# elybrand/quantized_neural_networks

Hardware: AMD Instinct MI355X
Metric: weights_quantized_per_sec (higher is better)
Workload: dtype f64; 1 GPU; Dense(4096->4096) whole-layer GPFQ, m=1024 calibration samples, M=3 alphabet, alphabet_scalar=3 (BASELINE.json configs[1], the north-star layer); N=4096, C=4096, m=1024, M=3, neurons_per_gpu=4096, arithmetic=f32 products / f64 residual and dot products (reference's mixed flow)

## Files before the change

quantized_neural_networks_amd/csrc/gpfq_blk.hip:

```cpp
#include <atomic>
#include <cmath>
#include <cstring>
#include <type_traits>

#include <cstdlib>
#include <mutex>
#include <optional>
#include <utility>
#include "gpfq_device.hpp"
#include <hip/hip_ext.h>
#include "gpfq_launch.hpp"
#include "gpfq_roles.hpp"

namespace gpfq {

namespace {

struct BlkStats {
    double rden, G, cb, ca, Ea, nrm;
    double sE1, sE2;
};
struct BandEntry {
    double H1, H2, E1, E2;
};
static_assert(sizeof(BlkStats) == 64 && sizeof(BandEntry) == 32, "header layout");

__host__ __device__ constexpr int blk_band(int B, bool CL = false) { return CL ? 3 * B - 1 : 2 * B - 1; }
__host__ __device__ constexpr int blk_hdr_bytes(int B, bool CL = false) { return (64 + blk_band(B, CL) * 32 + 127) & ~127; }
__host__ __device__ constexpr bool blk_row64(int G, int B) { return B > 1 && G > 1; }
__host__ __device__ constexpr int64_t blk_rec_bytes(int64_t mp, int B, int G, bool CL = false) { return blk_hdr_bytes(B, CL) + (blk_row64(G, B) ? 16 : 12) * mp; }

template <int B, bool R64, bool CL = false>
__global__ void __launch_bounds__(256)
gpfq_blk_prep_kernel(const float *__restrict__ X, const float *__restrict__ Xq, int64_t ld, int64_t N, int m, int mp,
                     const float *__restrict__ nrm32, char *__restrict__ recs, char *__restrict__ hdrs,
                     const DevAlphabet *__restrict__ alpha, int sym, int nsl, int64_t slice_bytes)
{
    const float sym_a = sym ? alpha->sym_a : 0.f;
    constexpr int GREC = R64 ? 2 : 1;
    constexpr int ND = blk_band(B, CL), NV = 3 + 4 * ND;
    constexpr int DN = CL ? 2 * B : B;
    __shared__ double sm[4][((NV + 3) & ~3) + 1];
    const int64_t t = blockIdx.x;
    constexpr int hdr = blk_hdr_bytes(B, CL);
    const int mps = nsl > 1 ? mp / nsl : mp;
    char *rb = recs + t * blk_rec_bytes(mps, B, GREC, CL);
    float  *ox = reinterpret_cast<float *>(rb + hdr);
    float  *oq = ox + mps;
    double *od = reinterpret_cast<double *>(rb + hdr + 8 * (int64_t)mps);
    const bool has_prev = t >= B && t - B < N, has_cur = t < N, has_next = t + DN < N;
    const float *px = X + (t - B) * ld, *pq = Xq + (t - B) * ld;
    const float *cx = X + t * ld, *cq = Xq + t * ld;
    const float *nq = Xq + (t + DN) * ld;
    const int lane = threadIdx.x & 63, wave = threadIdx.x >> 6;
    const double up = 1.0 + 0x1p-20;

    constexpr int NP = (NV + 3) & ~3;
    double v[NP];
#pragma unroll
    for (int k = 0; k < NP; ++k) v[k] = 0.0;
    auto one = [&](float xc, float qc_, const float (&bx)[ND], const float (&bq)[ND]) {
        const double q = (double)qc_, pr = q * (double)xc;
        v[0] += pr; v[1] += fabs(pr); v[2] += fabs(q);
#pragma unroll
        for (int d = 1; d <= ND; ++d) {
            const double p1 = q * (double)bx[d - 1], p2 = q * (double)bq[d - 1];
            v[3 + 4 * (d - 1) + 0] += p1;       v[3 + 4 * (d - 1) + 1] += p2;
            v[3 + 4 * (d - 1) + 2] += fabs(p1); v[3 + 4 * (d - 1) + 3] += fabs(p2);
        }
    };
    const bool vec = (ld % 4 == 0) && (((uintptr_t)X | (uintptr_t)Xq) % 16 == 0);
    if (vec) {
        const float4 z4 = make_float4(0.f, 0.f, 0.f, 0.f);
        for (int i = 4 * threadIdx.x; i < mp; i += 1024) {
            auto row = [&](const float *base, int64_t r) -> float4 {
                if (r < 0 || r >= N || i >= m) return z4;
                float4 w = *reinterpret_cast<const float4 *>(base + r * ld + i);
                if (i + 3 >= m) { w.y = i + 1 < m ? w.y : 0.f; w.z = i + 2 < m ? w.z : 0.f; w.w = 0.f; }
                return w;
            };
            const float4 xp = row(X, t - B), qp = row(Xq, t - B), qn = row(Xq, t + DN);
            const float4 xc = row(X, t), qc4 = row(Xq, t);
            float4 bx4[ND], bq4[ND];
#pragma unroll
            for (int d = 1; d <= ND; ++d) { bx4[d - 1] = row(X, t - d); bq4[d - 1] = row(Xq, t - d); }
            const int sl = nsl > 1 ? i / mps : 0, il = i - sl * mps;
            const int64_t so = (int64_t)sl * slice_bytes;
            float *oxs = reinterpret_cast<float *>(reinterpret_cast<char *>(ox) + so), *oqs = reinterpret_cast<float *>(reinterpret_cast<char *>(oq) + so);
            double *ods = reinterpret_cast<double *>(reinterpret_cast<char *>(od) + so);
            *reinterpret_cast<float4 *>(oxs + il) = xp;
            *reinterpret_cast<float4 *>(oqs + il) = sym_a != 0.f ? make_float4(__fmul_rn(sym_a, qp.x), __fmul_rn(sym_a, qp.y), __fmul_rn(sym_a, qp.z), __fmul_rn(sym_a, qp.w)) : qp;
            if constexpr (R64) {
                *reinterpret_cast<double2 *>(ods + il) = make_double2((double)qn.x, (double)qn.y);
                *reinterpret_cast<double2 *>(ods + il + 2) = make_double2((double)qn.z, (double)qn.w);
            } else {
                *reinterpret_cast<float4 *>(reinterpret_cast<float *>(ods) + il) = qn;
            }
            float b1[ND], b2[ND];
#pragma unroll
            for (int d = 0; d < ND; ++d) { b1[d] = bx4[d].x; b2[d] = bq4[d].x; }
            one(xc.x, qc4.x, b1, b2);
#pragma unroll
            for (int d = 0; d < ND; ++d) { b1[d] = bx4[d].y; b2[d] = bq4[d].y; }
            one(xc.y, qc4.y, b1, b2);
#pragma unroll
            for (int d = 0; d < ND; ++d) { b1[d] = bx4[d].z; b2[d] = bq4[d].z; }
            one(xc.z, qc4.z, b1, b2);
#pragma unroll
            for (int d = 0; d < ND; ++d) { b1[d] = bx4[d].w; b2[d] = bq4[d].w; }
            one(xc.w, qc4.w, b1, b2);
        }
    } else {
        for (int i = threadIdx.x; i < mp; i += 256) {
            const bool in = i < m;
            const int sl = nsl > 1 ? i / mps : 0, il = i - sl * mps;
            const int64_t so = (int64_t)sl * slice_bytes;
            float *oxs = reinterpret_cast<float *>(reinterpret_cast<char *>(ox) + so), *oqs = reinterpret_cast<float *>(reinterpret_cast<char *>(oq) + so);
            double *ods = reinterpret_cast<double *>(reinterpret_cast<char *>(od) + so);
            oxs[il] = (has_prev && in) ? px[i] : 0.f;
            oqs[il] = (has_prev && in) ? (sym_a != 0.f ? __fmul_rn(sym_a, pq[i]) : pq[i]) : 0.f;
            if constexpr (R64) ods[il] = (double)((has_next && in) ? nq[i] : 0.f);
            else reinterpret_cast<float *>(ods)[il] = (has_next && in) ? nq[i] : 0.f;
            if (has_cur && in) {
                float b1[ND], b2[ND];
#pragma unroll
                for (int d = 1; d <= ND; ++d) {
                    b1[d - 1] = t - d >= 0 ? X[(t - d) * ld + i] : 0.f;
                    b2[d - 1] = t - d >= 0 ? Xq[(t - d) * ld + i] : 0.f;
                }
                one(cx[i], cq[i], b1, b2);
            }
        }
    }
#pragma unroll
    for (int g = 0; g < NP / 4; ++g) {
        double x = fold16(fold32(v[4 * g], v[4 * g + 2]), fold32(v[4 * g + 1], v[4 * g + 3]));
        x = ror_add<8>(x); x = ror_add<4>(x); x = ror_add<2>(x); x = ror_add<1>(x);
        if ((lane & 15) == 0) sm[wave][4 * g + (lane >> 4)] = x;
    }
    __syncthreads();
    auto total = [&](int k) { return (sm[0][k] + sm[1][k]) + (sm[2][k] + sm[3][k]); };
    if (threadIdx.x == 0) {
        BlkStats st{};
        const double nrm = has_cur ? (double)nrm32[t] : 0.0;
        const double s1 = total(1), s2 = total(2);
        st.nrm = nrm;
        st.rden = nrm < 1e-16 ? 0.0 : 1.0 / (nrm * nrm);
        st.G = total(0);
        st.cb = 0x1p-23 * s1 * st.rden * up;
        st.ca = 0x1p-149 * s2 * st.rden * up;
        st.Ea = 0x1p-149 * s2 * up;
        double e1 = 0.0, e2 = 0.0;
#pragma unroll
        for (int d = 1; d <= ND; ++d) { e1 += total(5 + 4 * (d - 1)); e2 += total(6 + 4 * (d - 1)); }
        st.sE1 = 0x1p-23 * e1 * up * up; st.sE2 = 0x1p-23 * e2 * up * up;
        for (int sl = 0; sl < (nsl > 1 ? nsl : 1); ++sl) *reinterpret_cast<BlkStats *>(rb + (int64_t)sl * slice_bytes) = st;
        *reinterpret_cast<BlkStats *>(hdrs + t * hdr) = st;
    } else if (threadIdx.x <= ND) {
        const int d = threadIdx.x;
        BandEntry e;
        e.H1 = total(3 + 4 * (d - 1)); e.H2 = total(4 + 4 * (d - 1));
        e.E1 = 0x1p-23 * total(5 + 4 * (d - 1)) * up; e.E2 = 0x1p-23 * total(6 + 4 * (d - 1)) * up;
        for (int sl = 0; sl < (nsl > 1 ? nsl : 1); ++sl) *reinterpret_cast<BandEntry *>(rb + (int64_t)sl * slice_bytes + 64 + 32 * (d - 1)) = e;
        *reinterpret_cast<BandEntry *>(hdrs + t * hdr + 64 + 32 * (d - 1)) = e;
    }
}

constexpr int kPrepRunMax = 16;
template <int B, bool R64>
__global__ void __launch_bounds__(256)
gpfq_blk_prep_run_kernel(const float *__restrict__ X, const float *__restrict__ Xq, int64_t ld, int64_t N, int m, int mp, int64_t nrec, int RUN,
                         const float *__restrict__ nrm32, char *__restrict__ recs, char *__restrict__ hdrs,
                         const DevAlphabet *__restrict__ alpha, int sym, unsigned *__restrict__ zero16)
{
    constexpr int GREC = R64 ? 2 : 1;
    constexpr int ND = blk_band(B), NV = 3 + 4 * ND, NP = (NV + 3) & ~3;
    constexpr int hdr = blk_hdr_bytes(B);
    __shared__ double sm[kPrepRunMax][4][NP + 1];
    __shared__ double nsm[kPrepRunMax][4];
    const bool own_norms = nrm32 == nullptr;
    if (zero16 && blockIdx.x == 0 && threadIdx.x < 16) zero16[threadIdx.x] = 0u;
    const float sym_a = sym ? alpha->sym_a : 0.f;
    const int64_t t0 = (int64_t)blockIdx.x * RUN;
    const int lane = threadIdx.x & 63, wave = threadIdx.x >> 6;
    const double up = 1.0 + 0x1p-20;
    for (int k = threadIdx.x; k < RUN * 4 * (NP + 1); k += 256) (&sm[0][0][0])[k] = 0.0;
    __syncthreads();
    const float4 z4 = make_float4(0.f, 0.f, 0.f, 0.f);
    const int64_t rbytes = blk_rec_bytes(mp, B, GREC);
    for (int i = 4 * threadIdx.x; i < mp; i += 1024) {
        auto row = [&](const float *base, int64_t r) -> float4 {
            if (r < 0 || r >= N || i >= m) return z4;
            float4 w = *reinterpret_cast<const float4 *>(base + r * ld + i);
            if (i + 3 >= m) { w.y = i + 1 < m ? w.y : 0.f; w.z = i + 2 < m ? w.z : 0.f; w.w = 0.f; }
            return w;
        };
        float4 wx[ND], wq[ND];
#pragma unroll
        for (int d = 1; d <= ND; ++d) { wx[d - 1] = row(X, t0 - d); wq[d - 1] = row(Xq, t0 - d); }
        float4 xc = row(X, t0), qc4 = row(Xq, t0), qn = row(Xq, t0 + B);
#pragma unroll 1
        for (int r = 0; r < RUN; ++r) {
            const int64_t t = t0 + r;
            const float4 xc1 = r + 1 < RUN ? row(X, t + 1) : z4, qc1 = r + 1 < RUN ? row(Xq, t + 1) : z4, qn1 = r + 1 < RUN ? row(Xq, t + 1 + B) : z4;
            if (t < nrec) {
                char *rb = recs + t * rbytes;
                float *ox = reinterpret_cast<float *>(rb + hdr), *oq = ox + mp;
                const float4 xp = wx[B - 1], qp = wq[B - 1];
                *reinterpret_cast<float4 *>(ox + i) = xp;
                *reinterpret_cast<float4 *>(oq + i) = sym_a != 0.f ? make_float4(__fmul_rn(sym_a, qp.x), __fmul_rn(sym_a, qp.y), __fmul_rn(sym_a, qp.z), __fmul_rn(sym_a, qp.w)) : qp;
                if constexpr (R64) {
                    double *od = reinterpret_cast<double *>(rb + hdr + 8 * (int64_t)mp);
                    *reinterpret_cast<double2 *>(od + i) = make_double2((double)qn.x, (double)qn.y);
                    *reinterpret_cast<double2 *>(od + i + 2) = make_double2((double)qn.z, (double)qn.w);
                } else {
                    *reinterpret_cast<float4 *>(reinterpret_cast<float *>(rb + hdr + 8 * (int64_t)mp) + i) = qn;
                }
            }
            if (own_norms) {
                double s = 0.0;
                s = fma((double)qc4.x, (double)qc4.x, s);
                s = fma((double)qc4.y, (double)qc4.y, s);
                s = fma((double)qc4.z, (double)qc4.z, s);
                s = fma((double)qc4.w, (double)qc4.w, s);
                s = wave_sum(s);
                if (lane == 0) nsm[r][wave] = s;
            }
            double v[NP];
#pragma unroll
            for (int k = 0; k < NP; ++k) v[k] = 0.0;
            auto one = [&](float xcs, float qcs, const float (&bx)[ND], const float (&bq)[ND]) {
                const double q = (double)qcs, pr = q * (double)xcs;
                v[0] += pr; v[1] += fabs(pr); v[2] += fabs(q);
#pragma unroll
                for (int d = 1; d <= ND; ++d) {
                    const double p1 = q * (double)bx[d - 1], p2 = q * (double)bq[d - 1];
                    v[3 + 4 * (d - 1) + 0] += p1;       v[3 + 4 * (d - 1) + 1] += p2;
                    v[3 + 4 * (d - 1) + 2] += fabs(p1); v[3 + 4 * (d - 1) + 3] += fabs(p2);
                }
            };
            float b1[ND], b2[ND];
#pragma unroll
            for (int d = 0; d < ND; ++d) { b1[d] = wx[d].x; b2[d] = wq[d].x; }
            one(xc.x, qc4.x, b1, b2);
#pragma unroll
            for (int d = 0; d < ND; ++d) { b1[d] = wx[d].y; b2[d] = wq[d].y; }
            one(xc.y, qc4.y, b1, b2);
#pragma unroll
            for (int d = 0; d < ND; ++d) { b1[d] = wx[d].z; b2[d] = wq[d].z; }
            one(xc.z, qc4.z, b1, b2);
#pragma unroll
            for (int d = 0; d < ND; ++d) { b1[d] = wx[d].w; b2[d] = wq[d].w; }
            one(xc.w, qc4.w, b1, b2);
#pragma unroll
            for (int g = 0; g < NP / 4; ++g) {
                double x = fold16(fold32(v[4 * g], v[4 * g + 2]), fold32(v[4 * g + 1], v[4 * g + 3]));
                x = ror_add<8>(x); x = ror_add<4>(x); x = ror_add<2>(x); x = ror_add<1>(x);
                if ((lane & 15) == 0) sm[r][wave][4 * g + (lane >> 4)] += x;
            }
#pragma unroll
            for (int d = ND - 1; d >= 1; --d) { wx[d] = wx[d - 1]; wq[d] = wq[d - 1]; }
            wx[0] = xc; wq[0] = qc4;
            xc = xc1; qc4 = qc1; qn = qn1;
        }
    }
    __syncthreads();
    for (int w = threadIdx.x; w < RUN * (ND + 1); w += 256) {
        const int r = w / (ND + 1), e = w - r * (ND + 1);
        const int64_t t = t0 + r;
        if (t >= nrec) continue;
        auto total = [&](int k) { return (sm[r][0][k] + sm[r][1][k]) + (sm[r][2][k] + sm[r][3][k]); };
        char *rb = recs + t * rbytes;
        if (e == 0) {
            BlkStats st{};
            const double nrm = t < N ? (own_norms ? (double)(float)sqrt(nsm[r][0] + nsm[r][1] + nsm[r][2] + nsm[r][3]) : (double)nrm32[t]) : 0.0;
            const double s1 = total(1), s2 = total(2);
            st.nrm = nrm;
            st.rden = nrm < 1e-16 ? 0.0 : 1.0 / (nrm * nrm);
            st.G = total(0);
            st.cb = 0x1p-23 * s1 * st.rden * up;
            st.ca = 0x1p-149 * s2 * st.rden * up;
            st.Ea = 0x1p-149 * s2 * up;
            double e1 = 0.0, e2 = 0.0;
#pragma unroll
            for (int d = 1; d <= ND; ++d) { e1 += total(5 + 4 * (d - 1)); e2 += total(6 + 4 * (d - 1)); }
            st.sE1 = 0x1p-23 * e1 * up * up; st.sE2 = 0x1p-23 * e2 * up * up;
            *reinterpret_cast<BlkStats *>(rb) = st;
            *reinterpret_cast<BlkStats *>(hdrs + t * hdr) = st;
        } else {
            const int d = e;
            BandEntry be;
            be.H1 = total(3 + 4 * (d - 1)); be.H2 = total(4 + 4 * (d - 1));
            be.E1 = 0x1p-23 * total(5 + 4 * (d - 1)) * up; be.E2 = 0x1p-23 * total(6 + 4 * (d - 1)) * up;
            *reinterpret_cast<BandEntry *>(rb + 64 + 32 * (d - 1)) = be;
            *reinterpret_cast<BandEntry *>(hdrs + t * hdr + 64 + 32 * (d - 1)) = be;
        }
    }
}

__global__ void __launch_bounds__(256)
gpfq_blk_scale_kernel(char *__restrict__ recs, int64_t rec_bytes, int hdr, int mps, int64_t slice_bytes, const DevAlphabet *__restrict__ alpha)
{
    const float a = alpha->sym_a;
    float4 *row = reinterpret_cast<float4 *>(recs + (int64_t)blockIdx.y * slice_bytes + (int64_t)blockIdx.x * rec_bytes + hdr + 4 * (int64_t)mps);
    for (int i = threadIdx.x; i < mps / 4; i += 256) {
        const float4 v = row[i];
        row[i] = make_float4(__fmul_rn(a, v.x), __fmul_rn(a, v.y), __fmul_rn(a, v.z), __fmul_rn(a, v.w));
    }
}

template <int G, int NL, bool CL = false> constexpr bool blk_sweep_flush() { return (G == 4 && NL == 1) || CL; }

struct BlkLds {
    int tile_bytes, tile_pitch, off_w, off_d, off_wq, off_x2, off_e, off_out, off_ctl, off_zero, off_hr, hr_pitch, total;
};
constexpr int kOutSteps = 32;

__host__ __device__ constexpr int blk_sublanes(int nb) { return 64 / nb > 8 ? 8 : 64 / nb; }
__host__ __device__ constexpr int blk_slots(int nsw, int nb) { return (nsw + blk_sublanes(nb) - 1) / blk_sublanes(nb) * blk_sublanes(nb); }

__host__ __device__ inline BlkLds blk_lds(int mp, int nb, int B, int nsw, int G, bool CL = false)
{
    BlkLds L;
    const int nw = blk_slots(nsw, nb);
    L.tile_bytes = B * (int)blk_rec_bytes(mp, B, G, CL);
    L.tile_pitch = (L.tile_bytes + 1023) & ~1023;
    int o = 2 * L.tile_pitch;
    L.off_w = o;    o += 2 * nb * B * 4;    o = (o + 15) & ~15;
    L.off_d = o;    o += 2 * nw * B * nb * 8;
    L.off_wq = o;   o += 2 * nb * B * 8;
    L.off_x2 = o;   o += nw * nb * 16;
    L.off_e = o;    o += 68 * 8;
    L.off_out = o;  o += nb * kOutSteps * 8;
    L.off_ctl = o;  o += 16;
    L.off_zero = o; o += 32;
    o = (o + 15) & ~15;
    L.hr_pitch = (B * blk_hdr_bytes(B, CL) + 1023) & ~1023;
    L.off_hr = o;   o += 3 * L.hr_pitch;
    L.total = o;
    return L;
}

struct BlkK {
    const char *recs;
    const char *hdrs;
    const float *Wt;
    int64_t ldw, ldt;
    int64_t N, C;
    int m, M, zero_idx, nblk;
    int8_t *qidx;
    float *Qt;
    int64_t o_sj, o_st;
    const DevAlphabet *alpha;
    int *alpha_err;
    double *resid, *u_out;
    unsigned long long *fallback_count;
    unsigned long long *stamps;
    const float *Xq;
    int64_t ldx;
    unsigned char pw[12];
    int nsl;
    int cl_map;
    int64_t slice_bytes;
    unsigned long long *mbox;
    int64_t u_ld;
    double slack;
    int *cl_err;
    unsigned long long cl_timeout;
    int cl_fault;
};

constexpr int kTop3Ship = 3;
constexpr int kPkAheadShip = 3;
struct BlkPrioSched { int d21[3], d10[3]; };
constexpr BlkPrioSched kPrioSched[2] = {{{4, 4, 4}, {8, 8, 8}}, {{2, 4, 6}, {6, 8, 10}}};
constexpr int kPrioShip = 3 + 4 * 1;
#ifdef GPFQ_BLK_DIAG
#include "gpfq_blk_diag.hpp"
#else
constexpr bool kNoMfmaD = false, kNoFused = false;
constexpr int kTop3 = kTop3Ship;
constexpr int kPkAhead = kPkAheadShip;
constexpr int kPrio = kPrioShip;
#define STAMP(var) do { } while (0)
#define STAMP_DO(...)
#endif

struct ClState { int64_t cl; int slice; unsigned seq; bool dead; int64_t rec_off; int m_sl; };
typedef unsigned cl_u32x4 __attribute__((ext_vector_type(4)));

__device__ __forceinline__ cl_u32x4 cl_load16(const unsigned long long *p)
{
    cl_u32x4 r;
    asm volatile("global_load_dwordx4 %0, %1, off sc1" : "=&v"(r) : "v"(p) : "memory");
    return r;
}

template <int KV>
__device__ __forceinline__ void cl_publish(const BlkK &K, ClState &cs, int lane, const double (&v)[KV])
{
    const unsigned seq = ++cs.seq;
    if (K.cl_fault && cs.cl == 0 && cs.slice == 1) return;
    unsigned long long *buf = K.mbox + ((cs.cl * 2 + (int64_t)(seq & 1u)) * (int64_t)K.nsl) * 256;
    unsigned long long *mine = buf + ((int64_t)cs.slice * 64 + lane) * 4;
#pragma unroll
    for (int k = 0; k < KV; ++k) {
        const cl_u32x4 w = {(unsigned)__double2loint(v[k]), seq, (unsigned)__double2hiint(v[k]), seq};
        asm volatile("global_store_dwordx4 %0, %1, off sc1" :: "v"(mine + 2 * k), "v"(w) : "memory");
// ... 50 lines not shown
template <int KV, int CLB>
__device__ __forceinline__ void cl_exchange(const BlkK &K, ClState &cs, int lane, double (&v)[KV])
{
    cl_publish<KV>(K, cs, lane, v);
    cl_gather<KV, CLB>(K, cs, lane, v);
}

struct BlkPairs { int pw[11]; };
constexpr BlkPairs kP8{{1, 1, 1, 1, 1, 1, 1, 1}}, kP12{{1, 2, 2, 1, 1, 2, 2, 1}}, kP16{{1, 2, 2, 2, 1, 3, 3, 2}},
                   kP24{{1, 3, 3, 3, 2, 4, 4, 4}}, kP32{{2, 4, 4, 4, 3, 5, 5, 5}}, kP40{{5, 5, 5, 5, 5, 5, 5, 5}};
constexpr BlkPairs kP16x7{{3, 3, 2, 1, 3, 2, 2}}, kP24x7{{4, 4, 4, 1, 4, 4, 3}}, kP32x7{{5, 5, 5, 2, 5, 5, 5}};
constexpr BlkPairs kP32quad{{2, 5, 5, 4, 2, 5, 5, 4}};
constexpr BlkPairs kP16x11{{2, 2, 1, 1, 2, 2, 1, 1, 1, 1, 2}}, kP24x11{{2, 2, 2, 2, 2, 2, 2, 1, 3, 3, 3}}, kP32x11{{3, 3, 3, 3, 3, 3, 3, 2, 3, 3, 3}},
                   kP48x11{{4, 5, 4, 4, 5, 4, 4, 5, 4, 4, 5}}, kP64x11{{4, 6, 6, 6, 6, 6, 6, 6, 6, 6, 6}};
constexpr BlkPairs kP64oct{{6, 6, 6, 6, 6, 6, 6, 4, 6, 6, 6}};
struct BlkInst { int G, S, B, NSW, NL, CLM; BlkPairs split; };
constexpr BlkInst kBlkInst[] = {
    {4, 16, 4,  7, 1, 0, kP16x7},   {4, 16, 4,  7, 2, 0, kP16x7},   {4, 24, 4,  7, 1, 0, kP24x7},   {4, 24, 4,  7, 2, 0, kP24x7},   {4, 32, 4,  7, 1, 0, kP32x7},   {4, 32, 4,  7, 2, 0, kP32x7},
    {4, 16, 4,  8, 1, 0, kP16},     {4, 16, 4,  8, 2, 0, kP16},     {4, 24, 4,  8, 1, 0, kP24},     {4, 24, 4,  8, 2, 0, kP24},     {4, 32, 4,  8, 1, 0, kP32quad}, {4, 32, 4,  8, 2, 0, kP32quad},
    {1,  4, 4,  4, 1, 0, {{1, 1, 1, 1}}}, {1,  4, 4,  4, 2, 0, {{1, 1, 1, 1}}},
    {1,  8, 4,  8, 1, 0, kP8},      {1,  8, 4,  8, 2, 0, kP8},      {1, 12, 2,  8, 1, 0, kP12},     {1, 12, 2,  8, 2, 0, kP12},
    {1, 16, 2,  8, 1, 0, kP16},     {1, 16, 2,  8, 2, 0, kP16},     {1, 24, 1,  8, 1, 0, kP24},     {1, 24, 1,  8, 2, 0, kP24},
    {1, 32, 1,  8, 1, 0, kP32},     {1, 32, 1,  8, 2, 0, kP32},     {1, 40, 1,  8, 1, 0, kP40},     {1, 40, 1,  8, 2, 0, kP40},
    {1, 40, 1,  8, 4, 0, kP40},     {2, 48, 1, 11, 4, 0, kP48x11},  {2, 64, 1, 11, 4, 0, kP64x11},  {1, 24, 1,  8, 4, 0, kP24},     {1, 32, 1,  8, 4, 0, kP32},
    {4, 48, 2, 11, 4, 0, kP48x11},  {4, 64, 2, 11, 4, 0, kP64x11},
    {4, 16, 4, 11, 4, 0, kP16x11},  {4, 24, 4, 11, 4, 0, kP24x11},  {4, 32, 4, 11, 4, 0, kP32x11},  {8, 64, 4, 11, 2, 0, kP64oct},
    {4, 16, 4,  8, 4, 0, kP16},     {4, 24, 4,  8, 4, 0, kP24},     {4, 32, 4,  8, 4, 0, kP32},
    {1,  8, 4,  8, 4, 0, kP8},      {1, 12, 2,  8, 4, 0, kP12},     {1, 16, 2,  8, 4, 0, {{1, 2, 2, 3, 2, 2, 2, 2}}},
    {2, 16, 4,  8, 4, 0, kP16},     {2, 24, 2,  8, 4, 0, kP24},     {2, 32, 2,  8, 4, 0, kP32},
    {4, 24, 4,  8, 4, 1, kP24},     {4, 24, 4, 11, 4, 1, kP24x11},  {4, 32, 4, 11, 4, 1, kP32x11},  {8, 64, 4, 11, 2, 1, kP64oct},  {4, 32, 4,  8, 1, 1, kP32quad}, {4, 32, 4,  8, 2, 1, kP32quad},
};
constexpr int kBlkInsts = (int)(sizeof(kBlkInst) / sizeof(kBlkInst[0]));
constexpr bool blk_sym_only(const BlkInst &r) { return r.G == 8; }

constexpr int blk_inst_find(int G, int S, int B, int NSW, int NL, int CLM)
{
    int row = -1;
    for (int i = 0; i < kBlkInsts && (B < 0 || row < 0); ++i) {
        const BlkInst &r = kBlkInst[i];
        if (r.G != G || r.S != S || r.NSW != NSW || r.NL != NL || (B >= 0 && (r.B != B || r.CLM != CLM))) continue;
        if (row < 0) row = i;
        for (int w = 0; w < 11; ++w)
            if (r.split.pw[w] != kBlkInst[row].split.pw[w]) return -1;
    }
    return row;
}
constexpr int blk_pairs(const BlkInst &r) { int n = 0; for (int w = 0; w < r.NSW; ++w) n += r.split.pw[w]; return n; }

template <int G, int S, int NSW, int NL> constexpr const int *blk_split()
{
    constexpr int row = blk_inst_find(G, S, -1, NSW, NL, 0);
    static_assert(row >= 0, "kBlkInst has no row for this instantiation, or two with different splits");
    static_assert(blk_pairs(kBlkInst[row]) == S, "the row's pairs do not sum to S");
    return kBlkInst[row].split.pw;
}

template <int G, int S, int NSW, int NL> constexpr bool blk_split_has(int k)
{
    for (int w = 0; w < NSW; ++w)
        if (blk_split<G, S, NSW, NL>()[w] == k) return true;
    return false;
}

template <int G, int PW, int MP, int B, int NSW, bool SYM, int NL, int CLM>
__device__ __forceinline__ void blk_sweep_role(const BlkK &K, char *lds_generic, const BlkLds &L, int wave, int lane, int pbase, const ClState &cs)
{
    constexpr bool CL = CLM != 0;
    constexpr int NB = NL * G, KQ = 64 / G, NW = blk_slots(NSW, NB);
    constexpr int RSH = NL == 4 ? 0 : (NL == 2 ? 1 : 2);
    constexpr int HDR = blk_hdr_bytes(B, CL);
    constexpr int RB = (int)blk_rec_bytes(MP, B, G, CL);
    lchar *lds = (lchar *)lds_generic;
    const int ng = lane & (G - 1), kq = lane / G, row = lane >> 4;
    const bool writer = (lane & 15 & ~(G - 1)) == 0 && (row & ((1 << RSH) - 1)) == 0;
    const int nloc = NL * ng;
    const int nrow = row >> RSH;
    const int64_t jbase = cs.cl * NB;
    const unsigned ldsT_addr = lds_addr(lds_generic), ldsW_addr = lds_addr(lds_generic + L.off_w);
    const int64_t N = K.N;
    const int nslots = K.nblk + 1;
    constexpr int PU = G == 8 ? 2 : 1;
    static_assert(PW % PU == 0, "whole units per wavefront");
    auto pair_off = [](int p) { return PU * (p / PU) * KQ + p % PU; };
    const int o_x  = HDR + 8 * (pbase + PU * kq);
    int o_q = o_x + 4 * MP;
    asm volatile("" : "+v"(o_q));
    constexpr int DB = blk_row64(G, B) ? 16 : 8;
    const int o_d  = HDR + 8 * MP + DB * (pbase + PU * kq);
    using DRaw = std::conditional_t<blk_row64(G, B), double2, float2>;
    auto ld_d = [&](int off) -> DRaw { return lds_ld<DRaw>(lds, off); };
    auto to_d2 = [](const DRaw &v) -> double2 { return make_double2((double)v.x, (double)v.y); };
    const int o_wq = L.off_wq + nloc * B * 8;
    const int o_dw = L.off_d + (wave * B * NB + nloc + nrow) * 8;
    const int o_x2 = L.off_x2 + (wave * NB + nloc + nrow) * 16;

    double u[NL][2 * PW];
#pragma unroll
    for (int i = 0; i < NL; ++i)
#pragma unroll
        for (int e = 0; e < 2 * PW; ++e) u[i][e] = 0.0;

    constexpr int NPIECES = (B * RB + 1023) >> 10;
    constexpr int PER_MIN = NPIECES / NSW;
    constexpr int PTS = PW >= 2 ? 2 : 1;
    constexpr int PPP = PER_MIN / (PTS * B) > 0 ? PER_MIN / (PTS * B) : 1;
    const unsigned lane16 = (unsigned)lane * 16u;
    auto issue_piece = [&](int b1, int k) {
        const int pc = wave + NSW * k;
        glds16_s(K.recs + (CL ? cs.rec_off : (int64_t)0) + (int64_t)b1 * L.tile_bytes + ((int64_t)pc << 10), lane16,
                 ldsT_addr + (unsigned)(b1 & 1) * (unsigned)L.tile_pitch + ((unsigned)pc << 10));
    };
    auto load_weights = [&](int b1) {
        const unsigned dw = ldsW_addr + (unsigned)((b1 & 1) * NB * B * 4);
        for (int i0 = wave * 64; i0 < NB * B; i0 += NSW * 64) {
            const int i = i0 + lane;
            const int n = i / B, s = i - n * B;
            const int64_t jn = jbase + n, t = (int64_t)b1 * B + s;
            if (i < NB * B && jn < K.C && t < N) glds4(K.Wt + jn * K.ldw + t * K.ldt, dw + 4 * (unsigned)i0);
        }
    };

    constexpr int NHP = (B * HDR + 1023) >> 10;
    auto load_headers = [&](int b2, int buf) {
        if (wave < NHP && b2 <= K.nblk)
            glds16_s(K.hdrs + (int64_t)b2 * B * HDR + ((int64_t)wave << 10), lane16,
                     lds_addr(lds_generic + L.off_hr) + (unsigned)buf * (unsigned)L.hr_pitch + ((unsigned)wave << 10));
    };
    for (int k = 0; wave + NSW * k < NPIECES; ++k) issue_piece(0, k);
    load_weights(0);
    load_headers(0, 0); load_headers(1, 1);
    dma_wait();
    slot_barrier();
    int hbuf = 2;
    unsigned long long st0 = 0, st1 = 0, st2 = 0, st3 = 0, st4 = 0, st5 = 0, acc_dma = 0, acc_u = 0, acc_d = 0, acc_w = 0, acc_b = 0, acc_t = 0;
    (void)st0; (void)st1; (void)st2; (void)st3; (void)st4; (void)st5; (void)acc_dma; (void)acc_u; (void)acc_d; (void)acc_w; (void)acc_b; (void)acc_t;

    constexpr bool kMfmaD = (G == 4 || (G == 8 && NL == 2)) && B == 4 && blk_row64(G, B) && (!kNoMfmaD || G == 8);
    constexpr bool kFused = kMfmaD && (!kNoFused || G == 8);
    static_assert(G != 8 || kFused, "the eight-group lane map exists in the fused form only");
    constexpr bool kBatchTop = kFused && (NL == 4 || G == 8) && NSW == 11;
    constexpr bool kTopSym = kBatchTop && SYM;
    constexpr int kPrioForm = CL ? (kPrio >> 2) & 3 : kPrio & 3;
    constexpr bool kPrioUp = kTopSym && G == 8 && (kPrioForm & 1) != 0;
    constexpr int NUW = PW / PU;
    constexpr bool kLateHdr = kTopSym && NUW >= 2 && (kTop3 & 1) != 0, kLateW = kTopSym && NUW >= 2 && (kTop3 & 2) != 0;
    constexpr int kHdrStep = NUW >= 3 ? 8 : 6, kWStep = NUW >= 3 ? 10 : 7;
    static_assert(!(kLateHdr || kLateW) || (NUW <= 3 && B == 4 && PTS == 2 && PER_MIN <= 6), "the free pair-steps of a two- or three-pair wavefront");
    static_assert(!kLateW || NB * B == 64, "one 256-byte weight piece per block");
    unsigned long long w_lanes = 0ull, w_tail = 0ull;
    int w_whole = 0;
    const float *wsrc = nullptr;
    if constexpr (kLateW) {
        w_lanes = wave == 0 ? __builtin_amdgcn_ballot_w64(jbase + lane / B < K.C) : 0ull;
        w_tail = w_lanes & (0x1111111111111111ull * ((1ull << (int)(N % B)) - 1ull));
        w_whole = (int)(N / B);
        wsrc = K.Wt + (jbase + lane / B) * K.ldw + (int64_t)(B + lane % B) * K.ldt;
    }
    (void)w_lanes; (void)w_tail; (void)w_whole; (void)wsrc;
    constexpr bool kPreloadAll = PW * B <= 8 && PW <= 5 && !kFused;
    constexpr bool kHoist = kPreloadAll && PW * B <= 4;
    constexpr int PB = kPreloadAll ? B : 1, PP = kPreloadAll ? PW : 1;
    constexpr bool kPreD = kHoist && PW * B * (blk_row64(G, B) ? 4 : 2) <= 16 && !kMfmaD;
    constexpr int DBn = kPreD ? B : 1, DPn = kPreD ? PW : 1;
    float2 xs[PB][PP], qs[PB][PP], wqa[PB][NL];
    DRaw ds[DBn][DPn];
    auto preload_wq = [&](int b) {
        const int pbq = ((b - 1) & 1) * NB * B * 8;
#pragma unroll
        for (int s = 0; s < PB; ++s)
#pragma unroll
            for (int n = 0; n < NL; ++n) wqa[s][n] = lds_ld<float2>(lds, o_wq + pbq + (n * B + s) * 8);
    };
    auto preload_rows = [&](int b) {
        const int tbase = (b & 1) * L.tile_pitch;
#pragma unroll
        for (int s = 0; s < PB; ++s)
#pragma unroll
            for (int p = 0; p < PP; ++p) {
                xs[s][p] = lds_ld<float2>(lds, tbase + s * RB + o_x + 8 * p * KQ);
                qs[s][p] = lds_ld<float2>(lds, tbase + s * RB + o_q + 8 * p * KQ);
                if constexpr (kPreD) ds[s][p] = ld_d(tbase + s * RB + o_d + DB * p * KQ);
            }
    };
    if constexpr (kHoist) { preload_wq(0); preload_rows(0); }

    auto slow_path = [&](int b, int ctl) {
        for (;;) {
            const int S = __builtin_amdgcn_readfirstlane(ctl);
            if (S < 0) break;
            const int nb_ = ((b + 1) & 1) * L.tile_pitch;
            const int cbq = (b & 1) * NB * B * 8;
            double eu[NL], ew[NL];
#pragma unroll
            for (int n = 0; n < NL; ++n) { eu[n] = 0.0; ew[n] = 0.0; }
#pragma unroll
            for (int n = 0; n < NL; ++n) {
                const float w = lds_ld<float2>(lds, o_wq + cbq + (n * B + S) * 8).x;
#pragma unroll 1
                for (int p = 0; p < PW; ++p) {
                    double t0 = u[n][0], t1 = u[n][1];
#pragma unroll
                    for (int pp = 1; pp < PW; ++pp) { t0 = (p == pp) ? u[n][2 * pp] : t0; t1 = (p == pp) ? u[n][2 * pp + 1] : t1; }
                    for (int j = 0; j < S; ++j) {
                        const int rb = nb_ + j * RB;
                        const float2 x2 = lds_ld<float2>(lds, rb + o_x + 8 * pair_off(p)), q2 = lds_ld<float2>(lds, rb + o_q + 8 * pair_off(p));
                        const float2 wq = lds_ld<float2>(lds, o_wq + cbq + (n * B + j) * 8);
                        if constexpr (SYM) {
                            t0 += (double)__fmaf_rn(wq.y, q2.x, __fmul_rn(wq.x, x2.x));
                            t1 += (double)__fmaf_rn(wq.y, q2.y, __fmul_rn(wq.x, x2.y));
                        } else {
                            t0 += (double)__fsub_rn(__fmul_rn(wq.x, x2.x), __fmul_rn(wq.y, q2.x));
                            t1 += (double)__fsub_rn(__fmul_rn(wq.x, x2.y), __fmul_rn(wq.y, q2.y));
                        }
                    }
                    const int rb = nb_ + S * RB;
                    const float2 x2 = lds_ld<float2>(lds, rb + o_x + 8 * pair_off(p));
                    float2 q2;
                    if constexpr (SYM) {
                        const int i0 = 2 * (pbase + pair_off(p) + PU * kq);
                        const float *xr = K.Xq + ((int64_t)b * B + S) * K.ldx + (CL ? (int64_t)cs.slice * MP : (int64_t)0);
                        const int mrow = CL ? cs.m_sl : K.m;
                        q2.x = i0 < mrow ? xr[i0] : 0.f;
                        q2.y = i0 + 1 < mrow ? xr[i0 + 1] : 0.f;
                    } else {
                        q2 = lds_ld<float2>(lds, rb + o_q + 8 * pair_off(p));
                    }
                    eu[n] = fma((double)q2.x, t0, eu[n]);
                    eu[n] = fma((double)q2.y, t1, eu[n]);
                    ew[n] = fma((double)q2.x, t0 + (double)__fmul_rn(w, x2.x), ew[n]);
                    ew[n] = fma((double)q2.y, t1 + (double)__fmul_rn(w, x2.y), ew[n]);
                }
            }
            const double vu = fold_klanes_n<G, NL>(eu), vw = fold_klanes_n<G, NL>(ew);
            if (writer) lds_st<double2>(lds, o_x2, make_double2(vu, vw));
            slot_barrier();
            slot_barrier();
            if constexpr (kBatchTop) ctl = lds_read_now(lds + L.off_ctl + 4 * (b & 1));
            else ctl = lds_ld<int>(lds, L.off_ctl + 4 * (b & 1));
        }
    };
    if constexpr (kBatchTop) __builtin_amdgcn_s_waitcnt(0);
    for (int b = 0; b < nslots; ++b) {
        STAMP(st0);
        STAMP_DO(if (b) acc_t += st0 - st5;)
        if (blk_sweep_flush<G, NL, CL>() && b >= 1 && wave == b % NSW && lane < NB * B && (!CL || cs.slice == 0)) {
            const int nn = lane / B, sidx = lane % B;
            const int64_t t = (int64_t)(b - 1) * B + sidx, jn = jbase + nn;
            if (t < N && jn < K.C) {
                const int2 v = lds_ld<int2>(lds, L.off_out + (nn * kOutSteps + (int)(t % kOutSteps)) * 8);
                if (K.qidx) K.qidx[jn * N + t] = (int8_t)v.x;
                if (K.Qt) K.Qt[jn * N + t] = __int_as_float(v.y);
            }
        }
        if constexpr (!kLateW) {
            if (b + 1 < nslots) load_weights(b + 1);
        }
        if constexpr (!kLateHdr) { load_headers(b + 2, hbuf); hbuf = hbuf == 2 ? 0 : hbuf + 1; }
        const int bn = b + 1 < nslots ? b + 1 : b;
        STAMP(st1);
        const int tbase = (b & 1) * L.tile_pitch;
        const int pbq = ((b - 1) & 1) * NB * B * 8;

        auto update_pair = [&](int p, const float2 &x2, const float2 &q2, const float (&wv)[NL], const float (&qv)[NL]) {
            const pk2 xv = {x2.x, x2.y}, qx = {q2.x, q2.y};
            pk2 pr[NL], rr[NL], dd[NL];
            double c0[NL], c1[NL];
#pragma unroll
            for (int n = 0; n < NL; ++n) pr[n] = pk2{wv[n], wv[n]} * xv;
            if constexpr (SYM) {
#pragma unroll
                for (int n = 0; n < NL; ++n) dd[n] = __builtin_elementwise_fma(pk2{qv[n], qv[n]}, qx, pr[n]);
            } else {
#pragma unroll
                for (int n = 0; n < NL; ++n) rr[n] = pk2{qv[n], qv[n]} * qx;
#pragma unroll
                for (int n = 0; n < NL; ++n) dd[n] = pr[n] - rr[n];
            }
#pragma unroll
            for (int n = 0; n < NL; ++n) { c0[n] = (double)dd[n].x; c1[n] = (double)dd[n].y; }
#pragma unroll
            for (int n = 0; n < NL; ++n) { u[n][2 * p] += c0[n]; u[n][2 * p + 1] += c1[n]; }
        };
        auto update_unit2 = [&](int P, const float4 &x4, const float4 &q4, const float (&wv)[NL], const float (&qv)[NL]) {
            const pk2 xv[2] = {{x4.x, x4.y}, {x4.z, x4.w}}, qx[2] = {{q4.x, q4.y}, {q4.z, q4.w}};
            pk2 pr[2][NL], rr[2][NL], dd[2][NL];
            double c0[2][NL], c1[2][NL];
#pragma unroll
            for (int h = 0; h < 2; ++h)
#pragma unroll
                for (int n = 0; n < NL; ++n) pr[h][n] = pk2{wv[n], wv[n]} * xv[h];
            if constexpr (SYM) {
#pragma unroll
                for (int h = 0; h < 2; ++h)
#pragma unroll
                    for (int n = 0; n < NL; ++n) dd[h][n] = __builtin_elementwise_fma(pk2{qv[n], qv[n]}, qx[h], pr[h][n]);
            } else {
#pragma unroll
                for (int h = 0; h < 2; ++h)
#pragma unroll
                    for (int n = 0; n < NL; ++n) rr[h][n] = pk2{qv[n], qv[n]} * qx[h];
#pragma unroll
                for (int h = 0; h < 2; ++h)
#pragma unroll
                    for (int n = 0; n < NL; ++n) dd[h][n] = pr[h][n] - rr[h][n];
            }
#pragma unroll
            for (int h = 0; h < 2; ++h)
#pragma unroll
                for (int n = 0; n < NL; ++n) { c0[h][n] = (double)dd[h][n].x; c1[h][n] = (double)dd[h][n].y; }
#pragma unroll
            for (int h = 0; h < 2; ++h)
#pragma unroll
                for (int n = 0; n < NL; ++n) { u[n][4 * P + 2 * h] += c0[h][n]; u[n][4 * P + 2 * h + 1] += c1[h][n]; }
        };
        (void)update_unit2;
        auto unit2_products = [&](pk2 (&dd)[2][NL], const float4 &x4, const float4 &q4, const float2 (&wq)[NL]) {
            const pk2 xv[2] = {{x4.x, x4.y}, {x4.z, x4.w}}, qx[2] = {{q4.x, q4.y}, {q4.z, q4.w}};
#pragma unroll
            for (int h = 0; h < 2; ++h)
#pragma unroll
                for (int n = 0; n < NL; ++n) dd[h][n] = pk2{wq[n].x, wq[n].x} * xv[h];
#pragma unroll
            for (int h = 0; h < 2; ++h)
#pragma unroll
                for (int n = 0; n < NL; ++n) dd[h][n] = __builtin_elementwise_fma(pk2{wq[n].y, wq[n].y}, qx[h], dd[h][n]);
        };
        auto unit2_accumulate_ahead = [&](int P, pk2 (&dd)[2][NL], bool nxt, const float4 &x4, const float4 &q4, const float2 (&wq)[NL]) {
            const pk2 xv[2] = {{x4.x, x4.y}, {x4.z, x4.w}}, qx[2] = {{q4.x, q4.y}, {q4.z, q4.w}};
            double c0[2][NL], c1[2][NL];
#pragma unroll
            for (int h = 0; h < 2; ++h)
#pragma unroll
                for (int n = 0; n < NL; ++n) {
                    c0[h][n] = (double)dd[h][n].x; c1[h][n] = (double)dd[h][n].y;
                    if (nxt) dd[h][n] = pk2{wq[n].x, wq[n].x} * xv[h];
                    __builtin_amdgcn_sched_barrier(0);
                }
#pragma unroll
            for (int h = 0; h < 2; ++h)
#pragma unroll
                for (int n = 0; n < NL; ++n) {
                    u[n][4 * P + 2 * h] += c0[h][n]; u[n][4 * P + 2 * h + 1] += c1[h][n];
                    if (nxt) dd[h][n] = __builtin_elementwise_fma(pk2{wq[n].y, wq[n].y}, qx[h], dd[h][n]);
                    __builtin_amdgcn_sched_barrier(0);
                }
        };
        (void)unit2_products; (void)unit2_accumulate_ahead;
        if constexpr (kFused) {
            const int rbm = tbase + (G == 8 ? lane & 3 : ng) * RB + o_d;
            constexpr int NU = PW / PU;
            constexpr bool kRows2 = kTopSym && G == 8 && (kPkAhead & 1) != 0;
            constexpr bool kPkA = kRows2 && (kPkAhead & 2) != 0;
            constexpr int PF = (NSW == 7 || kRows2) ? 2 : 1, NPS = NU * B;
            using XRow = std::conditional_t<PU == 2, float4, float2>;
            struct DRow2 { double2 v[2]; };
            using DRow = std::conditional_t<PU == 2, DRow2, double2>;
            auto dhalf = [](const DRow &r, int h) -> const double2 & { if constexpr (PU == 2) return r.v[h]; else return r; };
            float2 fwq[B][NL];
            XRow xbuf[PF], qbuf[PF];
            DRow dcur;
            auto row_off = [&](int i, bool q) { return tbase + (i % B) * RB + (q ? o_q : o_x) + 8 * PU * (i / B) * KQ; };
            auto ld_drow = [&](int off) -> DRow {
                if constexpr (PU == 2) return DRow{{lds_ld<double2>(lds, off), lds_ld<double2>(lds, off + 16)}};
                else return lds_ld<double2>(lds, off);
            };
            auto first_requests = [&]() {
#pragma unroll
                for (int s = 0; s < B; ++s)
#pragma unroll
                    for (int n = 0; n < NL; ++n) fwq[s][n] = lds_ld<float2>(lds, o_wq + pbq + (n * B + s) * 8);
#pragma unroll
                for (int i = 0; i < PF; ++i)
                    if (i < NPS) { xbuf[i] = lds_ld<XRow>(lds, row_off(i, false)); qbuf[i] = lds_ld<XRow>(lds, row_off(i, true)); }
                dcur = ld_drow(rbm);
            };
            if constexpr (kTopSym && G == 8) {
                static_assert(!(kTopSym && G == 8) || (B == 4 && NL == 2 && PU == 2 && PF == (kRows2 ? 2 : 1) && NPS >= 4), "slot_top_sym2: two neurons per lane, pair-steps 0..2 are unit 0's steps 0..2");
                nf4 w01[2], w23[2], x2n, q2n;
                nd2 d01[2];
                __builtin_amdgcn_s_setprio(2);
                slot_top_sym2<RB>(w01, w23, x2n, q2n, d01, u[0][0], u[0][1], u[0][2], u[0][3], u[1][0], u[1][1], u[1][2], u[1][3],
                                  lds + row_off(0, false), lds + row_off(0, true), lds + o_wq + pbq, lds + rbm);
                __builtin_amdgcn_s_waitcnt(0xC07F);
                __builtin_memcpy(&xbuf[0], &x2n, sizeof(XRow)); __builtin_memcpy(&qbuf[0], &q2n, sizeof(XRow));
                if constexpr (kRows2) { xbuf[PF - 1] = lds_ld<XRow>(lds, row_off(3, false)); qbuf[PF - 1] = lds_ld<XRow>(lds, row_off(3, true)); }
#pragma unroll
                for (int h = 0; h < PU; ++h) dcur.v[h] = make_double2(d01[h].x, d01[h].y);
#pragma unroll
                for (int n = 0; n < NL; ++n) {
                    fwq[0][n] = make_float2(w01[n].x, w01[n].y); fwq[1][n] = make_float2(w01[n].z, w01[n].w);
                    fwq[2][n] = make_float2(w23[n].x, w23[n].y); fwq[3][n] = make_float2(w23[n].z, w23[n].w);
                }
            } else if constexpr (kTopSym) {
                static_assert(!kTopSym || (B == 4 && NL == 4 && PF == 1), "slot_top_sym: four neurons per lane, pair-steps 0..2 are pair 0's steps 0..2");
                nf4 w01[4], w23[4];
                nf2 x2n, q2n;
                nd2 d0;
                __builtin_amdgcn_s_setprio(2);
                slot_top_sym<RB>(w01, w23, x2n, q2n, d0, u[0][0], u[0][1], u[1][0], u[1][1], u[2][0], u[2][1], u[3][0], u[3][1],
                                 lds + row_off(0, false), lds + row_off(0, true), lds + o_wq + pbq, lds + rbm);
                __builtin_amdgcn_s_waitcnt(0xC07F);
                xbuf[0] = make_float2(x2n.x, x2n.y); qbuf[0] = make_float2(q2n.x, q2n.y);
                dcur = make_double2(d0.x, d0.y);
#pragma unroll
                for (int n = 0; n < NL; ++n) {
                    fwq[0][n] = make_float2(w01[n].x, w01[n].y); fwq[1][n] = make_float2(w01[n].z, w01[n].w);
                    fwq[2][n] = make_float2(w23[n].x, w23[n].y); fwq[3][n] = make_float2(w23[n].z, w23[n].w);
                }
            } else if constexpr (kBatchTop) {
                static_assert(!kBatchTop || (B == 4 && NL == 4), "lds_read_slot_top reads four neurons' steps 0 and 1: 16 bytes at a stride of 4 steps x 8 bytes");
                nf2 x0, q0;
                nf4 w01[4];
                lds_read_slot_top(x0, q0, w01, lds + row_off(0, false), lds + row_off(0, true), lds + o_wq + pbq);
                xbuf[0] = make_float2(x0.x, x0.y); qbuf[0] = make_float2(q0.x, q0.y);
#pragma unroll
                for (int n = 0; n < NL; ++n) { fwq[0][n] = make_float2(w01[n].x, w01[n].y); fwq[1][n] = make_float2(w01[n].z, w01[n].w); }
#pragma unroll
                for (int s = 2; s < B; ++s)
#pragma unroll
                    for (int n = 0; n < NL; ++n) fwq[s][n] = lds_ld<float2>(lds, o_wq + pbq + (n * B + s) * 8);
                dcur = lds_ld<double2>(lds, rbm);
            } else {
                first_requests();
            }
            pk2 ddn[2][NL];
            if constexpr (kPkA) unit2_products(ddn, xbuf[2 % PF], qbuf[2 % PF], fwq[2]);
            (void)ddn;
            DRow dprev;
            if constexpr (PU == 2) dprev = DRow{{make_double2(0.0, 0.0), make_double2(0.0, 0.0)}};
            else dprev = make_double2(0.0, 0.0);
            double acc[NL];
#pragma unroll
            for (int n = 0; n < NL; ++n) acc[n] = 0.0;
            constexpr int NM = 2 * PU * NL;
            auto mfma_pair = [&](int pp, int i, const DRow &dd) {
                const int n = i % NL, e = i / NL;
                const double2 &dh = dhalf(dd, e / 2);
                acc[n] = __builtin_amdgcn_mfma_f64_4x4x4f64(u[n][2 * PU * pp + e], (e & 1) ? dh.y : dh.x, acc[n], 0, 0, 0);
            };
            constexpr int kSched = (kTopSym && G == 8 && NU == 3) ? (kPrioForm >> 1) & 1 : 0;
            auto prio_at = [&](int ips) {
                constexpr BlkPrioSched sc = kPrioSched[kSched];
                if (sc.d21[0] == sc.d21[1] && sc.d21[1] == sc.d21[2]) {
                    if (ips == sc.d21[0]) __builtin_amdgcn_s_setprio(1);
                } else {
                    if (ips == sc.d21[0]) setprio_if_age<0, 1>(wave);
                    if (ips == sc.d21[1]) setprio_if_age<1, 1>(wave);
                    if (ips == sc.d21[2]) setprio_if_age<2, 1>(wave);
                }
                if (sc.d10[0] == sc.d10[1] && sc.d10[1] == sc.d10[2]) {
                    if (ips == sc.d10[0]) __builtin_amdgcn_s_setprio(0);
                } else {
                    if (ips == sc.d10[0]) setprio_if_age<0, 0>(wave);
                    if (ips == sc.d10[1]) setprio_if_age<1, 0>(wave);
                    if (ips == sc.d10[2]) setprio_if_age<2, 0>(wave);
                }
            };
            (void)prio_at;
#pragma unroll
            for (int p = 0; p < NU; ++p) {
                if constexpr (kSched != 0) {
                    if (p == 0) __builtin_amdgcn_s_setprio(2);
                } else {
                    const int pr = 2 - (3 * p) / NU;
                    if (p == 0 || pr != 2 - (3 * (p - 1)) / NU) {
                        const int v = pr;
                        if (v >= 2) __builtin_amdgcn_s_setprio(2);
                        else if (v == 1) __builtin_amdgcn_s_setprio(1);
                        else __builtin_amdgcn_s_setprio(0);
                    }
                }
                if (p > 0) dcur = ld_drow(rbm + DB * PU * p * KQ);
#pragma unroll
                for (int st = 0; st < B; ++st) {
                    const int ips = p * B + st;
                    if (kTopSym && ips < 2) continue;
                    const XRow x2 = xbuf[ips % PF], q2 = qbuf[ips % PF];
                    const int pn = (ips + 1) / B, sn = (ips + 1) % B;
                    (void)pn; (void)sn;
                    if (ips + PF < NPS) {
                        xbuf[ips % PF] = lds_ld<XRow>(lds, row_off(ips + PF, false));
                        qbuf[ips % PF] = lds_ld<XRow>(lds, row_off(ips + PF, true));
                    }
                    if (kTopSym && ips < 4) {
#pragma unroll
                        for (int i = 0; i < PPP; ++i) {
                            const int k = (PTS * (ips - 2)) * PPP + i;
                            if (PTS * B * PPP <= PER_MIN || k < PER_MIN) issue_piece(bn, k);
                        }
                    }
                    if (p < PTS) {
#pragma unroll
                        for (int i = 0; i < PPP; ++i) {
                            const int k = (PTS * st + p) * PPP + i;
                            if (PTS * B * PPP <= PER_MIN || k < PER_MIN) issue_piece(bn, k);
                        }
                    }
                    if (kLateHdr && ips == kHdrStep) {
                        int b2 = b + 2;
                        asm volatile("" : "+s"(b2));
                        const unsigned on = ((unsigned)(wave - NHP) & (unsigned)(b2 - K.nblk - 1)) >> 31;
                        glds16_s_lanes(K.hdrs + (int64_t)b2 * B * HDR + ((int64_t)wave << 10), lane16,
                                       lds_addr(lds_generic + L.off_hr) + (unsigned)hbuf * (unsigned)L.hr_pitch + ((unsigned)wave << 10), 0ull - (unsigned long long)on);
                        hbuf = hbuf == 2 ? 0 : hbuf + 1;
                    }
                    if (kLateW && ips == kWStep) {
                        int b1 = b + 1;
                        asm volatile("" : "+s"(b1));
                        glds4_lanes(wsrc, ldsW_addr + (unsigned)((b1 & 1) * NB * B * 4), b1 < w_whole ? w_lanes : b1 == w_whole ? w_tail : 0ull);
                        wsrc += (int64_t)B * K.ldt;
                    }
                    __builtin_amdgcn_sched_barrier(0);
                    if constexpr (kSched != 0) prio_at(ips);
                    float wv[NL], qv[NL];
#pragma unroll
                    for (int n = 0; n < NL; ++n) { wv[n] = fwq[st][n].x; qv[n] = fwq[st][n].y; }
                    if constexpr (kPkA) unit2_accumulate_ahead(p, ddn, ips + 1 < NPS, xbuf[(ips + 1) % PF], qbuf[(ips + 1) % PF], fwq[(st + 1) % B]);
                    else if constexpr (PU == 2) update_unit2(p, x2, q2, wv, qv);
                    else update_pair(p, x2, q2, wv, qv);
                    if (p > 0) {
#pragma unroll
                        for (int i = 0; i < NM; ++i)
                            if (i * B / NM == st) mfma_pair(p - 1, i, dprev);
                    }
                    __builtin_amdgcn_sched_barrier(0);
                }
                dprev = dcur;
            }
            for (int k = PTS * B * PPP < PER_MIN ? PTS * B * PPP : PER_MIN; wave + NSW * k < NPIECES; ++k) issue_piece(bn, k);
            STAMP(st2);
#pragma unroll
            for (int i = 0; i < NM; ++i) mfma_pair(NU - 1, i, dprev);
#pragma unroll
            for (int n = 0; n < NL; ++n) {
                acc[n] = ror_add<8>(acc[n]);
                if constexpr (G == 4) acc[n] = ror_add<4>(acc[n]);
            }
            const bool dwriter = G == 8 ? (lane & 8) == 0 : (lane & 12) == 0;
            const int dgroup = G == 8 ? (lane >> 4) + (lane & 4) : lane >> 4;
            if (b + 1 < nslots && dwriter) {
                const int od = L.off_d + ((((((b + 1) & 1) * NW + wave) * B) + (lane & 3)) * NB + NL * dgroup) * 8;
                if constexpr (NL == 4) {
                    lds_st<double2>(lds, od, make_double2(acc[0], acc[1]));
                    lds_st<double2>(lds, od + 16, make_double2(acc[2], acc[3]));
                } else if constexpr (NL == 2) {
                    lds_st<double2>(lds, od, make_double2(acc[0], acc[NL - 1]));
                } else {
                    lds_st<double>(lds, od, acc[0]);
                }
            }
        } else {
        if constexpr (kPreloadAll) {
            if constexpr (!kHoist) { preload_wq(b); preload_rows(b); __builtin_amdgcn_sched_barrier(0); }
#pragma unroll
            for (int s = 0; s < B; ++s) {
                if (s == 0) __builtin_amdgcn_s_setprio(2);
                if (s == B / 2) __builtin_amdgcn_s_setprio(1);
                float wv[NL], qv[NL];
#pragma unroll
                for (int n = 0; n < NL; ++n) { wv[n] = wqa[s][n].x; qv[n] = wqa[s][n].y; }
#pragma unroll
                for (int p = 0; p < PW; ++p) {
                    if (p < PTS) {
#pragma unroll
                        for (int i = 0; i < PPP; ++i) {
                            const int k = (PTS * s + p) * PPP + i;
                            if (PTS * B * PPP <= PER_MIN || k < PER_MIN) issue_piece(bn, k);
                        }
                    }
                    update_pair(p, xs[s][p], qs[s][p], wv, qv);
                    __builtin_amdgcn_sched_barrier(0);
                }
            }
        } else
        {
            float2 x2n = lds_ld<float2>(lds, tbase + o_x), q2n = lds_ld<float2>(lds, tbase + o_q);
            float2 wqn[NL];
#pragma unroll
            for (int n = 0; n < NL; ++n) wqn[n] = lds_ld<float2>(lds, o_wq + pbq + (n * B) * 8);
#pragma clang loop unroll_count(B == 4 ? 2 : 1)
            for (int s = 0; s < B; ++s) {
                if (s == 0) __builtin_amdgcn_s_setprio(2);
                if (s == B / 2) __builtin_amdgcn_s_setprio(1);
                float wv[NL], qv[NL];
#pragma unroll
                for (int n = 0; n < NL; ++n) { wv[n] = wqn[n].x; qv[n] = wqn[n].y; }
                const int rb = tbase + s * RB;
                const int sn = s + 1 < B ? s + 1 : s;
#pragma unroll
                for (int n = 0; n < NL; ++n) wqn[n] = lds_ld<float2>(lds, o_wq + pbq + (n * B + sn) * 8);
#pragma unroll
                for (int p = 0; p < PW; ++p) {
                    const float2 x2 = x2n, q2 = q2n;
                    const int rbn = p + 1 < PW ? rb : tbase + sn * RB, pn = p + 1 < PW ? p + 1 : 0;
                    x2n = lds_ld<float2>(lds, rbn + o_x + 8 * pn * KQ);
                    q2n = lds_ld<float2>(lds, rbn + o_q + 8 * pn * KQ);
                    if (p < PTS) {
#pragma unroll
                        for (int i = 0; i < PPP; ++i) {
                            const int k = (PTS * s + p) * PPP + i;
                            if (PTS * B * PPP <= PER_MIN || k < PER_MIN) issue_piece(bn, k);
                        }
                    }
                    __builtin_amdgcn_sched_barrier(0);
                    update_pair(p, x2, q2, wv, qv);
                    __builtin_amdgcn_sched_barrier(0);
                }
            }
        }
        for (int k = PTS * B * PPP < PER_MIN ? PTS * B * PPP : PER_MIN; wave + NSW * k < NPIECES; ++k) issue_piece(bn, k);
        STAMP(st2);
        if constexpr (kMfmaD) {
            if (b + 1 < nslots) {
                __builtin_amdgcn_s_setprio(0);
                double acc[NL];
#pragma unroll
                for (int n = 0; n < NL; ++n) acc[n] = 0.0;
                const int rbm = tbase + ng * RB + o_d;
                double2 d2n = lds_ld<double2>(lds, rbm);
#pragma unroll
                for (int p = 0; p < PW; ++p) {
                    const double2 d2 = d2n;
                    if (p + 1 < PW) d2n = lds_ld<double2>(lds, rbm + DB * (p + 1) * KQ);
#pragma unroll
                    for (int n = 0; n < NL; ++n) acc[n] = __builtin_amdgcn_mfma_f64_4x4x4f64(u[n][2 * p], d2.x, acc[n], 0, 0, 0);
#pragma unroll
                    for (int n = 0; n < NL; ++n) acc[n] = __builtin_amdgcn_mfma_f64_4x4x4f64(u[n][2 * p + 1], d2.y, acc[n], 0, 0, 0);
                }
#pragma unroll
                for (int n = 0; n < NL; ++n) { acc[n] = ror_add<8>(acc[n]); acc[n] = ror_add<4>(acc[n]); }
                if ((lane & 12) == 0) {
                    const int od = L.off_d + ((((((b + 1) & 1) * NW + wave) * B) + (lane & 3)) * NB + NL * (lane >> 4)) * 8;
#pragma unroll
                    for (int n = 0; n < NL; ++n) lds_st<double>(lds, od + 8 * n, acc[n]);
                }
            }
        } else
        if (b + 1 < nslots && kPreloadAll) {
            DRaw dsl[B][PW];
#pragma unroll
            for (int r = 0; r < B; ++r)
#pragma unroll
                for (int p = 0; p < PW; ++p) {
                    if constexpr (kPreD) dsl[r][p] = ds[r][p];
                    else dsl[r][p] = ld_d(tbase + r * RB + o_d + DB * p * KQ);
                }
            if constexpr (!kPreD) __builtin_amdgcn_sched_barrier(0);
#pragma unroll
            for (int r = 0; r < B; ++r) {
                if (r == B / 2) __builtin_amdgcn_s_setprio(0);
                double acc[NL];
#pragma unroll
                for (int n = 0; n < NL; ++n) acc[n] = 0.0;
#pragma unroll
                for (int p = 0; p < PW; ++p) {
                    const double2 d2 = to_d2(dsl[r][p]);
#pragma unroll
                    for (int n = 0; n < NL; ++n) {
                        acc[n] = fma(d2.x, u[n][2 * p], acc[n]);
                        acc[n] = fma(d2.y, u[n][2 * p + 1], acc[n]);
                    }
                }
                const double v = fold_klanes_n<G, NL>(acc);
                if (writer) lds_st<double>(lds, o_dw + ((((b + 1) & 1) * NW) * B + r) * NB * 8, v);
            }
        } else
        if (b + 1 < nslots) {
            DRaw d2n = ld_d(tbase + o_d);
#pragma clang loop unroll_count(B == 4 ? 2 : 1)
            for (int r = 0; r < B; ++r) {
                if (r == B / 2) __builtin_amdgcn_s_setprio(0);
                double acc[NL];
#pragma unroll
                for (int n = 0; n < NL; ++n) acc[n] = 0.0;
                const int rb = tbase + r * RB;
                const int rn = r + 1 < B ? r + 1 : r;
#pragma unroll
                for (int p = 0; p < PW; ++p) {
                    const double2 d2 = to_d2(d2n);
                    const int rbn = p + 1 < PW ? rb : tbase + rn * RB, pn = p + 1 < PW ? p + 1 : 0;
                    d2n = ld_d(rbn + o_d + DB * pn * KQ);
                    __builtin_amdgcn_sched_barrier(0);
#pragma unroll
                    for (int n = 0; n < NL; ++n) {
                        acc[n] = fma(d2.x, u[n][2 * p], acc[n]);
                        acc[n] = fma(d2.y, u[n][2 * p + 1], acc[n]);
                    }
                    __builtin_amdgcn_sched_barrier(0);
                }
                const double v = fold_klanes_n<G, NL>(acc);
                if (writer) lds_st<double>(lds, o_dw + ((((b + 1) & 1) * NW) * B + r) * NB * 8, v);
            }
        }
        }
        STAMP(st3);
        dma_wait();
        STAMP(st4);
        if constexpr (kPrioUp) __builtin_amdgcn_s_setprio(2);
        slot_barrier();
        STAMP(st5);
        STAMP_DO(acc_dma += st1 - st0; acc_u += st2 - st1; acc_d += st3 - st2; acc_w += st4 - st3; acc_b += st5 - st4;)

        {
        int ctl;
        if constexpr (kBatchTop) ctl = lds_read_now(lds + L.off_ctl + 4 * (b & 1));
        else ctl = lds_ld<int>(lds, L.off_ctl + 4 * (b & 1));
        if constexpr (kHoist) {
            if (b + 1 < nslots) { preload_wq(b + 1); preload_rows(b + 1); }
        }
        if (__builtin_amdgcn_readfirstlane(ctl) >= 0) {
            slow_path(b, ctl);
            if constexpr (kHoist) {
                if (b + 1 < nslots) { preload_wq(b + 1); preload_rows(b + 1); }
            }
        }
        }
    }

    STAMP_DO(
    if (K.stamps && blockIdx.x == 0 && lane == 0 && (wave == 0 || wave == 7)) {
        unsigned long long *o = K.stamps + (wave == 0 ? 0 : 8);
        o[0] = acc_dma; o[1] = acc_u; o[2] = acc_d; o[3] = acc_w; o[4] = acc_b; o[5] = (unsigned long long)nslots; o[6] = acc_t;
    }
    if (K.stamps && blockIdx.x == 0 && lane == 0) {
        K.stamps[32 + wave] = acc_dma + acc_u + acc_d + acc_w;
        if (K.N * (int64_t)sizeof(RowStats) >= 64 * 8) { K.stamps[21 + wave] = acc_t; K.stamps[48 + wave] = acc_b; }
    }
    )
    if constexpr (kPrioUp) __builtin_amdgcn_s_setprio(0);
    if constexpr (G == 8) {
        if (K.resid) {
            double ss[4];
#pragma unroll
            for (int n = 0; n < NL; ++n)
#pragma unroll
                for (int h = 0; h < PU; ++h) {
                    double q = 0.0;
#pragma unroll
                    for (int P = 0; P < PW / PU; ++P)
#pragma unroll
                        for (int e = 0; e < 2; ++e) q = fma(u[n][2 * (PU * P + h) + e], u[n][2 * (PU * P + h) + e], q);
                    ss[PU * n + h] = q;
                }
            double v = fold_klanes<G>(ss);
            v = fold16(v, v);
            if (writer) lds_st<double>(lds, o_dw, v);
        }
    } else
    if (K.resid) {
        double ss[NL];
#pragma unroll
        for (int n = 0; n < NL; ++n) {
            double q = 0.0;
#pragma unroll
            for (int e = 0; e < 2 * PW; ++e) q = fma(u[n][e], u[n][e], q);
            ss[n] = q;
        }
        const double v = fold_klanes_n<G, NL>(ss);
        if (writer) lds_st<double>(lds, o_dw, v);
    }
    slot_barrier();
    if (K.u_out) {
#pragma unroll
        for (int n = 0; n < NL; ++n) {
            const int64_t jn = jbase + nloc + n;
            if (jn < K.C) {
#pragma unroll
                for (int p = 0; p < PW; ++p)
#pragma unroll
                    for (int e = 0; e < 2; ++e) {
                        const int i = 2 * (pbase + pair_off(p) + PU * kq) + e;
                        if constexpr (CL) {
                            if (i < cs.m_sl) K.u_out[jn * K.u_ld + (int64_t)cs.slice * MP + i] = u[n][2 * p + e];
                        } else {
                            if (i < K.m) K.u_out[jn * (int64_t)K.m + i] = u[n][2 * p + e];
                        }
                    }
            }
        }
    }
}

template <int G, int MP, int B, int NSW, bool SYM, int NL, int CLM, bool KOUT = false>
__device__ __forceinline__ void blk_decision_role(const BlkK &K, char *lds_generic, const BlkLds &L, int lane, ClState &cs)
{
    constexpr bool CL = CLM != 0;
    constexpr int NB = NL * G, R = blk_sublanes(NB), NW = blk_slots(NSW, NB);
    constexpr int RB = (int)blk_rec_bytes(MP, B, G, CL);
    lchar *lds = (lchar *)lds_generic;
    const bool shadow = lane / R >= NB;
    const int n = shadow ? NB - 1 : lane / R, r = lane % R;
    const int64_t wg = cs.cl;
    const int64_t jn = wg * NB + n;
    const bool active = jn < K.C;
// ... 30 lines not shown

    constexpr bool kOwnFlush = !blk_sweep_flush<G, NL, CL>();
    auto flush = [&](int64_t t0, int64_t t1) {
        if constexpr (KOUT) {
            constexpr int NJ = NB < 8 ? NB : 8, GJ = NB / NJ;
            for (int e = lane; e < GJ * kOutSteps; e += 64) {
                const int g = e / kOutSteps, c = e % kOutSteps;
                const int64_t ts = t0 + c, j0 = wg * NB + g * NJ;
                if (ts >= t1 || j0 >= K.C || (CL && cs.slice != 0)) continue;
                int idxj[NJ]; float qj[NJ];
#pragma unroll
                for (int k = 0; k < NJ; ++k) {
                    const int2 v = lds_ld<int2>(lds, L.off_out + ((g * NJ + k) * kOutSteps + (int)(ts % kOutSteps)) * 8);
                    idxj[k] = v.x; qj[k] = __int_as_float(v.y);
                }
                const int64_t o = ts * K.o_st + j0;
                const bool whole = j0 + NJ <= K.C && K.o_sj == 1;
                if (K.qidx) {
                    if (whole && NJ >= 4 && ((uintptr_t)(K.qidx + o) & (NJ - 1)) == 0) {
                        unsigned lo = 0, hi = 0;
#pragma unroll
                        for (int k = 0; k < NJ; ++k) { if (k < 4) lo |= (unsigned)(idxj[k] & 0xff) << (8 * k); else hi |= (unsigned)(idxj[k] & 0xff) << (8 * (k - 4)); }
                        if constexpr (NJ == 8) *reinterpret_cast<uint2 *>(K.qidx + o) = make_uint2(lo, hi);
                        else *reinterpret_cast<unsigned *>(K.qidx + o) = lo;
                    } else {
#pragma unroll
                        for (int k = 0; k < NJ; ++k) if (j0 + k < K.C) K.qidx[ts * K.o_st + (j0 + k) * K.o_sj] = (int8_t)idxj[k];
                    }
                }
                if (K.Qt) {
                    if (whole && NJ >= 4 && ((uintptr_t)(K.Qt + o) & 15) == 0) {
#pragma unroll
                        for (int k = 0; k + 3 < NJ; k += 4) *reinterpret_cast<float4 *>(K.Qt + o + k) = make_float4(qj[k], qj[k + 1], qj[k + 2], qj[k + 3]);
                    } else {
#pragma unroll
                        for (int k = 0; k < NJ; ++k) if (j0 + k < K.C) K.Qt[ts * K.o_st + (j0 + k) * K.o_sj] = qj[k];
                    }
                }
            }
            return;
        }
        for (int e = lane; e < NB * (kOutSteps / 8); e += 64) {
            const int nn = e / (kOutSteps / 8), c = e % (kOutSteps / 8);
            const int64_t j = wg * NB + nn, ts = t0 + 8 * c;
            if (j >= K.C || ts >= t1 || (CL && cs.slice != 0)) continue;
            int idx8[8]; float q8[8];
#pragma unroll
            for (int k = 0; k < 8; ++k) {
                const int2 v = lds_ld<int2>(lds, L.off_out + (nn * kOutSteps + (int)((ts + k) % kOutSteps)) * 8);
                idx8[k] = v.x; q8[k] = __int_as_float(v.y);
            }
            if (ts + 8 <= t1 && ((j * N + ts) & 7) == 0) {
                if (K.qidx) {
                    unsigned lo = 0, hi = 0;
#pragma unroll
                    for (int k = 0; k < 4; ++k) { lo |= (unsigned)(idx8[k] & 0xff) << (8 * k); hi |= (unsigned)(idx8[4 + k] & 0xff) << (8 * k); }
                    *reinterpret_cast<uint2 *>(K.qidx + j * N + ts) = make_uint2(lo, hi);
                }
                if (K.Qt) {
                    float4 *dst = reinterpret_cast<float4 *>(K.Qt + j * N + ts);
                    if (((uintptr_t)dst & 15) == 0) {
                        dst[0] = make_float4(q8[0], q8[1], q8[2], q8[3]);
                        dst[1] = make_float4(q8[4], q8[5], q8[6], q8[7]);
                    } else {
#pragma unroll
                        for (int k = 0; k < 8; ++k) K.Qt[j * N + ts + k] = q8[k];
                    }
                }
            } else {
#pragma unroll
                for (int k = 0; k < 8; ++k)
                    if (ts + k < t1) {
                        if (K.qidx) K.qidx[j * N + ts + k] = (int8_t)idx8[k];
                        if (K.Qt)   K.Qt[j * N + ts + k]   = q8[k];
                    }
            }
        }
    };
    int64_t flushed = 0, flush_hi = 0;

    const int smh = lane & (B - 1);
    constexpr bool kHdrChain = NSW == 7;
    constexpr int BI = B > 1 ? B - 1 : 1, HDRB = blk_hdr_bytes(B, CL);
    double2 g01 = make_double2(0.0, 0.0);
    double2 ghp[B];
    double2 ghi[BI];
    auto prefetch_headers = [&](int buf) {
        const int rm = L.off_hr + buf * L.hr_pitch + smh * HDRB;
        g01 = lds_ld<double2>(lds, rm);
#pragma unroll
        for (int j = 0; j < B; ++j) ghp[j] = lds_ld<double2>(lds, rm + 64 + 32 * (B + smh - j - 1));
#pragma unroll
        for (int j = 0; j + 1 < B; ++j) ghi[j] = lds_ld<double2>(lds, j < smh ? rm + 64 + 32 * (smh - j - 1) : L.off_zero);
    };
    slot_barrier();
    if constexpr (!CL) prefetch_headers(0);
    int hnext = 1;
    __builtin_amdgcn_s_setprio(3);

    unsigned long long dt0 = 0, dt1 = 0, dt2 = 0, dta = 0, dtb = 0, dacc_work = 0, dacc_bar = 0, dacc_pro = 0, dacc_chain = 0, dacc_tail = 0;
    (void)dt0; (void)dt1; (void)dt2; (void)dta; (void)dtb; (void)dacc_work; (void)dacc_bar; (void)dacc_pro; (void)dacc_chain; (void)dacc_tail;
    for (int b = 0; b < nslots; ++b) {
        STAMP(dt0);
        STAMP_DO(if (b) dacc_tail += dt0 - dt2;)
        const int tbase = (b & 1) * L.tile_pitch;
        const int cbq = (b & 1) * NB * B * 8;
        float  wc[B], qc[B];
        double D[B];
        double DmT = 0.0;
        (void)DmT;
        int stop = B;
        double cPm = 0.0, ePm = 0.0;
        int ctl_now = -1;
        unsigned anyP = 0u;
#pragma unroll
        for (int j = 0; j < B; ++j) anyP |= __float_as_uint(wprev[j]) | __float_as_uint(qprev[j]);
        if constexpr (CL) {
#pragma unroll
            for (int j = 0; j < B; ++j) anyP |= __float_as_uint(wprev2[j]) | __float_as_uint(qprev2[j]);
        }
        const int nvalid = (int)min((int64_t)B, N - (int64_t)b * B);
        const int oslot0 = (int)(((int64_t)b * B) % kOutSteps);
        const int o_dummy = L.off_ctl + 8;
        auto quad_bcast = [&](double x, int s) -> double {
            int lo = __double2loint(x), hi = __double2hiint(x);
            if (s == 0) { lo = __builtin_amdgcn_mov_dpp(lo, 0x00, 0xF, 0xF, true); hi = __builtin_amdgcn_mov_dpp(hi, 0x00, 0xF, 0xF, true); }
            if (s == 1) { lo = __builtin_amdgcn_mov_dpp(lo, 0x55, 0xF, 0xF, true); hi = __builtin_amdgcn_mov_dpp(hi, 0x55, 0xF, 0xF, true); }
            if (s == 2) { lo = __builtin_amdgcn_mov_dpp(lo, 0xAA, 0xF, 0xF, true); hi = __builtin_amdgcn_mov_dpp(hi, 0xAA, 0xF, 0xF, true); }
            if (s == 3) { lo = __builtin_amdgcn_mov_dpp(lo, 0xFF, 0xF, 0xF, true); hi = __builtin_amdgcn_mov_dpp(hi, 0xFF, 0xF, 0xF, true); }
            return __hiloint2double(hi, lo);
        };
        if (b < K.nblk) {
            const int sm = smh;
            double dp[NW];
#pragma unroll
            for (int w = 0; w < NW; ++w) dp[w] = lds_ld<double>(lds, L.off_d + ((((b & 1) * NW + w) * B + sm) * NB + n) * 8);
#pragma unroll
            for (int s = 0; s < B; ++s) wc[s] = lds_ld<float>(lds, o_w + (b & 1) * NB * B * 4 + 4 * s);
            const float w_own_raw = lds_ld<float>(lds, o_w + (b & 1) * NB * B * 4 + 4 * sm);
            double2 hp2[CL ? B : 1];
            if constexpr (CL) {
                prefetch_headers(b % 3);
#pragma unroll
                for (int j = 0; j < B; ++j) hp2[j] = lds_ld<double2>(lds, tbase + sm * RB + 64 + 32 * (2 * B + sm - j - 1));
            }
            if constexpr (kOwnFlush) {
                if (flush_hi > flushed) {
                    flush(flushed, flush_hi);
                    flushed = flush_hi;
                }
            }
            double2 hp[B], hi_[BI];
            const double2 o01 = g01;
#pragma unroll
            for (int j = 0; j + 1 < B; ++j) hi_[j] = ghi[j];
#pragma unroll
            for (int s = 0; s < B; ++s) hp[s] = ghp[s];
            __builtin_amdgcn_sched_barrier(0);
            double wd[B];
#pragma unroll
            for (int s = 0; s < B; ++s) {
                wc[s] = s < nvalid ? wc[s] : 0.f;
                qc[s] = 0.f;
                wd[s] = (double)wc[s];
            }
            double Dm;
            {
                double t[NW];
#pragma unroll
                for (int w = 0; w < NW; ++w) t[w] = dp[w];
#pragma unroll
                for (int span = 1; span < NW; span *= 2)
#pragma unroll
                    for (int w = 0; w + span < NW; w += 2 * span) t[w] += t[w + span];
                Dm = t[0];
            }
#pragma unroll
            for (int j = 0; j < B; ++j) {
                const double wj = (double)wprev[j], qj = (double)qprev[j];
                cPm = fma(wj, hp[j].x, cPm); cPm = fma(-qj, hp[j].y, cPm);
            }
            if constexpr (CL) {
#pragma unroll
                for (int j = 0; j < B; ++j) {
                    const double wj = (double)wprev2[j], qj = (double)qprev2[j];
                    cPm = fma(wj, hp2[j].x, cPm); cPm = fma(-qj, hp2[j].y, cPm);
                }
            }
            double Aw = cPm;
#pragma unroll
            for (int j = 0; j + 1 < B; ++j) Aw = fma(wd[j], hi_[j].x, Aw);
            if constexpr (CL) {
                static_assert(!CL || (B == 4 && R % 4 == 0), "cluster form: a quad of lanes = the four steps of a neuron's block");
                __builtin_amdgcn_sched_barrier(0);
                if (b + 1 < K.nblk) {
                    const double xv[1] = {Dm};
                    cl_publish<1>(K, cs, lane, xv);
                }
                Dm = DmCur;
                DmT = Dm;
                __builtin_amdgcn_sched_barrier(0);
            }
            const double Am = Dm + Aw;
            double A[B];
#pragma unroll
            for (int s = 0; s < B; ++s) A[s] = quad_bcast(Am, s);
            const int rbm = tbase + sm * RB;
            const double2 o23 = lds_ld<double2>(lds, rbm + 16);
            const double rEa = lds_ld<double>(lds, rbm + 32);
            const double2 o67 = lds_ld<double2>(lds, rbm + 48);
            STAMP(dta);
            const double u_a0 = al_a0, u_step = al_step, u_inv = al_inv, u_c0 = al_c0, u_kmax = (double)(M - 1);
            const double u_amax = fmax(fabs(u_a0), fabs(fma(u_kmax, u_step, u_a0))) * (1.0 + 0x1p-20);
            const unsigned long long u_plus = al_plus, u_minus = al_minus;
            const int u_zero = K.zero_idx;
            const float sym_a32 = (float)sym_top;
            auto pick = [&](double tt, double &kd) -> float {
                if constexpr (SYM && NB <= 8) {
                    const bool up = tt > sym_hb, mid = tt > -sym_hb;
                    kd = up ? u_kmax : (mid ? 1.0 : 0.0);
                    return up ? sym_a32 : (mid ? 0.f : -sym_a32);
                }
                kd = fmin(fmax(rint(fma(tt, u_inv, u_c0)), 0.0), u_kmax);
                const int ki = (int)kd;
                const int adj = (int)((unsigned)(u_plus >> ki) & 1u) - (int)((unsigned)(u_minus >> ki) & 1u);
                const float v = __int_as_float(__float_as_int((float)fma(kd, u_step, u_a0)) + adj);
                return ki == u_zero ? 0.f : v;
            };
            float q32s[B];
            double qd[B];
#pragma unroll
            for (int s = 0; s < B; ++s) {
                const double rden_s = quad_bcast(o01.x, s), wG_s = wd[s] * quad_bcast(o01.y, s);
                double du = A[s];
#pragma unroll
                for (int j = 0; j + 1 < B; ++j)
                    if (j < s) du = fma(-qd[j], quad_bcast(hi_[j].y, s), du);
                const double tq = (du + wG_s) * rden_s;
                const double tt = fabs(du) < 1e-10 ? wd[s] : tq;
                double kd;
                float q32 = pick(tt, kd);
                q32 = rden_s == 0.0 ? 0.f : q32;
                q32s[s] = q32;
                qd[s] = (double)q32;
            }
            double du_m = Am;
#pragma unroll
            for (int j = 0; j + 1 < B; ++j) du_m = fma(-qd[j], hi_[j].y, du_m);
            if constexpr (kHdrChain) {
                if (b + 1 < K.nblk) prefetch_headers(hnext);
                __builtin_amdgcn_sched_barrier(0);
            }
            const bool valid_m = sm < nvalid;
            const float w_m = valid_m ? w_own_raw : 0.f;
            const double wdm = (double)w_m, rden = o01.x, wGm = wdm * o01.y;
            const double rcb = o23.x, rca = o23.y;
            const bool rule1 = rden == 0.0;
            const bool small = fabs(du_m) < 1e-10;
            const double tq_m = (du_m + wGm) * rden;
            const double tt_m = small ? wdm : tq_m;
            double kd_m;
            const float qk32 = pick(tt_m, kd_m);
            const int ki = (int)kd_m;
            double a_lo, a_k, a_hi;
            if constexpr (SYM) {
                const double kInfD = __longlong_as_double(0x7ff0000000000000LL);
                const double gap = M == 3 ? sym_top : 2.0 * sym_top;
                a_k = fma(kd_m, gap, -sym_top);
                a_lo = ki == 0 ? -kInfD : a_k - gap;
                a_hi = ki == M - 1 ? kInfD : a_k + gap;
            } else
            {
                const int oe = L.off_e + 8 * (1 + ki);
                a_lo = lds_ld<double>(lds, oe); a_k = lds_ld<double>(lds, oe + 8); a_hi = lds_ld<double>(lds, oe + 16);
            }
            const double d_k = fabs(a_k - tt_m), d_lo = fabs(a_lo - tt_m), d_hi = fabs(a_hi - tt_m);
            const double slack43 = (CL ? K.slack : 0x1p-43) * (fabs(Dm) + fabs(du_m - Dm) + fabs(wGm)) * rden;
            const double base2 = 2.0 * fma(fabs(wdm), rcb, rca) + slack43;
            bool ok;
            float wmx = fmaxf(fabsf(wprev[0]), fabsf(wc[0]));
#pragma unroll
            for (int j = 1; j < B; ++j) wmx = fmaxf(wmx, fmaxf(fabsf(wprev[j]), fabsf(wc[j])));
            if constexpr (CL) {
#pragma unroll
                for (int j = 0; j < B; ++j) wmx = fmaxf(wmx, fabsf(wprev2[j]));
            }
            constexpr int NPEND = blk_band(B, CL);
            const double eps_q = fma((double)wmx, o67.x, u_amax * o67.y) + (double)NPEND * rEa;
            const bool sure_q = fabs(du_m) - eps_q >= 1e-10;
            const double delta2_q = base2 + 2.0 * eps_q * rden;
// ... 14 lines not shown
#pragma unroll
                    for (int j = 0; j < B; ++j) {
                        const double2 e2 = lds_ld<double2>(lds, rbm + 64 + 32 * (2 * B + sm - j - 1) + 16);
                        ePm = fma(fabs((double)wprev2[j]), e2.x, ePm); ePm = fma(fabs((double)qprev2[j]), e2.y, ePm);
                    }
                }
                double eps = ePm;
#pragma unroll
                for (int j = 0; j + 1 < B; ++j) { eps = fma(fabs(wd[j]), ei_[j].x, eps); eps = fma(fabs(qd[j]), ei_[j].y, eps); }
                unsigned any_m = anyP;
#pragma unroll
                for (int j = 0; j + 1 < B; ++j) any_m |= j < sm ? (__float_as_uint(wc[j]) | __float_as_uint(q32s[j])) : 0u;
                eps += ((any_m << 1) != 0u) ? (double)NPEND * rEa : 0.0;
                const bool du_exact = eps == 0.0;
                const bool msq = du_exact & small;
                const bool sure = du_exact | (fabs(du_m) - eps >= 1e-10);
                const double delta2 = base2 + 2.0 * eps * rden;
                const bool far = (d_lo - d_k > delta2) & (d_hi - d_k > delta2);
                const bool first = (d_k < d_lo) & (d_k <= d_hi);
                const bool cert = (msq ? first : far) & sure;
                ok = rule1 | cert | !valid_m;
            }
            const unsigned long long bad = __ballot(!ok);
            const float q_m = rule1 ? 0.f : qk32;
            const bool st = r < B;
            if (bad == 0ull) {
                STAMP(dtb);
#pragma unroll
                for (int s = 0; s < B; ++s) qc[s] = q32s[s];
                const float qpub = SYM ? (q_m > 0.f ? -1.f : (q_m < 0.f ? 1.f : 0.f)) : q_m;
                lds_st<float2>(lds, st ? o_wq + cbq + 8 * sm : o_dummy, make_float2(w_m, qpub));
                lds_st<int2>(lds, (st & valid_m) ? o_out + ((oslot0 + sm) % kOutSteps) * 8 : o_dummy,
                             make_int2(rule1 ? K.zero_idx : ki, __float_as_int(q_m)));
                ctl_now = -1;
                if (lane == 0) lds_st<int>(lds, L.off_ctl + 4 * (b & 1), -1);
            } else
            {
            const unsigned field = (unsigned)(bad >> (lane & ~(R - 1))) & ((1u << B) - 1u);
            stop = field ? __builtin_ctz(field) : B;
            STAMP(dtb);
#pragma unroll
            for (int s = 0; s < B; ++s) qc[s] = s < stop ? q32s[s] : 0.f;
            const bool keep = sm < stop;
            const float q_st = keep ? q_m : 0.f;
            const float qpub = SYM ? (q_st > 0.f ? -1.f : (q_st < 0.f ? 1.f : 0.f)) : q_st;
            lds_st<float2>(lds, st ? o_wq + cbq + 8 * sm : o_dummy, make_float2(w_m, qpub));
            lds_st<int2>(lds, (st & keep & valid_m) ? o_out + ((oslot0 + sm) % kOutSteps) * 8 : o_dummy,
                         make_int2(rule1 ? K.zero_idx : ki, __float_as_int(q_m)));
            const unsigned long long badA = __ballot(!ok & active);
            int smin = B;
#pragma unroll
            for (int k = B - 1; k >= 0; --k) {
                unsigned long long pat = 0ull;
#pragma unroll
                for (int g = 0; g < 64 / B; ++g) pat |= 1ull << (g * B + k);
                if (badA & pat) smin = k;
            }
            ctl_now = smin < B ? smin : -1;
            if (lane == 0) lds_st<int>(lds, L.off_ctl + 4 * (b & 1), ctl_now);
            }
            if constexpr (!kHdrChain) {
                asm volatile("s_waitcnt lgkmcnt(0)" ::: "memory");
                if constexpr (!CL) { if (b + 1 < K.nblk) prefetch_headers(hnext); }
            }
            if constexpr (CL) {
                if (b + 1 < K.nblk) {
                    double xv[1] = {0.0};
                    if (NL == 4 && K.nsl > 8) cl_gather<1, NL == 4 ? 16 : 8>(K, cs, lane, xv);
                    else cl_gather<1, 8>(K, cs, lane, xv);
                    DmCur = xv[0];
                }
            }
        } else {
            STAMP(dta);
            STAMP(dtb);
            if (lane == 0) lds_st<int>(lds, L.off_ctl + 4 * (b & 1), -1);
        }

        auto decide = [&](int s, bool commit, auto inregs_tag) -> bool {
            constexpr bool IN_REGS = decltype(inregs_tag)::value;
            double am[4];
#pragma unroll
            for (int q = 0; q < 4; ++q) am[q] = (IN_REGS && r + q * R < M) ? lds_ld<double>(lds, L.off_e + 8 * (2 + r + q * R)) : kNaN;
            const int rb = tbase + s * RB;
            const double2 r01 = lds_ld<double2>(lds, rb), r23 = lds_ld<double2>(lds, rb + 16), r45 = lds_ld<double2>(lds, rb + 32);
            const double rden = r01.x, rG = r01.y, rcb = r23.x, rca = r23.y, rEa = r45.x, nrm = r45.y;
            const bool rule1 = nrm < 1e-16;
            double corr = quad_bcast(cPm, s), eps = quad_bcast(ePm, s);
            unsigned anyinc = anyP;
#pragma unroll
            for (int j = 0; j < B; ++j) {
                if (j < s) {
                    const int d = s - j;
                    const double2 h = lds_ld<double2>(lds, rb + 64 + 32 * (d - 1)), e = lds_ld<double2>(lds, rb + 64 + 32 * (d - 1) + 16);
                    const double wj = (double)wc[j], qj = (double)qc[j];
                    corr = fma(wj, h.x, corr); corr = fma(-qj, h.y, corr);
                    eps = fma(fabs(wj), e.x, eps); eps = fma(fabs(qj), e.y, eps);
                    anyinc |= __float_as_uint(wc[j]) | __float_as_uint(qc[j]);
                }
            }
            eps += ((anyinc << 1) != 0u) ? (double)blk_band(B, CL) * rEa : 0.0;
            const double wd = (double)wc[s];
            const double du = D[s] + corr;
            const bool   du_exact = eps == 0.0;
            const bool   msq = du_exact & (fabs(du) < 1e-10);
            const bool   sure = du_exact | (fabs(du) - eps >= 1e-10);
            const double wG = wd * rG;
            const double tq = (du + wG) * rden;
            const double tt = msq ? wd : tq;
            const double delta2 = 2.0 * (fma(fabs(wd), rcb, rca) + eps * rden)
                                  + (CL ? K.slack : 0x1p-43) * (fabs(D[s]) + fabs(corr) + fabs(wG)) * rden;
            int idx_l;
            double q_l;
            bool cert;
            if constexpr (SYM) {
                const bool up = tt > sym_hb, mid = tt > -sym_hb;
                idx_l = up ? M - 1 : (mid ? 1 : 0);
                q_l = up ? sym_top : (mid ? 0.0 : -sym_top);
                const double m2 = 2.0 * fmin(fabs(tt - sym_hb), fabs(tt + sym_hb));
                cert = (msq | (m2 > delta2)) & sure;
            } else {
            int c = 0;
            if constexpr (IN_REGS) {
#pragma unroll
                for (int q = 0; q < 4; ++q) c += (am[q] < tt) ? 1 : 0;
            } else {
                for (int kk = r; kk < M; kk += R) c += (lds_ld<double>(lds, L.off_e + 8 * (2 + kk)) < tt) ? 1 : 0;
            }
            const int p = sub_sumi<R>(c);
            const int oe = L.off_e + 8 * p;
            const double lolo = lds_ld<double>(lds, oe), lo = lds_ld<double>(lds, oe + 8), hi = lds_ld<double>(lds, oe + 16),
                         hihi = lds_ld<double>(lds, oe + 24);
            const double d_lo = fabs(lo - tt), d_hi = fabs(hi - tt), d_ll = fabs(lolo - tt), d_hh = fabs(hihi - tt);
            const bool at0 = p == 0, atM = p == M;
            const bool use_hi = at0 | (!atM & !(d_lo <= d_hi));
            idx_l = use_hi ? p : p - 1;
            q_l   = use_hi ? hi : lo;
            const double m2_in = fabs(d_hi - d_lo), m2_lo = d_hh - d_hi, m2_hi = d_ll - d_lo;
            const double m2 = at0 ? m2_lo : (atM ? m2_hi : m2_in);
            const bool plateau = !use_hi & (p >= 2) & !(d_ll > d_lo);
            cert = !plateau & (msq | (m2 > delta2)) & sure;
            }
            const bool valid = s < nvalid;
            const float q32 = (rule1 | !valid) ? 0.f : (float)q_l;
            const int   idx = rule1 ? K.zero_idx : idx_l;
            const bool ok = rule1 | cert | !valid;
            const bool sel = commit & ok;
            qc[s] = sel ? q32 : qc[s];
            wc[s] = (sel & !valid) ? 0.f : wc[s];
            const bool st = sel & (r == 0);
            const float qpub = SYM ? (q32 > 0.f ? -1.f : (q32 < 0.f ? 1.f : 0.f)) : q32;
            lds_st<float2>(lds, st ? o_wq + cbq + 8 * s : o_dummy, make_float2(wc[s], qpub));
            lds_st<int2>(lds, (st & valid) ? o_out + ((oslot0 + s) % kOutSteps) * 8 : o_dummy, make_int2(idx, __float_as_int(q32)));
            return ok;
        };
        using T_ = std::true_type;
        using F_ = std::false_type;
        hnext = hnext == 2 ? 0 : hnext + 1;
        STAMP(dt1);
        if (kHdrChain || b >= K.nblk) asm volatile("s_waitcnt lgkmcnt(0)" ::: "memory");
        asm volatile("s_barrier" ::: "memory");
        STAMP(dt2);
        STAMP_DO(dacc_work += dt1 - dt0; dacc_bar += dt2 - dt1; dacc_pro += dta - dt0; dacc_chain += dtb - dta;)

        for (;;) {
            const int S = ctl_now;
            if (S < 0) break;
            slot_barrier();
            if constexpr (CL) {
#pragma unroll
                for (int s = 0; s < B; ++s) D[s] = quad_bcast(DmT, s);
            } else {
#pragma unroll
            for (int s = 0; s < B; ++s) {
                double d = 0.0;
#pragma unroll
                for (int q = 0; q < NW / R; ++q) d += lds_ld<double>(lds, o_d + ((((b & 1) * NW + q * R) * B) + s) * NB * 8);
                D[s] = sub_sum<R>(d);
            }
            }
            double du = 0.0, dw = 0.0;
#pragma unroll
            for (int q = 0; q < NW / R; ++q) {
                const double2 v = lds_ld<double2>(lds, o_x2 + q * R * NB * 16);
                du += v.x; dw += v.y;
            }
            du = sub_sum<R>(du); dw = sub_sum<R>(dw);
            if constexpr (CL) {
                double xv[2] = {du, dw};
                cl_exchange<2, 4>(K, cs, lane, xv);
                du = xv[0]; dw = xv[1];
            }
            const bool mine = active && stop == S;
            if (mine) {
                const int64_t t = (int64_t)b * B + S;
                const double nrm = lds_ld<double2>(lds, tbase + S * RB + 32).y;
                float wS = 0.f;
#pragma unroll
                for (int s = 0; s < B; ++s) wS = (s == S) ? wc[s] : wS;
                const double te = dw / (nrm * nrm);
                const double t2 = fabs(du) < 1e-10 ? (double)wS : te;
                int bi = 0;
                double bq = lds_ld<double>(lds, L.off_e + 16), bdist = fabs(bq - t2);
                for (int kk = 1; kk < M; ++kk) {
                    const double ak = lds_ld<double>(lds, L.off_e + 8 * (2 + kk)), dk = fabs(ak - t2);
                    if (dk < bdist) { bdist = dk; bi = kk; bq = ak; }
                }
                const float q32 = (float)bq;
#pragma unroll
                for (int s = 0; s < B; ++s) qc[s] = (s == S) ? q32 : qc[s];
                if (r == 0) {
                    lds_st<float2>(lds, o_wq + cbq + 8 * S, make_float2(wS, SYM ? (q32 > 0.f ? -1.f : (q32 < 0.f ? 1.f : 0.f)) : q32));
                    lds_st<int2>(lds, o_out + (int)(t % kOutSteps) * 8, make_int2(bi, __float_as_int(q32)));
                    if (!shadow) ++n_fallback;
                }
            }
            int stop2 = mine ? B : stop;
#pragma unroll
            for (int s = 0; s < B; ++s) {
                if (s > S) {
                    const bool ok = in_regs ? decide(s, mine && stop2 == B, T_{}) : decide(s, mine && stop2 == B, F_{});
                    if (mine && stop2 == B && !ok) stop2 = s;
                }
            }
            stop = stop2;
            const int smin = wave_min_stop(active ? stop : B);
            ctl_now = smin < B ? smin : -1;
            if (lane == 0) lds_st<int>(lds, L.off_ctl + 4 * (b & 1), ctl_now);
            slot_barrier();
        }

#pragma unroll
        for (int j = 0; j < B; ++j) {
            if constexpr (CL) { wprev2[j] = wprev[j]; qprev2[j] = qprev[j]; }
            wprev[j] = (b < K.nblk) ? wc[j] : 0.f; qprev[j] = (b < K.nblk) ? qc[j] : 0.f;
        }
        if constexpr (kOwnFlush) {
            const int64_t done = min((int64_t)(b + 1) * B, N);
            if (b < K.nblk && (done - flushed >= kOutSteps - B + 1 || done == N)) { flush_hi = done; }
        }
    }
    if constexpr (kOwnFlush) {
        if (flush_hi > flushed) { asm volatile("s_waitcnt lgkmcnt(0)" ::: "memory"); flush(flushed, flush_hi); }
    }

    if (K.fallback_count && n_fallback && (!CL || cs.slice == 0)) atomicAdd(K.fallback_count, n_fallback);
    STAMP_DO(if (K.stamps && blockIdx.x == 0 && lane == 0) { K.stamps[16] = dacc_work; K.stamps[17] = dacc_bar; K.stamps[18] = dacc_pro; K.stamps[19] = dacc_chain; K.stamps[20] = dacc_tail; })
    slot_barrier();
    if (K.resid) {
        double tot = 0.0;
#pragma unroll
        for (int q = 0; q < NW / R; ++q) tot += lds_ld<double>(lds, o_d + q * R * B * NB * 8);
        tot = sub_sum<R>(tot);
        if constexpr (CL) {
            double xv[1] = {tot};
            cl_exchange<1, 8>(K, cs, lane, xv);
            tot = xv[0];
        }
        if (active && r == 0 && (!CL || cs.slice == 0)) K.resid[jn] = sqrt(tot);
    }
}

}

template <int G, int S, int B, int NSW, bool SYM, int NL, int CLM = 0, bool KOUT = false>
__global__ void __launch_bounds__(64 * (NSW + 1))
gpfq_blk_kernel(BlkK K)
{
    constexpr bool CL = CLM != 0;
    constexpr int NB = NL * G, KQ = 64 / G, MP = 2 * KQ * S;
    if (K.alpha->ok == 0) {
        if (K.alpha_err && blockIdx.x == 0 && threadIdx.x == 0) *K.alpha_err = 1;
        return;
    }
    ClState cs{0, 0, 0u, false, 0, 0};
    if constexpr (CL) {
        const int id = (int)blockIdx.x, j = id >> 3;
        if (K.cl_map == 0) {
            cs.slice = j % K.nsl;
// ... 47 lines not shown
constexpr int64_t kClusterMaxM = 28672;
static bool blk_chip_ok(const Options &opt)
{
    static std::atomic<int> cache[64];
    int dev = 0;
    if (hipGetDevice(&dev) != hipSuccess) { (void)hipGetLastError(); return true; }
    if (dev < 0 || dev >= 64) return false;
    int v = cache[dev].load(std::memory_order_relaxed);
    if (v == 0) {
        int cus = 0;
        bool ok = hipDeviceGetAttribute(&cus, hipDeviceAttributeMultiprocessorCount, dev) == hipSuccess && cus == 256;
        for (const char *name : {"HSA_CU_MASK", "ROC_GLOBAL_CU_MASK", "HSA_CU_MASK_SKIP_INIT"})
            if (const char *e = getenv(name)) ok = ok && e[0] == 0;
        v = ok ? 1 : 2;
        cache[dev].store(v, std::memory_order_relaxed);
    }
    const int forced = opt.blk_chip_ok;
    return forced >= 0 ? forced != 0 : v == 1;
}
static int blk_cluster_map(int nsl, const Options &opt)
{
    if (opt.blk_cluster_map >= 0) return opt.blk_cluster_map;
    if (nsl > 0 && (8 % nsl == 0 || nsl % 8 == 0)) return 1;
    return 1;
}

static BlkShape blk_shape(int64_t m, int64_t C, const Options &opt)
{
    if (m <= 0 || C <= 0) return {0, 0, 0, 0, 0, 0, 0};
    {
        const int clm = opt.blk_cluster;
        const int ns = (int)((m + 1023) / 1024);
        const bool one_round = ns <= 32 && ((C + 15) / 16 + 7) / 8 <= 32 / ns;
        const bool take = blk_chip_ok(opt) && (clm == 1 ? (m > 3072 || (m > 1536 && one_round && (m > 2048 || C > 128))) : (clm > 1 && m > clm));
        if (clm == 1 && blk_chip_ok(opt) && m > 2048 && m <= 3072 && C > 2048 && opt.blk_cluster768 != 0)
            return {4, 24, 4, 768, 11, 4, 4};
        if (take && m <= kClusterMaxM) {
            const int cn = opt.blk_cluster_nl;
            int nl = 4;
            if (cn == 1 || cn == 2) nl = cn;
            else if (cn == 0 && ((C + 7) / 8 + 7) / 8 <= 32 / ns) nl = 2;
            return {4, 32, 4, 1024, nl == 4 ? 11 : 8, nl, ns};
        }
    }
    const int nw_opt = opt.blk_sweep_waves;
    const int nw4 = nw_opt ? nw_opt : 8, nw4_long = nw_opt ? nw_opt : 11;
    const int quad = opt.blk_quad_groups;
    if (quad && C <= 2048 && (quad >= 2 || C > 128) && m > 256 && m <= 1024) {
        const int nl = C > 1024 ? 2 : 1;
        const int qw = opt.blk_quad_waves;
        const int qnw = qw ? qw : (nl == 1 ? 7 : 8);
        if (m <= 512) return {4, 16, 4, 512, qnw, nl};
        if (m <= 768) return {4, 24, 4, 768, qnw, nl};
        return {4, 32, 4, 1024, qw == 7 ? 7 : 8, nl};
    }
    if (C <= 512 && opt.blk_pair_groups) {
        const int nl = C <= 128 && opt.blk_single_groups ? 1 : 2;
        if (m > 256 && m <= 512) return {1, 4, 4, 512, 4, nl};
        if (m > 512 && m <= 1024) return {1, 8, 4, 1024, 8, nl};
        if (m > 1024 && m <= 1536) return {1, 12, 2, 1536, 8, nl};
        if (m > 1536 && m <= 2048) return {1, 16, 2, 2048, 8, nl};
        if (m > 2048 && m <= 3072) return {1, 24, 1, 3072, 8, nl};
        if (m > 3072 && m <= 4096) return {1, 32, 1, 4096, 8, nl};
        if (m > 4096 && m <= 5120) return {1, 40, 1, 5120, 8, nl};
    }
    if (m > 256 && m <= 512) return {4, 16, 4, 512, nw4, 4};
    if (m > 512 && m <= 768) return {4, 24, 4, 768, nw4, 4};
    const bool four = C <= 1024 && opt.blk_four_groups;
    if (four && m > 768 && m <= 1024) return {1, 8, 4, 1024, 8, 4};
    if (four && m > 1024 && m <= 1536) return {1, 12, 2, 1536, 8, 4};
    if (four && m > 1536 && m <= 2048) return {1, 16, 2, 2048, 8, 4};
    if (m > 768 && m <= 1024) return C <= 2048 ? BlkShape{2, 16, 4, 1024, 8, 4} : BlkShape{4, 32, 4, 1024, nw4_long, 4};
    const int64_t rounds16 = (C + 4095) / 4096, rounds8 = (C + 2047) / 2048;
    const bool wide = C > 2048 && 8 * rounds16 <= 5 * rounds8 && opt.blk_wide_groups;
    if (m > 1024 && m <= 1536) return wide ? BlkShape{4, 48, 2, 1536, 11, 4} : BlkShape{2, 24, 2, 1536, 8, 4};
    if (m > 1536 && m <= 2048) return wide ? BlkShape{4, 64, 2, 2048, 11, 4} : BlkShape{2, 32, 2, 2048, 8, 4};
    if (m > 2048 && m <= 3072) return four ? BlkShape{1, 24, 1, 3072, 8, 4} : BlkShape{2, 48, 1, 3072, 11, 4};
    if (m > 3072 && m <= 4096) return four ? BlkShape{1, 32, 1, 4096, 8, 4} : BlkShape{2, 64, 1, 4096, 11, 4};
    if (m > 4096 && m <= 5120) return {1, 40, 1, 5120, 8, 4};
    return {0, 0, 0, 0, 0, 0, 0};
}

constexpr int kGroupsByShape = 8;
static int blk_groups(const BlkShape &sh, bool sym, const Options &opt)
{
    const bool applies = sym && sh.G == 4 && sh.S == 32 && sh.B == 4 && sh.NW == 11 && sh.NL == 4;
    if (!applies) return 4;
    return opt.blk_groups ? opt.blk_groups : kGroupsByShape;
}


__global__ void gpfq_alphabet_store_kernel(DevAlphabet *out, DevAlphabet D, unsigned *counters)
{
    if (threadIdx.x == 0 && blockIdx.x == 0) *out = D;
    if (counters && threadIdx.x < 16) counters[threadIdx.x] = 0u;
}

__global__ void gpfq_alphabet_device_kernel(DevAlphabet *out, const float *__restrict__ median32, double alphabet_scalar, AlphabetArg unit, int want_sym)
{
    if (threadIdx.x != 0 || blockIdx.x != 0) return;
    form_device_alphabet(out, median32[0], alphabet_scalar, unit, want_sym);
}

static size_t blk_recs_bytes(int64_t nblk, const BlkShape &sh)
{
    return ((size_t)((nblk + 1) * sh.B + 1) * (size_t)blk_rec_bytes(sh.mp, sh.B, sh.G, sh.NS != 0) + 255) & ~(size_t)255;
}
static int64_t blk_clusters(int64_t C, const BlkShape &sh) { return (((C + sh.NL * sh.G - 1) / (sh.NL * sh.G)) + 7) / 8 * 8; }
static size_t blk_mbox_bytes(int64_t C, const BlkShape &sh) { return sh.NS > 1 ? (size_t)blk_clusters(C, sh) * 2 * sh.NS * 64 * 4 * 8 : 0; }
static size_t blk_hdrs_bytes(int64_t nblk, int B, bool CL = false) { return (size_t)((nblk + 1) * B + 1) * (size_t)blk_hdr_bytes(B, CL) + 2048; }
static size_t blk_hdrs_off(int64_t nblk, const BlkShape &sh) { return blk_recs_bytes(nblk, sh) * (size_t)(sh.NS ? sh.NS : 1); }
static size_t blk_mbox_off(int64_t nblk, const BlkShape &sh) { return blk_hdrs_off(nblk, sh) + ((blk_hdrs_bytes(nblk, sh.B, sh.NS != 0) + 255) & ~(size_t)255); }

static float blk_sym_a(const PipeArgs &a) { return (a.opt.variant >> 4) & 2 ? 0.f : blk_sym_of(a.A.a, a.A.M); }

constexpr bool blk_kout_shape(int G, int B, int NL, int CLM) { return ((G == 4 && NL == 4) || (G == 8 && NL == 2)) && B == 4 && CLM == 0; }

static const BlkInst *blk_instance(const PipeArgs &a, BlkShape *sh)
{
    *sh = blk_shape(a.m, a.C, a.opt);
    if (!sh->G) return nullptr;
    const bool sym = blk_sym_a(a) != 0.f;
    int G = sh->G, S = sh->S, NSW = sh->NW, NL = sh->NL;
    if (sh->NS && S == 24) {
        NSW = a.opt.blk_cluster768 > 0 ? a.opt.blk_cluster768 : (sym ? 11 : 8);
    } else if (blk_groups(*sh, sym, a.opt) == 8) {
        G = 8; S = 64; NL = 2;
    }
    const int row = blk_inst_find(G, S, sh->B, NSW, NL, sh->NS ? 1 : 0);
    return row < 0 || (blk_sym_only(kBlkInst[row]) && !sym) ? nullptr : &kBlkInst[row];
}

static const char *blk_family(const BlkInst &r)
{
    if (r.CLM)
        return r.G == 8 ? "gpfq_blk_kernel, cluster form (rows cut into 1024-sample slices: one workgroup of 11 sweep wavefronts + 1 decision wavefront per slice, partial dot products exchanged once per slot; eight neuron groups)"
                        : "gpfq_blk_kernel, cluster form (rows cut into 1024-sample slices: one workgroup of 8 or 11 sweep wavefronts + 1 decision wavefront per slice, partial dot products exchanged once per slot)";
    return r.G == 8 ? "gpfq_blk_kernel (4 to 11 sweep wavefronts + 1 decision wavefront per workgroup, blocks of steps per slot; eight neuron groups)"
                    : "gpfq_blk_kernel (4 to 11 sweep wavefronts + 1 decision wavefront per workgroup, blocks of steps per slot)";
}

bool blk_instance_query(const PipeArgs &a, int32_t out[8])
{
    BlkShape sh;
    const BlkInst *r = blk_instance(a, &sh);
    if (!r) return false;
    const int32_t v[8] = {r->G, r->S, r->B, r->NSW, blk_sym_a(a) != 0.f, r->NL, r->CLM, blk_kout_shape(r->G, r->B, r->NL, r->CLM)};
    std::memcpy(out, v, sizeof v);
    return true;
}
bool blk_keras_out_supported(const PipeArgs &a) { int32_t v[8]; return blk_instance_query(a, v) && v[7]; }

bool blk_supported(const PipeArgs &a)
{
    BlkShape sh;
    if (a.N < 1 || a.m < 1 || !blk_instance(a, &sh)) return false;
    if (a.A.M > 64 || !a.A.ascending) return false;
    DevAlphabet D{};
    D.M = a.A.M;
    for (int k = 0; k < a.A.M; ++k) D.a[k] = a.A.a[k];
    if (!blk_uniform(D)) return false;
    return a.N + 64 < (1LL << 31) / 64;
}

constexpr size_t kAlphaBlock = 1024;
static_assert(sizeof(DevAlphabet) <= kAlphaBlock, "alphabet block");

size_t blk_workspace_bytes(int64_t N, int64_t m, int64_t Cn, const Options &opt)
{
    if (m <= 0 || N < 0) return 0;
    size_t need = 0;
    for (int64_t C : {(int64_t)1 << 30, (int64_t)2048, (int64_t)1024, (int64_t)512, Cn > 0 ? Cn : (int64_t)1}) {
        const BlkShape sh = blk_shape(m, C, opt);
        if (!sh.G) continue;
        const int64_t nblk = (N + sh.B - 1) / sh.B;
        const size_t b = blk_mbox_off(nblk, sh) + blk_mbox_bytes(Cn, sh);
        if (b > need) need = b;
    }
    return need ? need + kAlphaBlock : 0;
}

template <int G, int S, int B, int NSW, bool SYM, int NL, int CLM = 0, bool KOUT = false>
static hipError_t launch_blk_sym(const PipeArgs &a, const BlkShape &sh, const DevAlphabet *alpha, hipStream_t stream)
{
    constexpr bool CL = CLM != 0;
    if constexpr (!KOUT && blk_kout_shape(G, B, NL, CLM)) {
        if (a.o_st != 1) return launch_blk_sym<G, S, B, NSW, SYM, NL, CLM, true>(a, sh, alpha, stream);
    }
    if (!KOUT && a.o_st != 1) return hipErrorInvalidValue;
    constexpr int NB = NL * G;
    const BlkLds L = blk_lds(sh.mp, NB, B, NSW, G, CL);
    const unsigned grid = CL ? (unsigned)(blk_clusters(a.C, sh) * sh.NS) : (unsigned)((a.C + NB - 1) / NB);
    auto *kern = gpfq_blk_kernel<G, S, B, NSW, SYM, NL, CLM, KOUT>;
    hipError_t e = ensure_dynamic_lds((const void *)kern, (size_t)L.total);
    if (e != hipSuccess) return e;
    BlkK K;
    const int64_t nblk_ = (a.N + B - 1) / B;
    char *const wbase = static_cast<char *>(a.workspace) + kAlphaBlock;
    K.recs = wbase; K.Wt = a.Wt; K.ldw = a.ldw; K.ldt = a.ldt;
    K.hdrs = K.recs + blk_hdrs_off(nblk_, sh);
    K.alpha = alpha;
    K.alpha_err = a.fallback_count ? reinterpret_cast<int *>(a.fallback_count + 1) + 1 : nullptr;
    K.nsl = CL ? sh.NS : 0; K.cl_map = blk_cluster_map(sh.NS, a.opt); K.slice_bytes = (int64_t)blk_recs_bytes(nblk_, sh); K.mbox = nullptr; K.cl_err = nullptr;
    K.u_ld = a.m; K.slack = 0x1p-43 * (double)(sh.NS > 1 ? sh.NS : 1);
    K.cl_timeout = 100000ull * (unsigned long long)a.opt.blk_cluster_timeout_ms; K.cl_fault = a.opt.blk_cluster_fault;
    if constexpr (CLM == 1) {
        char *mb = wbase + blk_mbox_off(nblk_, sh);
        const size_t mbytes = blk_mbox_bytes(a.C, sh);
        e = hipMemsetAsync(mb, 0, mbytes, stream);
        if (e != hipSuccess) return e;
        K.mbox = reinterpret_cast<unsigned long long *>(mb);
        K.cl_err = a.fallback_count ? reinterpret_cast<int *>(a.fallback_count + 1) : nullptr;
    }
    K.N = a.N; K.C = a.C; K.m = (int)a.m; K.M = a.A.M; K.zero_idx = a.A.zero_idx; K.nblk = (int)((a.N + B - 1) / B);
    K.qidx = a.qidx; K.Qt = a.Qt; K.resid = a.resid; K.u_out = a.u_out; K.fallback_count = a.fallback_count;
    K.o_sj = a.o_st == 1 ? a.N : a.o_sj; K.o_st = a.o_st;
    K.stamps = a.fallback_count ? a.fallback_count + 8 : nullptr;
    K.Xq = a.Xq; K.ldx = a.ld;
    {
        const int *pw = blk_split<G, S, NSW, NL>();
        for (int w = 0; w < 12; ++w) K.pw[w] = (unsigned char)(w < NSW ? pw[w] : 0);
    }
    hipEvent_t ev0, ev1;
    if (main_kernel_events(&ev0, &ev1))
        hipExtLaunchKernelGGL(kern, dim3(grid), dim3(64 * (NSW + 1)), (unsigned)L.total, stream, ev0, ev1, 0, K);
    else
        hipLaunchKernelGGL(kern, dim3(grid), dim3(64 * (NSW + 1)), (size_t)L.total, stream, K);
    return hipGetLastError();
}

template <int I>
static hipError_t launch_blk_row(const PipeArgs &a, const BlkShape &sh, const DevAlphabet *alpha, hipStream_t stream)
{
    constexpr BlkInst R = kBlkInst[I / 2];
    if constexpr (I % 2 || !blk_sym_only(R)) return launch_blk_sym<R.G, R.S, R.B, R.NSW, I % 2 != 0, R.NL, R.CLM>(a, sh, alpha, stream);
    else return hipErrorInvalidValue;
}
template <int... I>
static hipError_t launch_blk_rows(std::integer_sequence<int, I...>, int i, const PipeArgs &a, const BlkShape &sh, const DevAlphabet *alpha, hipStream_t stream)
{
    hipError_t e = hipErrorInvalidValue;
    (void)((i == I && ((e = launch_blk_row<I>(a, sh, alpha, stream)), true)) || ...);
    return e;
}

struct ClusterLaunchGuard {
    static std::mutex &mu() { static std::mutex m; return m; }
    struct Last { hipEvent_t ev = nullptr; hipStream_t stream = nullptr; bool any = false; };
    static Last &last(int dev) { static Last L[64]; return L[dev & 63]; }
    std::unique_lock<std::mutex> lock;
    hipStream_t stream;
    int dev = 0;
    hipError_t err = hipSuccess;
    explicit ClusterLaunchGuard(hipStream_t s) : lock(mu()), stream(s)
    {
        err = hipGetDevice(&dev);
        if (err != hipSuccess) return;
        Last &l = last(dev);
        if (!l.ev) err = hipEventCreateWithFlags(&l.ev, hipEventDisableTiming);
        if (err == hipSuccess && l.any && l.stream != stream) err = hipStreamWaitEvent(stream, l.ev, 0);
    }
    ~ClusterLaunchGuard()
    {
        if (err != hipSuccess) return;
        Last &l = last(dev);
        if (hipEventRecord(l.ev, stream) == hipSuccess) { l.any = true; l.stream = stream; }
    }
};

static hipError_t blk_alphabet(const PipeArgs &a, const DevAlphabet **alpha, hipStream_t stream)
{
    if (a.dev_alpha) {
        *alpha = a.dev_alpha;
        return a.zero_counters && a.fallback_count ? hipMemsetAsync(a.fallback_count, 0, 64, stream) : hipSuccess;
    }
    DevAlphabet D{};
    D.M = a.A.M; D.zero_idx = a.A.zero_idx;
    D.rad = std::nan("");
    for (int k = 0; k < a.A.M && k < 64; ++k) D.a[k] = a.A.a[k];
    if (!blk_uniform(D)) return hipErrorInvalidValue;
    D.sym_a = blk_sym_a(a);
    D.ok = 1;
    DevAlphabet *dst = static_cast<DevAlphabet *>(a.workspace);
    hipLaunchKernelGGL(gpfq_alphabet_store_kernel, dim3(1), dim3(64), 0, stream, dst, D,
                       a.zero_counters ? reinterpret_cast<unsigned *>(a.fallback_count) : (unsigned *)nullptr);
    *alpha = dst;
    return hipGetLastError();
}

bool blk_unit_wants_sym(const AlphabetArg &unit)
{
    PipeArgs a{};
    a.A = unit;
    return blk_sym_a(a) != 0.f;
}

hipError_t launch_alphabet_device(const float *median32, double alphabet_scalar, const AlphabetArg &unit, void *dev_alphabet, hipStream_t stream)
{
    PipeArgs a{};
    a.A = unit;
    hipLaunchKernelGGL(gpfq_alphabet_device_kernel, dim3(1), dim3(64), 0, stream, static_cast<DevAlphabet *>(dev_alphabet), median32,
                       alphabet_scalar, unit, blk_sym_a(a) != 0.f ? 1 : 0);
    return hipGetLastError();
}

hipError_t launch_blk(const PipeArgs &a, hipStream_t stream)
{
    BlkShape sh;
    const BlkInst *const inst = blk_instance(a, &sh);
    if (!inst) return hipErrorInvalidValue;
    const int64_t nblk = (a.N + sh.B - 1) / sh.B;
    const int64_t nrec = (nblk + 1) * sh.B + 1;
    const bool r64 = blk_row64(sh.G, sh.B);
    const bool do_prep = a.phase != 2, do_run = a.phase != 1;
    if (do_run || inst->CLM) note_dense_kernel(blk_family(*inst));
    const DevAlphabet *alpha = nullptr;
    hipError_t e = do_run ? blk_alphabet(a, &alpha, stream) : hipSuccess;
    if (e != hipSuccess) return e;
    char *const wbase = static_cast<char *>(a.workspace) + kAlphaBlock;
    const int sym_shape = blk_sym_a(a) != 0.f ? 1 : 0;
    const int sym_prep = a.phase == 0 ? sym_shape : 0;
    if (a.phase == 2 && sym_shape) {
        const int mps = sh.mp;
        hipLaunchKernelGGL(gpfq_blk_scale_kernel, dim3((unsigned)nrec, (unsigned)(sh.NS ? sh.NS : 1)), dim3(256), 0, stream, wbase,
                           (int64_t)blk_rec_bytes(mps, sh.B, sh.G, sh.NS != 0), blk_hdr_bytes(sh.B, sh.NS != 0), mps, sh.NS ? (int64_t)blk_recs_bytes(nblk, sh) : (int64_t)0, alpha);
        e = hipGetLastError();
        if (e != hipSuccess) return e;
    }
    const bool vec_rows = (a.ld % 4 == 0) && (((uintptr_t)a.X | (uintptr_t)a.Xq) % 16 == 0);
    const int prep_run = a.opt.blk_prep_run;
    const bool run_form = !sh.NS && vec_rows && (prep_run > 1 || (prep_run == 1 && nrec >= 2048));
    const float *nrm32 = a.nrm32;
    unsigned *zero16 = nullptr;
    if (do_prep && !nrm32 && a.nrm32_out) {
        zero16 = reinterpret_cast<unsigned *>(a.fallback_count);
        const bool fuse = run_form && sh.mp == 1024 && a.m % 4 == 0 && a.opt.blk_prep_norms;
        if (!fuse) {
            e = launch_row_norms(a.Xq, a.N, a.m, a.ld, a.nrm32_out, stream, zero16);
            if (e != hipSuccess) return e;
            nrm32 = a.nrm32_out; zero16 = nullptr;
        }
    }
    auto *prep = sh.B == 4 ? (r64 ? gpfq_blk_prep_kernel<4, true> : gpfq_blk_prep_kernel<4, false>)
                           : (sh.B == 2 ? (r64 ? gpfq_blk_prep_kernel<2, true> : gpfq_blk_prep_kernel<2, false>) : gpfq_blk_prep_kernel<1, false>);
    const int sym = sym_prep;
    if (!do_prep) {
    } else if (sh.NS) {
        hipLaunchKernelGGL((gpfq_blk_prep_kernel<4, true, true>), dim3((unsigned)nrec), dim3(256), 0, stream, a.X, a.Xq, a.ld, a.N, (int)a.m, sh.mp * sh.NS,
                           nrm32, wbase, wbase + blk_hdrs_off(nblk, sh), alpha, sym,
                           sh.NS, (int64_t)blk_recs_bytes(nblk, sh));
    } else if (run_form) {
        int run = 8;
        if (prep_run >= 4 && prep_run <= kPrepRunMax) run = prep_run;
        else {
            int64_t best = -1;
            for (int rl = 4; rl <= kPrepRunMax; ++rl) {
                const int64_t wgs = (nrec + rl - 1) / rl, cost = ((wgs + 1023) / 1024) * (1 + rl);
                if (best < 0 || cost < best) { best = cost; run = rl; }
            }
        }
        auto *prun = sh.B == 4 ? (r64 ? gpfq_blk_prep_run_kernel<4, true> : gpfq_blk_prep_run_kernel<4, false>)
                               : (sh.B == 2 ? (r64 ? gpfq_blk_prep_run_kernel<2, true> : gpfq_blk_prep_run_kernel<2, false>) : gpfq_blk_prep_run_kernel<1, false>);
        hipLaunchKernelGGL(prun, dim3((unsigned)((nrec + run - 1) / run)), dim3(256), 0, stream, a.X, a.Xq, a.ld, a.N, (int)a.m, sh.mp, nrec, run,
                           nrm32, wbase, wbase + blk_recs_bytes(nblk, sh), alpha, sym, zero16);
    } else {
        hipLaunchKernelGGL(prep, dim3((unsigned)nrec), dim3(256), 0, stream, a.X, a.Xq, a.ld, a.N, (int)a.m, sh.mp,
                           nrm32, wbase, wbase + blk_recs_bytes(nblk, sh), alpha, sym, 1, (int64_t)0);
    }
    e = hipGetLastError();
    if (e != hipSuccess || !do_run) return e;
    std::optional<ClusterLaunchGuard> one_at_a_time;
    if (inst->CLM && one_at_a_time.emplace(stream).err != hipSuccess) return one_at_a_time->err;
    return launch_blk_rows(std::make_integer_sequence<int, 2 * kBlkInsts>{}, 2 * (int)(inst - kBlkInst) + sym_shape, a, sh, alpha, stream);
}

}
```

quantized_neural_networks_amd/csrc/gpfq_capi.hip:

```cpp
#include <hip/hip_runtime.h>

#include <cmath>
#include <cstdarg>
#include <cstdio>
#include <atomic>
#include <cstring>
#include <map>
#include <mutex>
#include <utility>
#include <vector>

#include "../../include/gpfq.h"
#include "gpfq_launch.hpp"
#include "gpfq_packed.hpp"

namespace {

thread_local char g_err[512] = "";
thread_local const char *g_dense_kernel = "";
thread_local hipEvent_t g_main_ev[2] = {nullptr, nullptr};

int fail(int code, const char *fmt, ...)
{
    va_list ap;
// ... 410 lines not shown
int gpfq_dense_layer_supported(int64_t N, int64_t m, int64_t C, const double *unit_alphabet, int M)
{
    gpfq::PipeArgs pa;
    return dense_layer_supported(N, m, C, unit_alphabet, M, gpfq::options_snapshot(), &pa) ? 1 : 0;
}

int gpfq_dense_layer_keras_out_supported(int64_t N, int64_t m, int64_t C, const double *unit_alphabet, int M)
{
    gpfq::PipeArgs pa;
    return dense_layer_supported(N, m, C, unit_alphabet, M, gpfq::options_snapshot(), &pa) && gpfq::blk_keras_out_supported(pa) ? 1 : 0;
}

int gpfq_blk_instance(int64_t N, int64_t m, int64_t C, const double *alphabet, int M, int32_t out[8])
{
    gpfq::PipeArgs pa;
    if (!out || !dense_layer_supported(N, m, C, alphabet, M, gpfq::options_snapshot(), &pa)) return 0;
    return gpfq::blk_instance_query(pa, out) ? 1 : 0;
}

size_t gpfq_dense_layer_workspace_bytes(int64_t N, int64_t m, int64_t C)
{
    return dense_layer_workspace_bytes(N, m, C, gpfq::options_snapshot());
}

static int dense_layer_impl(int phase, const float *X, const float *Xq, int64_t ld, const float *nrm32,
                            const float *W, int64_t ldc, int64_t c_lo, int64_t C,
                            const void *dev_alphabet, const double *unit_alphabet, int M,
                            int64_t N, int64_t m,
                            int8_t *qidx, float *Q, int out_layout, int64_t ldo, double *resid,
                            void *workspace, size_t workspace_bytes, void *stream, const char *what)
{
    if (N < 1 || m < 1 || C < 0 || c_lo < 0)
        return fail(GPFQ_ERR_INVALID_ARG, "bad size N=%lld m=%lld C=%lld c_lo=%lld", (long long)N, (long long)m, (long long)C, (long long)c_lo);
    HostAlphabet H;
    int rc = unit_alphabet_arg(unit_alphabet, M, &H);
    if (rc != GPFQ_OK) return rc;
    if (C == 0) return GPFQ_OK;
    if (!X || !Xq) return fail(GPFQ_ERR_INVALID_ARG, "NULL pointer");
    if (phase != 1 && (!W || !dev_alphabet)) return fail(GPFQ_ERR_INVALID_ARG, "NULL pointer");
    if (ld < m) return fail(GPFQ_ERR_INVALID_ARG, "row pitch ld=%lld < m=%lld", (long long)ld, (long long)m);
    const gpfq::Options o = gpfq::options_snapshot();
    gpfq::PipeArgs pa{};
    pa.A = H.A; pa.N = N; pa.m = m; pa.C = C;
    pa.opt = o;
    if (phase != 1) {
        if (ldc < c_lo + C) return fail(GPFQ_ERR_INVALID_ARG, "kernel pitch ldc=%lld < c_lo + C=%lld", (long long)ldc, (long long)(c_lo + C));
        if (out_layout != GPFQ_LAYOUT_NEURON_MAJOR && out_layout != GPFQ_LAYOUT_KERAS) return fail(GPFQ_ERR_INVALID_ARG, "unknown output layout %d", out_layout);
        if (out_layout == GPFQ_LAYOUT_KERAS && ldo < c_lo + C) return fail(GPFQ_ERR_INVALID_ARG, "output pitch ldo=%lld < c_lo + C=%lld", (long long)ldo, (long long)(c_lo + C));
        if (out_layout == GPFQ_LAYOUT_KERAS && ldo != 1 && !gpfq::blk_keras_out_supported(pa))
            return fail(GPFQ_ERR_UNSUPPORTED, "the kernel of this shape (m=%lld, C=%lld) writes neuron-major outputs only (gpfq_dense_layer_keras_out_supported): "
                                              "ask for GPFQ_LAYOUT_NEURON_MAJOR and lay them out with gpfq_assemble_kernel_device", (long long)m, (long long)C);
    }
    gpfq::PipeArgs query;
    if (!dense_layer_supported(N, m, C, unit_alphabet, M, o, &query))
        return fail(GPFQ_ERR_UNSUPPORTED, "no block-pipelined kernel for N=%lld m=%lld C=%lld M=%d (gpfq_dense_layer_supported): use gpfq_quantize_neurons with a host alphabet",
                    (long long)N, (long long)m, (long long)C, M);
    if (!workspace || (uintptr_t)workspace % 16 != 0 || workspace_bytes < dense_layer_workspace_bytes(N, m, C, o))
        return fail(GPFQ_ERR_WORKSPACE, "%s needs %zu aligned workspace bytes", what, dense_layer_workspace_bytes(N, m, C, o));
    hipStream_t s = static_cast<hipStream_t>(stream);
    hipError_t e = hipSuccess;
    float *n32_out = nullptr;
    if (phase != 2) {
        if (!nrm32) {
            n32_out = reinterpret_cast<float *>(static_cast<char *>(workspace) + onchip_workspace_bytes(N, m, C, o));
        } else {
            e = hipMemsetAsync(workspace, 0, 64, s);
            if (e != hipSuccess) return hip_fail(e, what);
        }
    }
    pa.X = X; pa.Xq = Xq; pa.ld = ld; pa.nrm32 = nrm32; pa.nrm32_out = n32_out;
    pa.Wt = W ? W + c_lo : nullptr; pa.ldw = 1; pa.ldt = ldc;
    pa.resid = resid; pa.u_out = nullptr;
    if (out_layout == GPFQ_LAYOUT_KERAS) {
        pa.qidx = qidx ? qidx + c_lo : nullptr; pa.Qt = Q ? Q + c_lo : nullptr;
        pa.o_sj = 1; pa.o_st = ldo;
        if (ldo == 1) { pa.o_sj = N; pa.o_st = 1; }
    } else {
        pa.qidx = qidx; pa.Qt = Q;
    }
    pa.dev_alpha = static_cast<const gpfq::DevAlphabet *>(dev_alphabet);
    pa.phase = phase;
    pa.workspace = static_cast<char *>(workspace) + onchip_stats_bytes(N);
    pa.fallback_count = static_cast<unsigned long long *>(workspace);
    e = gpfq::launch_blk(pa, s);
    if (e != hipSuccess) return hip_fail(e, what);
    return (o.sync_errors && phase != 1) ? gpfq_call_status(workspace, stream) : GPFQ_OK;
}

int gpfq_quantize_dense_layer(const float *X, const float *Xq, int64_t ld, const float *nrm32,
                              const float *W, int64_t ldc, int64_t c_lo, int64_t C,
                              const void *dev_alphabet, const double *unit_alphabet, int M,
                              int64_t N, int64_t m,
                              int8_t *qidx, float *Q, int out_layout, int64_t ldo, double *resid,
                              void *workspace, size_t workspace_bytes, void *stream)
{
    return dense_layer_impl(0, X, Xq, ld, nrm32, W, ldc, c_lo, C, dev_alphabet, unit_alphabet, M, N, m, qidx, Q, out_layout, ldo, resid,
                            workspace, workspace_bytes, stream, "gpfq_quantize_dense_layer");
}

int gpfq_dense_layer_prepare(const float *X, const float *Xq, int64_t ld, const float *nrm32, const double *unit_alphabet, int M,
                             int64_t N, int64_t m, int64_t C, void *workspace, size_t workspace_bytes, void *stream)
{
    return dense_layer_impl(1, X, Xq, ld, nrm32, nullptr, 0, 0, C, nullptr, unit_alphabet, M, N, m, nullptr, nullptr, GPFQ_LAYOUT_KERAS, 0, nullptr,
                            workspace, workspace_bytes, stream, "gpfq_dense_layer_prepare");
}

int gpfq_dense_layer_run(const float *X, const float *Xq, int64_t ld,
                         const float *W, int64_t ldc, int64_t c_lo, int64_t C,
                         const void *dev_alphabet, const double *unit_alphabet, int M,
                         int64_t N, int64_t m,
                         int8_t *qidx, float *Q, int out_layout, int64_t ldo, double *resid,
                         void *workspace, size_t workspace_bytes, void *stream)
{
    return dense_layer_impl(2, X, Xq, ld, nullptr, W, ldc, c_lo, C, dev_alphabet, unit_alphabet, M, N, m, qidx, Q, out_layout, ldo, resid,
                            workspace, workspace_bytes, stream, "gpfq_dense_layer_run");
}

int gpfq_assemble_kernel_device(const void *qidx, int bits, const void *dev_alphabet, int M, int64_t N, int64_t C,
                                float *Q, void *qidx_t, void *stream)
{
    if (N < 0 || C < 0) return fail(GPFQ_ERR_INVALID_ARG, "negative size");
    if (bits != 2 && bits != 4 && bits != 8) return fail(GPFQ_ERR_INVALID_ARG, "bits must be 2, 4 or 8 (device-resident alphabets hold up to 64 members)");
    if (M < 1 || M > 64) return fail(GPFQ_ERR_UNSUPPORTED, "device-resident alphabets hold 1..64 members (got %d)", M);
    if (bits < 8 && M + 1 > (1 << bits)) return fail(GPFQ_ERR_INVALID_ARG, "%d-bit codes cannot hold an alphabet of %d", bits, M);
    if (N == 0 || C == 0) return GPFQ_OK;
    if (!qidx || !dev_alphabet) return fail(GPFQ_ERR_INVALID_ARG, "NULL pointer");
    if (N > 2147483647LL * 32) return fail(GPFQ_ERR_UNSUPPORTED, "kernel too large to assemble in one call");
    gpfq::AlphabetArg A{};
    A.M = M;
    hipError_t e = gpfq::launch_assemble(static_cast<const int8_t *>(qidx), A, N, C, bits, Q, static_cast<int8_t *>(qidx_t),
                                         static_cast<hipStream_t>(stream), nullptr, static_cast<const gpfq::DevAlphabet *>(dev_alphabet));
    return e == hipSuccess ? GPFQ_OK : hip_fail(e, "gpfq_assemble_kernel_device");
}

size_t gpfq_gram_workspace_bytes(int64_t N, int64_t m, int64_t C)
{
    if (N < 0 || m < 0 || C < 0) return 0;
    return gpfq::gram_workspace_bytes(N, m, C);
}

int gpfq_quantize_neurons_gram(const float *X, const float *Xq, int64_t ld, float *nrm32, int compute_norms,
                               const float *Wt, int64_t ldw,
                               const double *alphabet, int M, int zero_idx,
                               int64_t N, int64_t m, int64_t C,
                               void *qidx, float *Qt, double *resid, int32_t *uncertified,
                               void *workspace, size_t workspace_bytes, void *stream)
{
    if (N < 0 || m < 0 || C < 0)
        return fail(GPFQ_ERR_INVALID_ARG, "negative size N=%lld m=%lld C=%lld", (long long)N, (long long)m, (long long)C);
    HostAlphabet H;
    int rc = make_alphabet(alphabet, M, zero_idx, &H);
    if (rc != GPFQ_OK) return rc;
    if (C == 0) return GPFQ_OK;
    if (N > GPFQ_GRAM_MAX_N) return fail(GPFQ_ERR_UNSUPPORTED, "Gram path needs N <= %d (got %lld)", GPFQ_GRAM_MAX_N, (long long)N);
    if (m >= (1LL << 30)) return fail(GPFQ_ERR_UNSUPPORTED, "Gram path needs m < 2^30 (error-bound derivation)");
    if (!uncertified) return fail(GPFQ_ERR_INVALID_ARG, "uncertified is NULL");
    if (N > 0 && (!Wt || !nrm32)) return fail(GPFQ_ERR_INVALID_ARG, "Wt/nrm32 is NULL");
    if (N > 0 && m > 0 && (!X || !Xq)) return fail(GPFQ_ERR_INVALID_ARG, "X/Xq is NULL");
    if (ld < m) return fail(GPFQ_ERR_INVALID_ARG, "row pitch ld=%lld < m=%lld", (long long)ld, (long long)m);
    if (ldw < N) return fail(GPFQ_ERR_INVALID_ARG, "weight pitch ldw=%lld < N=%lld", (long long)ldw, (long long)N);
    const size_t need = gpfq::gram_workspace_bytes(N, m, C);
    if (!workspace || workspace_bytes < need || (uintptr_t)workspace % 16 != 0)
        return fail(GPFQ_ERR_WORKSPACE, "Gram path needs %zu aligned workspace bytes", need);
    gpfq::GramArgs a;
    a.X = X; a.Xq = Xq; a.ld = ld; a.nrm32 = nrm32; a.Wt = Wt; a.ldw = ldw; a.A = H.A; a.big = H.big();
    a.N = N; a.m = m; a.C = C; a.qidx = static_cast<int8_t *>(qidx); a.Qt = Qt; a.resid = resid; a.uncertified = uncertified;
    a.workspace = workspace;
    a.nrm32_out = compute_norms ? nrm32 : nullptr;
// ... 974 lines not shown
```

quantized_neural_networks_amd/csrc/gpfq_launch.hpp:

```cpp
#pragma once

#include <hip/hip_runtime.h>
#include <stddef.h>
#include <stdint.h>

#include "gpfq_device.hpp"
#include "gpfq_options.hpp"

namespace gpfq {

struct RowStats {
    double G, rden, cbound, cabs;
};

struct OnchipArgs {
    const float *X, *Xq;
    int64_t ld;
    const float *nrm32;
    const RowStats *stats = nullptr;
    unsigned long long *fallback_count = nullptr;
    int mode = 0;
    const float *Wt;
    int64_t ldw;
    AlphabetArg A;
    const AlphabetBig *big = nullptr;
    int64_t N, m, C;
    int8_t *qidx;
    float *Qt;
    double *resid;
    double *u_out;
    Options opt;
};

struct StreamArgs {
    const float *X, *Xq;
    int64_t ld;
    const float *nrm32;
    const float *Wt;
    int64_t ldw;
    AlphabetArg A;
    const AlphabetBig *big = nullptr;
    int64_t N, m, C;
    int8_t *qidx;
    float *Qt;
    double *resid;
    double *u_out;
    void *workspace;
    size_t workspace_bytes;
};

struct PipeArgs {
    const float *X, *Xq;
    int64_t ld;
    const float *nrm32;
    const float *Wt;
    int64_t ldw;
    AlphabetArg A;
    int64_t N, m, C;
    int8_t *qidx;
    float *Qt;
    double *resid;
    double *u_out;
    void *workspace;
    unsigned long long *fallback_count = nullptr;
    Options opt;
    int64_t ldt = 1;
    int64_t o_sj = 0, o_st = 1;
    const DevAlphabet *dev_alpha = nullptr;
    int zero_counters = 0;
    int phase = 0;
    float *nrm32_out = nullptr;
};
hipError_t launch_alphabet_device(const float *median32, double alphabet_scalar, const AlphabetArg &unit, void *dev_alphabet, hipStream_t stream);
bool blk_supported(const PipeArgs &a);
bool blk_keras_out_supported(const PipeArgs &a);
bool blk_instance_query(const PipeArgs &a, int32_t out[8]);
size_t blk_workspace_bytes(int64_t N, int64_t m, int64_t C, const Options &opt);
hipError_t launch_blk(const PipeArgs &a, hipStream_t stream);
bool pipe_supported(const PipeArgs &a);
size_t pipe_workspace_bytes(int64_t N, int64_t m);
hipError_t launch_pipe(const PipeArgs &a, hipStream_t stream);

hipError_t ensure_dynamic_lds(const void *kernel, size_t bytes);

void note_dense_kernel(const char *name);

bool main_kernel_events(hipEvent_t *start, hipEvent_t *stop);

hipError_t launch_onchip(const OnchipArgs &a, hipStream_t stream);
bool rows_supported(const OnchipArgs &a, int lpn);
hipError_t launch_rows(const OnchipArgs &a, int lpn, hipStream_t stream);
hipError_t launch_wide(const OnchipArgs &a, int W, hipStream_t stream);

size_t stream_workspace_bytes(int64_t N, int64_t m, int64_t C, bool need_u);
hipError_t launch_stream(const StreamArgs &a, hipStream_t stream);

struct GramArgs {
    const float *X, *Xq;
    int64_t ld;
    const float *nrm32;
    float *nrm32_out = nullptr;
    const float *Wt;
    int64_t ldw;
    AlphabetArg A;
    const AlphabetBig *big = nullptr;
    int64_t N, m, C;
    int8_t *qidx;
    float *Qt;
    double *resid;
    int32_t *uncertified;
    void *workspace;
    double slack = 1.0;
    Options opt;
};

size_t gram_workspace_bytes(int64_t N, int64_t m, int64_t C);
hipError_t launch_gram(const GramArgs &a, hipStream_t stream);

bool gram_mfma_supported(const float *X, const float *Xq, int64_t ld, int64_t N);
int64_t gram_mfma_walkers(int64_t N, int64_t m);
hipError_t launch_gram_mfma(const float *X, const float *Xq, int64_t ld, int64_t N, int64_t m, double *part, int *negflag,
                            hipStream_t stream);

struct DecideBatch {
    int64_t nch = 1, gram_cs = 0, nrm_cs = 0, w_cs = 0, out_cs = 0, unc_cs = 0, hist_cs = 0;
};
hipError_t launch_gram_reduce(const double *part, int64_t nparts, int N, double *gram, float *nrm32, int64_t nch,
                              hipStream_t stream);
struct FixSrc {
    const float *X, *Xq;
    int64_t ld, m;
    int planes;
    int64_t plane;
    int64_t pix;
    int n, H, W, oh, ow;
    int kw, sh, sw, rh, rw, pt, pl;
};
size_t gram_fix_bytes();
constexpr int kCanonNormMaxChannels = 15;
bool canonical_norms_apply(const FixSrc &src, int64_t nch);
hipError_t launch_canonical_norms(const FixSrc &src, int N, int64_t nch, float *nrm32, int64_t nrm_cs, void *fix_ws, hipStream_t stream);
hipError_t launch_gram_decide(const double *gram, const float *nrm32, const float *Wt, int64_t ldw, const AlphabetArg &A,
                              int N, int64_t C, double slack, int8_t *qidx, float *Qt, int32_t *uncertified,
                              float *q32_hist, const DecideBatch &bs, const FixSrc *src, void *fix_ws, const int *negflag,
                              hipStream_t stream, const AlphabetBig *big = nullptr);

struct ImageGramArgs {
    const float *act_w, *act_q;
    int64_t n, H, W, nch;
    int pad;
    const float *Wt;
    AlphabetArg A;
    const AlphabetBig *big = nullptr;
    int64_t F;
    int8_t *qidx;
    float *Qt;
    int32_t *uncertified;
    void *workspace;
// ... 233 lines not shown
```

quantized_neural_networks_amd/csrc/gpfq_roles.hpp:

```cpp
#pragma once

#include "gpfq_device.hpp"

namespace gpfq {
namespace {

constexpr int kSweepWaves = 8;

template <int ROR>
__device__ __forceinline__ double ror_add(double x)
{
    const int lo = __builtin_amdgcn_mov_dpp(__double2loint(x), 0x120 + ROR, 0xF, 0xF, true);
    const int hi = __builtin_amdgcn_mov_dpp(__double2hiint(x), 0x120 + ROR, 0xF, 0xF, true);
    return x + __hiloint2double(hi, lo);
}

__device__ __forceinline__ double fold32(double x, double y)
{
    const auto lo = __builtin_amdgcn_permlane32_swap((unsigned)__double2loint(x), (unsigned)__double2loint(y), false, false);
    const auto hi = __builtin_amdgcn_permlane32_swap((unsigned)__double2hiint(x), (unsigned)__double2hiint(y), false, false);
    return __hiloint2double((int)hi[0], (int)lo[0]) + __hiloint2double((int)hi[1], (int)lo[1]);
}

__device__ __forceinline__ double fold16(double x, double y)
// ... 211 lines not shown
    "v_pk_fma_f32 v[156:157], " W2 ", " Q ", v[156:157] op_sel:[1,0,0]\n\t"                                        \
    "v_pk_fma_f32 " X ", " W3 ", " Q ", " X " op_sel:[1,0,0]\n\t"                                                  \
    "v_cvt_f64_f32 " Q ", v152\n\tv_cvt_f64_f32 v[152:153], v153\n\t"                                              \
    "v_cvt_f64_f32 v[158:159], v154\n\tv_cvt_f64_f32 v[154:155], v155\n\t"                                         \
    "v_cvt_f64_f32 v[160:161], v156\n\tv_cvt_f64_f32 v[156:157], v157\n\t"                                         \
    "v_cvt_f64_f32 v[162:163], " XL "\n\tv_cvt_f64_f32 " X ", " XH "\n\t"                                          \
    "v_add_f64 %[u01], %[u01], v[152:153]\n\tv_add_f64 %[u10], %[u10], v[158:159]\n\t"                             \
    "v_add_f64 %[u11], %[u11], v[154:155]\n\tv_add_f64 %[u20], %[u20], v[160:161]\n\t"                             \
    "v_add_f64 %[u21], %[u21], v[156:157]\n\tv_add_f64 %[u30], %[u30], v[162:163]\n\t"                             \
    "v_add_f64 %[u00], %[u00], " Q "\n\tv_add_f64 %[u31], %[u31], " X "\n\t"
    asm volatile("ds_read_b64 v[148:149], %[ax]\n\tds_read_b64 v[150:151], %[aq]\n\t"
                 "ds_read_b128 v[34:37], %[aw]\n\tds_read_b128 v[30:33], %[aw] offset:32\n\t"
                 "ds_read_b128 v[26:29], %[aw] offset:64\n\tds_read_b128 v[22:25], %[aw] offset:96\n\t"
                 "ds_read_b64 v[164:165], %[ax] offset:%[r1]\n\tds_read_b64 v[166:167], %[aq] offset:%[r1]\n\t"
                 "ds_read_b128 %[w2], %[aw] offset:16\n\tds_read_b128 %[w3], %[aw] offset:48\n\t"
                 "ds_read_b128 %[w4], %[aw] offset:80\n\tds_read_b128 %[w5], %[aw] offset:112\n\t"
                 "ds_read_b128 %[d], %[ad]\n\t"
                 "ds_read_b64 %[x2], %[ax] offset:%[r2]\n\tds_read_b64 %[q2], %[aq] offset:%[r2]\n\t"
                 "s_waitcnt lgkmcnt(12)\n\tv_pk_mul_f32 v[152:153], v[148:149], v[34:35] op_sel_hi:[1,0]\n\t"
                 "s_waitcnt lgkmcnt(11)\n\tv_pk_mul_f32 v[154:155], v[148:149], v[30:31] op_sel_hi:[1,0]\n\t"
                 "s_waitcnt lgkmcnt(10)\n\tv_pk_mul_f32 v[156:157], v[148:149], v[26:27] op_sel_hi:[1,0]\n\t"
                 "s_waitcnt lgkmcnt(9)\n\tv_pk_mul_f32 v[148:149], v[148:149], v[22:23] op_sel_hi:[1,0]\n\t"
                 GPFQ_TOP_PAIR_STEP("v[34:35]", "v[30:31]", "v[26:27]", "v[22:23]", "v[148:149]", "v148", "v149", "v[150:151]")
                 "s_waitcnt lgkmcnt(7)\n\tv_pk_mul_f32 v[152:153], v[164:165], v[36:37] op_sel_hi:[1,0]\n\t"
                 "v_pk_mul_f32 v[154:155], v[164:165], v[32:33] op_sel_hi:[1,0]\n\t"
                 "v_pk_mul_f32 v[156:157], v[164:165], v[28:29] op_sel_hi:[1,0]\n\t"
                 "v_pk_mul_f32 v[164:165], v[164:165], v[24:25] op_sel_hi:[1,0]\n\t"
                 GPFQ_TOP_PAIR_STEP("v[36:37]", "v[32:33]", "v[28:29]", "v[24:25]", "v[164:165]", "v164", "v165", "v[166:167]")
                 "s_waitcnt lgkmcnt(0)"
                 : "=&{v[34:37]}"(w01[0]), "=&{v[30:33]}"(w01[1]), "=&{v[26:29]}"(w01[2]), "=&{v[22:25]}"(w01[3]),
                   [w2] "=&v"(w23[0]), [w3] "=&v"(w23[1]), [w4] "=&v"(w23[2]), [w5] "=&v"(w23[3]), [d] "=&v"(d), [x2] "=&v"(x2), [q2] "=&v"(q2),
                   [u00] "+v"(u00), [u01] "+v"(u01), [u10] "+v"(u10), [u11] "+v"(u11), [u20] "+v"(u20), [u21] "+v"(u21), [u30] "+v"(u30), [u31] "+v"(u31)
                 : [ax] "v"((unsigned)(uintptr_t)px), [aq] "v"((unsigned)(uintptr_t)pq), [aw] "v"((unsigned)(uintptr_t)pwq), [ad] "v"((unsigned)(uintptr_t)pd),
                   [r1] "i"(RB), [r2] "i"(2 * RB)
                 : "memory", "v148", "v149", "v150", "v151", "v152", "v153", "v154", "v155", "v156", "v157", "v158", "v159", "v160", "v161", "v162",
                   "v163", "v164", "v165", "v166", "v167");
#undef GPFQ_TOP_PAIR_STEP
}
template <int RB>
__device__ __forceinline__ void slot_top_sym2(nf4 (&w01)[2], nf4 (&w23)[2], nf4 &x2, nf4 &q2, nd2 (&d)[2],
                                              double &u00, double &u01, double &u02, double &u03, double &u10, double &u11, double &u12, double &u13,
                                              lchar *px, lchar *pq, lchar *pwq, lchar *pd)
{
    static_assert(2 * RB + 16 <= 65536, "the rows of pair-steps 1 and 2 are reached through the 16-bit offset field");
#define GPFQ_TOP2_PAIR_STEP(W0, W1, XA, XAL, XAH, XB, XBL, XBH, QA, QB)                                            \
    "v_pk_fma_f32 v[160:161], " W0 ", " QA ", v[160:161] op_sel:[1,0,0]\n\t"                                       \
    "v_pk_fma_f32 v[162:163], " W0 ", " QB ", v[162:163] op_sel:[1,0,0]\n\t"                                       \
    "v_pk_fma_f32 " XA ", " W1 ", " QA ", " XA " op_sel:[1,0,0]\n\t"                                               \
    "v_pk_fma_f32 " XB ", " W1 ", " QB ", " XB " op_sel:[1,0,0]\n\t"                                               \
    "v_cvt_f64_f32 " QA ", v160\n\tv_cvt_f64_f32 v[160:161], v161\n\t"                                             \
    "v_cvt_f64_f32 v[164:165], " XAL "\n\tv_cvt_f64_f32 " XA ", " XAH "\n\t"                                       \
    "v_cvt_f64_f32 " QB ", v162\n\tv_cvt_f64_f32 v[162:163], v163\n\t"                                             \
    "v_cvt_f64_f32 v[166:167], " XBL "\n\tv_cvt_f64_f32 " XB ", " XBH "\n\t"                                       \
    "v_add_f64 %[u01], %[u01], v[160:161]\n\tv_add_f64 %[u10], %[u10], v[164:165]\n\t"                             \
    "v_add_f64 %[u11], %[u11], " XA "\n\tv_add_f64 %[u02], %[u02], " QB "\n\t"                                     \
    "v_add_f64 %[u03], %[u03], v[162:163]\n\tv_add_f64 %[u12], %[u12], v[166:167]\n\t"                             \
    "v_add_f64 %[u00], %[u00], " QA "\n\tv_add_f64 %[u13], %[u13], " XB "\n\t"
    asm volatile("ds_read_b128 v[144:147], %[ax]\n\tds_read_b128 v[148:151], %[aq]\n\t"
                 "ds_read_b128 v[26:29], %[aw]\n\tds_read_b128 v[22:25], %[aw] offset:32\n\t"
                 "ds_read_b128 v[152:155], %[ax] offset:%[r1]\n\tds_read_b128 v[156:159], %[aq] offset:%[r1]\n\t"
                 "ds_read_b128 %[w2], %[aw] offset:16\n\tds_read_b128 %[w3], %[aw] offset:48\n\t"
                 "ds_read_b128 %[d0], %[ad]\n\tds_read_b128 %[d1], %[ad] offset:16\n\t"
                 "ds_read_b128 %[x2], %[ax] offset:%[r2]\n\tds_read_b128 %[q2], %[aq] offset:%[r2]\n\t"
                 "s_waitcnt lgkmcnt(9)\n\tv_pk_mul_f32 v[160:161], v[144:145], v[26:27] op_sel_hi:[1,0]\n\t"
                 "v_pk_mul_f32 v[162:163], v[146:147], v[26:27] op_sel_hi:[1,0]\n\t"
                 "s_waitcnt lgkmcnt(8)\n\tv_pk_mul_f32 v[144:145], v[144:145], v[22:23] op_sel_hi:[1,0]\n\t"
                 "v_pk_mul_f32 v[146:147], v[146:147], v[22:23] op_sel_hi:[1,0]\n\t"
                 GPFQ_TOP2_PAIR_STEP("v[26:27]", "v[22:23]", "v[144:145]", "v144", "v145", "v[146:147]", "v146", "v147", "v[148:149]", "v[150:151]")
                 "s_waitcnt lgkmcnt(6)\n\tv_pk_mul_f32 v[160:161], v[152:153], v[28:29] op_sel_hi:[1,0]\n\t"
                 "v_pk_mul_f32 v[162:163], v[154:155], v[28:29] op_sel_hi:[1,0]\n\t"
                 "v_pk_mul_f32 v[152:153], v[152:153], v[24:25] op_sel_hi:[1,0]\n\t"
                 "v_pk_mul_f32 v[154:155], v[154:155], v[24:25] op_sel_hi:[1,0]\n\t"
                 GPFQ_TOP2_PAIR_STEP("v[28:29]", "v[24:25]", "v[152:153]", "v152", "v153", "v[154:155]", "v154", "v155", "v[156:157]", "v[158:159]")
                 "s_waitcnt lgkmcnt(0)"
                 : "=&{v[26:29]}"(w01[0]), "=&{v[22:25]}"(w01[1]), [w2] "=&v"(w23[0]), [w3] "=&v"(w23[1]), [d0] "=&v"(d[0]), [d1] "=&v"(d[1]),
                   [x2] "=&v"(x2), [q2] "=&v"(q2),
                   [u00] "+v"(u00), [u01] "+v"(u01), [u02] "+v"(u02), [u03] "+v"(u03), [u10] "+v"(u10), [u11] "+v"(u11), [u12] "+v"(u12), [u13] "+v"(u13)
                 : [ax] "v"((unsigned)(uintptr_t)px), [aq] "v"((unsigned)(uintptr_t)pq), [aw] "v"((unsigned)(uintptr_t)pwq), [ad] "v"((unsigned)(uintptr_t)pd),
                   [r1] "i"(RB), [r2] "i"(2 * RB)
                 : "memory", "v144", "v145", "v146", "v147", "v148", "v149", "v150", "v151", "v152", "v153", "v154", "v155", "v156", "v157", "v158",
                   "v159", "v160", "v161", "v162", "v163", "v164", "v165", "v166", "v167");
#undef GPFQ_TOP2_PAIR_STEP
}
__device__ __forceinline__ int lds_read_now(lchar *p)
{
    int v;
    asm volatile("ds_read_b32 %0, %1\n\ts_waitcnt lgkmcnt(0)" : "=&v"(v) : "v"((unsigned)(uintptr_t)p) : "memory");
    return v;
}

}
}
```

Measured before the change: 6.524 billion weights/s.

## Interleave block record rows into per-wavefront owned units for G=8 tiles

Adds an alternative record layout in which the x, q and next-row d streams of each 32-sample unit are interleaved per block row, so each sweep wavefront fetches only the contiguous 1 KiB pieces it consumes, with swizzled d offsets. The prep and scale kernels write through a new address map, headers go only to the separate header array, and the sweep kernel computes offsets and piece issue from the owned layout. A second option issues next-step row LDS reads early in a split inline-asm pair. A prepare/run consistency check is added to the C API.

```diff
diff --git a/quantized_neural_networks_amd/csrc/gpfq_blk.hip b/quantized_neural_networks_amd/csrc/gpfq_blk.hip
--- a/quantized_neural_networks_amd/csrc/gpfq_blk.hip
+++ b/quantized_neural_networks_amd/csrc/gpfq_blk.hip
@@ -1,3 +1,4 @@
+#include <algorithm>
 #include <atomic>
 #include <cmath>
 #include <cstring>
@@ -30,24 +31,62 @@
 __host__ __device__ constexpr bool blk_row64(int G, int B) { return B > 1 && G > 1; }
 __host__ __device__ constexpr int64_t blk_rec_bytes(int64_t mp, int B, int G, bool CL = false) { return blk_hdr_bytes(B, CL) + (blk_row64(G, B) ? 16 : 12) * mp; }
 
+constexpr int kOwnRowsShip = 3 + 4 * 0;
+#ifdef GPFQ_BLK_OWN_ROWS
+constexpr int kOwnRows = GPFQ_BLK_OWN_ROWS;
+#else
+constexpr int kOwnRows = kOwnRowsShip;
+#endif
+__host__ __device__ constexpr bool blk_own_rows(int G, bool CL = false) { return G == 8 && ((kOwnRows >> (CL ? 2 : 0)) & 1) != 0; }
+__host__ __device__ constexpr bool blk_own_early(int G, bool CL = false) { return blk_own_rows(G, CL) && ((kOwnRows >> (CL ? 3 : 1)) & 1) != 0; }
+struct BlkOwn {
+    static constexpr int kUnit = 32, kX = 0, kQ = 128, kD = 256, kStep = 512;
+    __host__ __device__ static constexpr int d_off(int w, int s) { return kD + 32 * ((w / 4) ^ (4 * (s & 1))) + 8 * (w % 4); }
+};
+struct BlkRecMap {
+    int own;
+    int hdr, mps;
+    int64_t rec_bytes;
+    int64_t tile_bytes;
+    int64_t nrows;
+    int64_t stream_bytes;
+    __host__ __device__ int64_t grp(int64_t t, int i, int B) const { return (t / B) * tile_bytes + ((int64_t)(i / BlkOwn::kUnit) * B + t % B) * BlkOwn::kStep; }
+    __host__ __device__ int64_t x(int64_t t, int i, int B) const { return own ? grp(t, i, B) + BlkOwn::kX + 4 * (i % BlkOwn::kUnit) : t * rec_bytes + hdr + 4 * (int64_t)i; }
+    __host__ __device__ int64_t q(int64_t t, int i, int B) const { return own ? grp(t, i, B) + BlkOwn::kQ + 4 * (i % BlkOwn::kUnit) : t * rec_bytes + hdr + 4 * ((int64_t)mps + i); }
+    __host__ __device__ int64_t d(int64_t t, int i, int B) const { return own ? grp(t, i, B) + BlkOwn::d_off(i % BlkOwn::kUnit, (int)(t % B)) : t * rec_bytes + hdr + 8 * ((int64_t)mps + i); }
+    __host__ __device__ int64_t d32(int64_t t, int i) const { return t * rec_bytes + hdr + 8 * (int64_t)mps + 4 * (int64_t)i; }
+};
+__host__ __device__ constexpr int64_t blk_tile_bytes(int64_t mp, int B, int G, bool CL = false)
+{
+    return blk_own_rows(G, CL) ? (mp / BlkOwn::kUnit) * B * BlkOwn::kStep : B * blk_rec_bytes(mp, B, G, CL);
+}
+__host__ __device__ inline BlkRecMap blk_rec_map(int64_t nblk, int mps, int B, int G, bool CL)
+{
+    BlkRecMap M;
+    M.own = blk_own_rows(G, CL) ? 1 : 0;
+    M.hdr = blk_hdr_bytes(B, CL); M.mps = mps;
+    M.rec_bytes = blk_rec_bytes(mps, B, G, CL);
+    M.tile_bytes = blk_tile_bytes(mps, B, G, CL);
+    M.nrows = (nblk + 1) * B + (M.own ? 0 : 1);
+    M.stream_bytes = M.own ? (nblk + 1) * M.tile_bytes : M.nrows * M.rec_bytes;
+    return M;
+}
+
 template <int B, bool R64, bool CL = false>
 __global__ void __launch_bounds__(256)
 gpfq_blk_prep_kernel(const float *__restrict__ X, const float *__restrict__ Xq, int64_t ld, int64_t N, int m, int mp,
                      const float *__restrict__ nrm32, char *__restrict__ recs, char *__restrict__ hdrs,
-                     const DevAlphabet *__restrict__ alpha, int sym, int nsl, int64_t slice_bytes)
+                     const DevAlphabet *__restrict__ alpha, int sym, int nsl, int64_t slice_bytes, BlkRecMap RM)
 {
     const float sym_a = sym ? alpha->sym_a : 0.f;
-    constexpr int GREC = R64 ? 2 : 1;
     constexpr int ND = blk_band(B, CL), NV = 3 + 4 * ND;
     constexpr int DN = CL ? 2 * B : B;
     __shared__ double sm[4][((NV + 3) & ~3) + 1];
     const int64_t t = blockIdx.x;
     constexpr int hdr = blk_hdr_bytes(B, CL);
     const int mps = nsl > 1 ? mp / nsl : mp;
-    char *rb = recs + t * blk_rec_bytes(mps, B, GREC, CL);
-    float  *ox = reinterpret_cast<float *>(rb + hdr);
-    float  *oq = ox + mps;
-    double *od = reinterpret_cast<double *>(rb + hdr + 8 * (int64_t)mps);
+    char *rb = recs + t * RM.rec_bytes;
+    const bool rows = t < RM.nrows;
     const bool has_prev = t >= B && t - B < N, has_cur = t < N, has_next = t + DN < N;
     const float *px = X + (t - B) * ld, *pq = Xq + (t - B) * ld;
     const float *cx = X + t * ld, *cq = Xq + t * ld;
@@ -85,16 +124,17 @@
 #pragma unroll
             for (int d = 1; d <= ND; ++d) { bx4[d - 1] = row(X, t - d); bq4[d - 1] = row(Xq, t - d); }
             const int sl = nsl > 1 ? i / mps : 0, il = i - sl * mps;
-            const int64_t so = (int64_t)sl * slice_bytes;
-            float *oxs = reinterpret_cast<float *>(reinterpret_cast<char *>(ox) + so), *oqs = reinterpret_cast<float *>(reinterpret_cast<char *>(oq) + so);
-            double *ods = reinterpret_cast<double *>(reinterpret_cast<char *>(od) + so);
-            *reinterpret_cast<float4 *>(oxs + il) = xp;
-            *reinterpret_cast<float4 *>(oqs + il) = sym_a != 0.f ? make_float4(__fmul_rn(sym_a, qp.x), __fmul_rn(sym_a, qp.y), __fmul_rn(sym_a, qp.z), __fmul_rn(sym_a, qp.w)) : qp;
-            if constexpr (R64) {
-                *reinterpret_cast<double2 *>(ods + il) = make_double2((double)qn.x, (double)qn.y);
-                *reinterpret_cast<double2 *>(ods + il + 2) = make_double2((double)qn.z, (double)qn.w);
-            } else {
-                *reinterpret_cast<float4 *>(reinterpret_cast<float *>(ods) + il) = qn;
+            char *rs = recs + (int64_t)sl * slice_bytes;
+            if (rows) {
+                *reinterpret_cast<float4 *>(rs + RM.x(t, il, B)) = xp;
+                *reinterpret_cast<float4 *>(rs + RM.q(t, il, B)) = sym_a != 0.f ? make_float4(__fmul_rn(sym_a, qp.x), __fmul_rn(sym_a, qp.y), __fmul_rn(sym_a, qp.z), __fmul_rn(sym_a, qp.w)) : qp;
+                if constexpr (R64) {
+                    double2 *od2 = reinterpret_cast<double2 *>(rs + RM.d(t, il, B));
+                    od2[0] = make_double2((double)qn.x, (double)qn.y);
+                    od2[1] = make_double2((double)qn.z, (double)qn.w);
+                } else {
+                    *reinterpret_cast<float4 *>(rs + RM.d32(t, il)) = qn;
+                }
             }
             float b1[ND], b2[ND];
 #pragma unroll
@@ -114,13 +154,13 @@
         for (int i = threadIdx.x; i < mp; i += 256) {
             const bool in = i < m;
             const int sl = nsl > 1 ? i / mps : 0, il = i - sl * mps;
-            const int64_t so = (int64_t)sl * slice_bytes;
-            float *oxs = reinterpret_cast<float *>(reinterpret_cast<char *>(ox) + so), *oqs = reinterpret_cast<float *>(reinterpret_cast<char *>(oq) + so);
-            double *ods = reinterpret_cast<double *>(reinterpret_cast<char *>(od) + so);
-            oxs[il] = (has_prev && in) ? px[i] : 0.f;
-            oqs[il] = (has_prev && in) ? (sym_a != 0.f ? __fmul_rn(sym_a, pq[i]) : pq[i]) : 0.f;
-            if constexpr (R64) ods[il] = (double)((has_next && in) ? nq[i] : 0.f);
-            else reinterpret_cast<float *>(ods)[il] = (has_next && in) ? nq[i] : 0.f;
+            char *rs = recs + (int64_t)sl * slice_bytes;
+            if (rows) {
+                *reinterpret_cast<float *>(rs + RM.x(t, il, B)) = (has_prev && in) ? px[i] : 0.f;
+                *reinterpret_cast<float *>(rs + RM.q(t, il, B)) = (has_prev && in) ? (sym_a != 0.f ? __fmul_rn(sym_a, pq[i]) : pq[i]) : 0.f;
+                if constexpr (R64) *reinterpret_cast<double *>(rs + RM.d(t, il, B)) = (double)((has_next && in) ? nq[i] : 0.f);
+                else *reinterpret_cast<float *>(rs + RM.d32(t, il)) = (has_next && in) ? nq[i] : 0.f;
+            }
             if (has_cur && in) {
                 float b1[ND], b2[ND];
 #pragma unroll
@@ -154,14 +194,14 @@
 #pragma unroll
         for (int d = 1; d <= ND; ++d) { e1 += total(5 + 4 * (d - 1)); e2 += total(6 + 4 * (d - 1)); }
         st.sE1 = 0x1p-23 * e1 * up * up; st.sE2 = 0x1p-23 * e2 * up * up;
-        for (int sl = 0; sl < (nsl > 1 ? nsl : 1); ++sl) *reinterpret_cast<BlkStats *>(rb + (int64_t)sl * slice_bytes) = st;
+        for (int sl = 0; sl < (nsl > 1 ? nsl : 1) && !RM.own; ++sl) *reinterpret_cast<BlkStats *>(rb + (int64_t)sl * slice_bytes) = st;
         *reinterpret_cast<BlkStats *>(hdrs + t * hdr) = st;
     } else if (threadIdx.x <= ND) {
         const int d = threadIdx.x;
         BandEntry e;
         e.H1 = total(3 + 4 * (d - 1)); e.H2 = total(4 + 4 * (d - 1));
         e.E1 = 0x1p-23 * total(5 + 4 * (d - 1)) * up; e.E2 = 0x1p-23 * total(6 + 4 * (d - 1)) * up;
-        for (int sl = 0; sl < (nsl > 1 ? nsl : 1); ++sl) *reinterpret_cast<BandEntry *>(rb + (int64_t)sl * slice_bytes + 64 + 32 * (d - 1)) = e;
+        for (int sl = 0; sl < (nsl > 1 ? nsl : 1) && !RM.own; ++sl) *reinterpret_cast<BandEntry *>(rb + (int64_t)sl * slice_bytes + 64 + 32 * (d - 1)) = e;
         *reinterpret_cast<BandEntry *>(hdrs + t * hdr + 64 + 32 * (d - 1)) = e;
     }
 }
@@ -171,9 +211,8 @@
 __global__ void __launch_bounds__(256)
 gpfq_blk_prep_run_kernel(const float *__restrict__ X, const float *__restrict__ Xq, int64_t ld, int64_t N, int m, int mp, int64_t nrec, int RUN,
                          const float *__restrict__ nrm32, char *__restrict__ recs, char *__restrict__ hdrs,
-                         const DevAlphabet *__restrict__ alpha, int sym, unsigned *__restrict__ zero16)
-{
-    constexpr int GREC = R64 ? 2 : 1;
+                         const DevAlphabet *__restrict__ alpha, int sym, unsigned *__restrict__ zero16, BlkRecMap RM)
+{
     constexpr int ND = blk_band(B), NV = 3 + 4 * ND, NP = (NV + 3) & ~3;
     constexpr int hdr = blk_hdr_bytes(B);
     __shared__ double sm[kPrepRunMax][4][NP + 1];
@@ -187,7 +226,7 @@
     for (int k = threadIdx.x; k < RUN * 4 * (NP + 1); k += 256) (&sm[0][0][0])[k] = 0.0;
     __syncthreads();
     const float4 z4 = make_float4(0.f, 0.f, 0.f, 0.f);
-    const int64_t rbytes = blk_rec_bytes(mp, B, GREC);
+    const int64_t rbytes = RM.rec_bytes;
     for (int i = 4 * threadIdx.x; i < mp; i += 1024) {
         auto row = [&](const float *base, int64_t r) -> float4 {
             if (r < 0 || r >= N || i >= m) return z4;
@@ -203,18 +242,16 @@
         for (int r = 0; r < RUN; ++r) {
             const int64_t t = t0 + r;
             const float4 xc1 = r + 1 < RUN ? row(X, t + 1) : z4, qc1 = r + 1 < RUN ? row(Xq, t + 1) : z4, qn1 = r + 1 < RUN ? row(Xq, t + 1 + B) : z4;
-            if (t < nrec) {
-                char *rb = recs + t * rbytes;
-                float *ox = reinterpret_cast<float *>(rb + hdr), *oq = ox + mp;
+            if (t < nrec && t < RM.nrows) {
                 const float4 xp = wx[B - 1], qp = wq[B - 1];
-                *reinterpret_cast<float4 *>(ox + i) = xp;
-                *reinterpret_cast<float4 *>(oq + i) = sym_a != 0.f ? make_float4(__fmul_rn(sym_a, qp.x), __fmul_rn(sym_a, qp.y), __fmul_rn(sym_a, qp.z), __fmul_rn(sym_a, qp.w)) : qp;
+                *reinterpret_cast<float4 *>(recs + RM.x(t, i, B)) = xp;
+                *reinterpret_cast<float4 *>(recs + RM.q(t, i, B)) = sym_a != 0.f ? make_float4(__fmul_rn(sym_a, qp.x), __fmul_rn(sym_a, qp.y), __fmul_rn(sym_a, qp.z), __fmul_rn(sym_a, qp.w)) : qp;
                 if constexpr (R64) {
-                    double *od = reinterpret_cast<double *>(rb + hdr + 8 * (int64_t)mp);
-                    *reinterpret_cast<double2 *>(od + i) = make_double2((double)qn.x, (double)qn.y);
-                    *reinterpret_cast<double2 *>(od + i + 2) = make_double2((double)qn.z, (double)qn.w);
+                    double2 *od2 = reinterpret_cast<double2 *>(recs + RM.d(t, i, B));
+                    od2[0] = make_double2((double)qn.x, (double)qn.y);
+                    od2[1] = make_double2((double)qn.z, (double)qn.w);
                 } else {
-                    *reinterpret_cast<float4 *>(reinterpret_cast<float *>(rb + hdr + 8 * (int64_t)mp) + i) = qn;
+                    *reinterpret_cast<float4 *>(recs + RM.d32(t, i)) = qn;
                 }
             }
             if (own_norms) {
@@ -285,27 +322,30 @@
 #pragma unroll
             for (int d = 1; d <= ND; ++d) { e1 += total(5 + 4 * (d - 1)); e2 += total(6 + 4 * (d - 1)); }
             st.sE1 = 0x1p-23 * e1 * up * up; st.sE2 = 0x1p-23 * e2 * up * up;
-            *reinterpret_cast<BlkStats *>(rb) = st;
+            if (!RM.own) *reinterpret_cast<BlkStats *>(rb) = st;
             *reinterpret_cast<BlkStats *>(hdrs + t * hdr) = st;
         } else {
             const int d = e;
             BandEntry be;
             be.H1 = total(3 + 4 * (d - 1)); be.H2 = total(4 + 4 * (d - 1));
             be.E1 = 0x1p-23 * total(5 + 4 * (d - 1)) * up; be.E2 = 0x1p-23 * total(6 + 4 * (d - 1)) * up;
-            *reinterpret_cast<BandEntry *>(rb + 64 + 32 * (d - 1)) = be;
+            if (!RM.own) *reinterpret_cast<BandEntry *>(rb + 64 + 32 * (d - 1)) = be;
             *reinterpret_cast<BandEntry *>(hdrs + t * hdr + 64 + 32 * (d - 1)) = be;
         }
     }
 }
 
 __global__ void __launch_bounds__(256)
-gpfq_blk_scale_kernel(char *__restrict__ recs, int64_t rec_bytes, int hdr, int mps, int64_t slice_bytes, const DevAlphabet *__restrict__ alpha)
-{
+gpfq_blk_scale_kernel(char *__restrict__ recs, BlkRecMap RM, int B, int64_t slice_bytes, const DevAlphabet *__restrict__ alpha)
+{
+    const int64_t t = blockIdx.x;
+    if (t >= RM.nrows) return;
     const float a = alpha->sym_a;
-    float4 *row = reinterpret_cast<float4 *>(recs + (int64_t)blockIdx.y * slice_bytes + (int64_t)blockIdx.x * rec_bytes + hdr + 4 * (int64_t)mps);
-    for (int i = threadIdx.x; i < mps / 4; i += 256) {
-        const float4 v = row[i];
-        row[i] = make_float4(__fmul_rn(a, v.x), __fmul_rn(a, v.y), __fmul_rn(a, v.z), __fmul_rn(a, v.w));
+    char *base = recs + (int64_t)blockIdx.y * slice_bytes;
+    for (int i = threadIdx.x; i < RM.mps / 4; i += 256) {
+        float4 *p = reinterpret_cast<float4 *>(base + RM.q(t, 4 * i, B));
+        const float4 v = *p;
+        *p = make_float4(__fmul_rn(a, v.x), __fmul_rn(a, v.y), __fmul_rn(a, v.z), __fmul_rn(a, v.w));
     }
 }
 
@@ -323,7 +363,7 @@
 {
     BlkLds L;
     const int nw = blk_slots(nsw, nb);
-    L.tile_bytes = B * (int)blk_rec_bytes(mp, B, G, CL);
+    L.tile_bytes = (int)blk_tile_bytes(mp, B, G, CL);
     L.tile_pitch = (L.tile_bytes + 1023) & ~1023;
     int o = 2 * L.tile_pitch;
     L.off_w = o;    o += 2 * nb * B * 4;    o = (o + 15) & ~15;
@@ -540,11 +580,16 @@
     constexpr int PU = G == 8 ? 2 : 1;
     static_assert(PW % PU == 0, "whole units per wavefront");
     auto pair_off = [](int p) { return PU * (p / PU) * KQ + p % PU; };
-    const int o_x  = HDR + 8 * (pbase + PU * kq);
-    int o_q = o_x + 4 * MP;
+    constexpr bool kOwn = blk_own_rows(G, CL);
+    static_assert(!kOwn || (PU == 2 && KQ * 2 * PU == BlkOwn::kUnit && blk_row64(G, B)), "a unit is what the k-lanes read with one 16-byte request each");
+    constexpr int SB = kOwn ? BlkOwn::kStep : RB;
+    constexpr int UB32 = kOwn ? B * BlkOwn::kStep : 8 * PU * KQ, UB64 = kOwn ? B * BlkOwn::kStep : (blk_row64(G, B) ? 16 : 8) * PU * KQ;
+    const int wown = (2 * pbase / BlkOwn::kUnit) * B * BlkOwn::kStep;
+    const int o_x  = kOwn ? wown + BlkOwn::kX + 16 * kq : HDR + 8 * (pbase + PU * kq);
+    int o_q = kOwn ? wown + BlkOwn::kQ + 16 * kq : o_x + 4 * MP;
     asm volatile("" : "+v"(o_q));
     constexpr int DB = blk_row64(G, B) ? 16 : 8;
-    const int o_d  = HDR + 8 * MP + DB * (pbase + PU * kq);
+    const int o_d  = kOwn ? wown + BlkOwn::d_off(4 * kq, lane & 3) : HDR + 8 * MP + DB * (pbase + PU * kq);
     using DRaw = std::conditional_t<blk_row64(G, B), double2, float2>;
     auto ld_d = [&](int off) -> DRaw { return lds_ld<DRaw>(lds, off); };
     auto to_d2 = [](const DRaw &v) -> double2 { return make_double2((double)v.x, (double)v.y); };
@@ -558,13 +603,15 @@
 #pragma unroll
         for (int e = 0; e < 2 * PW; ++e) u[i][e] = 0.0;
 
+    constexpr int OWNP = (PW / PU) * B * BlkOwn::kStep >> 10;
+    static_assert(!kOwn || (PW / PU) * B * BlkOwn::kStep % 1024 == 0, "a wavefront's run of the tile is whole 1 KiB pieces");
     constexpr int NPIECES = (B * RB + 1023) >> 10;
-    constexpr int PER_MIN = NPIECES / NSW;
+    constexpr int PER_MIN = kOwn ? OWNP : NPIECES / NSW;
     constexpr int PTS = PW >= 2 ? 2 : 1;
     constexpr int PPP = PER_MIN / (PTS * B) > 0 ? PER_MIN / (PTS * B) : 1;
     const unsigned lane16 = (unsigned)lane * 16u;
     auto issue_piece = [&](int b1, int k) {
-        const int pc = wave + NSW * k;
+        const int pc = kOwn ? (wown >> 10) + k : wave + NSW * k;
         glds16_s(K.recs + (CL ? cs.rec_off : (int64_t)0) + (int64_t)b1 * L.tile_bytes + ((int64_t)pc << 10), lane16,
                  ldsT_addr + (unsigned)(b1 & 1) * (unsigned)L.tile_pitch + ((unsigned)pc << 10));
     };
@@ -584,7 +631,7 @@
             glds16_s(K.hdrs + (int64_t)b2 * B * HDR + ((int64_t)wave << 10), lane16,
                      lds_addr(lds_generic + L.off_hr) + (unsigned)buf * (unsigned)L.hr_pitch + ((unsigned)wave << 10));
     };
-    for (int k = 0; wave + NSW * k < NPIECES; ++k) issue_piece(0, k);
+    for (int k = 0; kOwn ? k < OWNP : wave + NSW * k < NPIECES; ++k) issue_piece(0, k);
     load_weights(0);
     load_headers(0, 0); load_headers(1, 1);
     dma_wait();
@@ -600,6 +647,13 @@
     constexpr bool kTopSym = kBatchTop && SYM;
     constexpr int kPrioForm = CL ? (kPrio >> 2) & 3 : kPrio & 3;
     constexpr bool kPrioUp = kTopSym && G == 8 && (kPrioForm & 1) != 0;
+    constexpr bool kEarly = kTopSym && blk_own_early(G, CL);
+    [[maybe_unused]] auto rows_early = [&](int b1) {
+        if constexpr (kEarly) {
+            const int tb1 = (b1 & 1) * L.tile_pitch;
+            slot_rows_early<SB, BlkOwn::kQ - BlkOwn::kX>(lds + tb1 + o_x, lds + tb1 + (lane & 3) * SB + o_d);
+        }
+    };
     constexpr int NUW = PW / PU;
     constexpr bool kLateHdr = kTopSym && NUW >= 2 && (kTop3 & 1) != 0, kLateW = kTopSym && NUW >= 2 && (kTop3 & 2) != 0;
     constexpr int kHdrStep = NUW >= 3 ? 8 : 6, kWStep = NUW >= 3 ? 10 : 7;
@@ -659,9 +713,10 @@
                     double t0 = u[n][0], t1 = u[n][1];
 #pragma unroll
                     for (int pp = 1; pp < PW; ++pp) { t0 = (p == pp) ? u[n][2 * pp] : t0; t1 = (p == pp) ? u[n][2 * pp + 1] : t1; }
+                    const int po = kOwn ? (p / PU) * UB32 + 8 * (p % PU) : 8 * pair_off(p);
                     for (int j = 0; j < S; ++j) {
-                        const int rb = nb_ + j * RB;
-                        const float2 x2 = lds_ld<float2>(lds, rb + o_x + 8 * pair_off(p)), q2 = lds_ld<float2>(lds, rb + o_q + 8 * pair_off(p));
+                        const int rb = nb_ + j * SB;
+                        const float2 x2 = lds_ld<float2>(lds, rb + o_x + po), q2 = lds_ld<float2>(lds, rb + o_q + po);
                         const float2 wq = lds_ld<float2>(lds, o_wq + cbq + (n * B + j) * 8);
                         if constexpr (SYM) {
                             t0 += (double)__fmaf_rn(wq.y, q2.x, __fmul_rn(wq.x, x2.x));
@@ -671,8 +726,8 @@
                             t1 += (double)__fsub_rn(__fmul_rn(wq.x, x2.y), __fmul_rn(wq.y, q2.y));
                         }
                     }
-                    const int rb = nb_ + S * RB;
-                    const float2 x2 = lds_ld<float2>(lds, rb + o_x + 8 * pair_off(p));
+                    const int rb = nb_ + S * SB;
+                    const float2 x2 = lds_ld<float2>(lds, rb + o_x + po);
                     float2 q2;
                     if constexpr (SYM) {
                         const int i0 = 2 * (pbase + pair_off(p) + PU * kq);
@@ -681,7 +736,7 @@
                         q2.x = i0 < mrow ? xr[i0] : 0.f;
                         q2.y = i0 + 1 < mrow ? xr[i0 + 1] : 0.f;
                     } else {
-                        q2 = lds_ld<float2>(lds, rb + o_q + 8 * pair_off(p));
+                        q2 = lds_ld<float2>(lds, rb + o_q + po);
                     }
                     eu[n] = fma((double)q2.x, t0, eu[n]);
                     eu[n] = fma((double)q2.y, t1, eu[n]);
@@ -698,6 +753,7 @@
         }
     };
     if constexpr (kBatchTop) __builtin_amdgcn_s_waitcnt(0);
+    if constexpr (kEarly) rows_early(0);
     for (int b = 0; b < nslots; ++b) {
         STAMP(st0);
         STAMP_DO(if (b) acc_t += st0 - st5;)
@@ -805,7 +861,7 @@
         };
         (void)unit2_products; (void)unit2_accumulate_ahead;
         if constexpr (kFused) {
-            const int rbm = tbase + (G == 8 ? lane & 3 : ng) * RB + o_d;
+            const int rbm = tbase + (G == 8 ? lane & 3 : ng) * SB + o_d;
             constexpr int NU = PW / PU;
             constexpr bool kRows2 = kTopSym && G == 8 && (kPkAhead & 1) != 0;
             constexpr bool kPkA = kRows2 && (kPkAhead & 2) != 0;
@@ -817,7 +873,7 @@
             float2 fwq[B][NL];
             XRow xbuf[PF], qbuf[PF];
             DRow dcur;
-            auto row_off = [&](int i, bool q) { return tbase + (i % B) * RB + (q ? o_q : o_x) + 8 * PU * (i / B) * KQ; };
+            auto row_off = [&](int i, bool q) { return tbase + (i % B) * SB + (q ? o_q : o_x) + UB32 * (i / B); };
             auto ld_drow = [&](int off) -> DRow {
                 if constexpr (PU == 2) return DRow{{lds_ld<double2>(lds, off), lds_ld<double2>(lds, off + 16)}};
                 else return lds_ld<double2>(lds, off);
@@ -837,8 +893,12 @@
                 nf4 w01[2], w23[2], x2n, q2n;
                 nd2 d01[2];
                 __builtin_amdgcn_s_setprio(2);
-                slot_top_sym2<RB>(w01, w23, x2n, q2n, d01, u[0][0], u[0][1], u[0][2], u[0][3], u[1][0], u[1][1], u[1][2], u[1][3],
-                                  lds + row_off(0, false), lds + row_off(0, true), lds + o_wq + pbq, lds + rbm);
+                if constexpr (kEarly) {
+                    slot_top_sym2_late(w01, w23, x2n, q2n, d01, u[0][0], u[0][1], u[0][2], u[0][3], u[1][0], u[1][1], u[1][2], u[1][3], lds + o_wq + pbq);
+                } else {
+                    slot_top_sym2<SB>(w01, w23, x2n, q2n, d01, u[0][0], u[0][1], u[0][2], u[0][3], u[1][0], u[1][1], u[1][2], u[1][3],
+                                      lds + row_off(0, false), lds + row_off(0, true), lds + o_wq + pbq, lds + rbm);
+                }
                 __builtin_amdgcn_s_waitcnt(0xC07F);
                 __builtin_memcpy(&xbuf[0], &x2n, sizeof(XRow)); __builtin_memcpy(&qbuf[0], &q2n, sizeof(XRow));
                 if constexpr (kRows2) { xbuf[PF - 1] = lds_ld<XRow>(lds, row_off(3, false)); qbuf[PF - 1] = lds_ld<XRow>(lds, row_off(3, true)); }
@@ -928,7 +988,7 @@
                         else __builtin_amdgcn_s_setprio(0);
                     }
                 }
-                if (p > 0) dcur = ld_drow(rbm + DB * PU * p * KQ);
+                if (p > 0) dcur = ld_drow(rbm + UB64 * p);
 #pragma unroll
                 for (int st = 0; st < B; ++st) {
                     const int ips = p * B + st;
@@ -985,7 +1045,7 @@
                 }
                 dprev = dcur;
             }
-            for (int k = PTS * B * PPP < PER_MIN ? PTS * B * PPP : PER_MIN; wave + NSW * k < NPIECES; ++k) issue_piece(bn, k);
+            for (int k = PTS * B * PPP < PER_MIN ? PTS * B * PPP : PER_MIN; kOwn ? k < OWNP : wave + NSW * k < NPIECES; ++k) issue_piece(bn, k);
             STAMP(st2);
 #pragma unroll
             for (int i = 0; i < NM; ++i) mfma_pair(NU - 1, i, dprev);
@@ -1066,7 +1126,7 @@
                 }
             }
         }
-        for (int k = PTS * B * PPP < PER_MIN ? PTS * B * PPP : PER_MIN; wave + NSW * k < NPIECES; ++k) issue_piece(bn, k);
+        for (int k = PTS * B * PPP < PER_MIN ? PTS * B * PPP : PER_MIN; kOwn ? k < OWNP : wave + NSW * k < NPIECES; ++k) issue_piece(bn, k);
         STAMP(st2);
         if constexpr (kMfmaD) {
             if (b + 1 < nslots) {
@@ -1155,7 +1215,12 @@
         dma_wait();
         STAMP(st4);
         if constexpr (kPrioUp) __builtin_amdgcn_s_setprio(2);
-        slot_barrier();
+        if constexpr (kEarly) {
+            if (b + 1 < nslots) { rows_early(b + 1); asm volatile("s_barrier" ::: "memory"); }
+            else slot_barrier();
+        } else {
+            slot_barrier();
+        }
         STAMP(st5);
         STAMP_DO(acc_dma += st1 - st0; acc_u += st2 - st1; acc_d += st3 - st2; acc_w += st4 - st3; acc_b += st5 - st4;)
 
@@ -1168,6 +1233,9 @@
         }
         if (__builtin_amdgcn_readfirstlane(ctl) >= 0) {
             slow_path(b, ctl);
+            if constexpr (kEarly) {
+                if (b + 1 < nslots) rows_early(b + 1);
+            }
             if constexpr (kHoist) {
                 if (b + 1 < nslots) { preload_wq(b + 1); preload_rows(b + 1); }
             }
@@ -1364,6 +1432,8 @@
     const int smh = lane & (B - 1);
     constexpr bool kHdrChain = NSW == 7;
     constexpr int BI = B > 1 ? B - 1 : 1, HDRB = blk_hdr_bytes(B, CL);
+    constexpr bool kOwnH = blk_own_rows(G, CL);
+    constexpr int HS = kOwnH ? HDRB : RB;
     double2 g01 = make_double2(0.0, 0.0);
     double2 ghp[B];
     double2 ghi[BI];
@@ -1385,7 +1455,7 @@
     for (int b = 0; b < nslots; ++b) {
         STAMP(dt0);
         STAMP_DO(if (b) dacc_tail += dt0 - dt2;)
-        const int tbase = (b & 1) * L.tile_pitch;
+        const int hbase = kOwnH ? L.off_hr + (hnext == 0 ? 2 : hnext - 1) * L.hr_pitch : (b & 1) * L.tile_pitch;
         const int cbq = (b & 1) * NB * B * 8;
         float  wc[B], qc[B];
         double D[B];
@@ -1424,7 +1494,7 @@
             if constexpr (CL) {
                 prefetch_headers(b % 3);
 #pragma unroll
-                for (int j = 0; j < B; ++j) hp2[j] = lds_ld<double2>(lds, tbase + sm * RB + 64 + 32 * (2 * B + sm - j - 1));
+                for (int j = 0; j < B; ++j) hp2[j] = lds_ld<double2>(lds, hbase + sm * HS + 64 + 32 * (2 * B + sm - j - 1));
             }
             if constexpr (kOwnFlush) {
                 if (flush_hi > flushed) {
@@ -1487,7 +1557,7 @@
             double A[B];
 #pragma unroll
             for (int s = 0; s < B; ++s) A[s] = quad_bcast(Am, s);
-            const int rbm = tbase + sm * RB;
+            const int rbm = hbase + sm * HS;
             const double2 o23 = lds_ld<double2>(lds, rbm + 16);
             const double rEa = lds_ld<double>(lds, rbm + 32);
             const double2 o67 = lds_ld<double2>(lds, rbm + 48);
@@ -1668,7 +1738,7 @@
             double am[4];
 #pragma unroll
             for (int q = 0; q < 4; ++q) am[q] = (IN_REGS && r + q * R < M) ? lds_ld<double>(lds, L.off_e + 8 * (2 + r + q * R)) : kNaN;
-            const int rb = tbase + s * RB;
+            const int rb = hbase + s * HS;
             const double2 r01 = lds_ld<double2>(lds, rb), r23 = lds_ld<double2>(lds, rb + 16), r45 = lds_ld<double2>(lds, rb + 32);
             const double rden = r01.x, rG = r01.y, rcb = r23.x, rca = r23.y, rEa = r45.x, nrm = r45.y;
             const bool rule1 = nrm < 1e-16;
@@ -1780,7 +1850,7 @@
             const bool mine = active && stop == S;
             if (mine) {
                 const int64_t t = (int64_t)b * B + S;
-                const double nrm = lds_ld<double2>(lds, tbase + S * RB + 32).y;
+                const double nrm = lds_ld<double2>(lds, hbase + S * HS + 32).y;
                 float wS = 0.f;
 #pragma unroll
                 for (int s = 0; s < B; ++s) wS = (s == S) ? wc[s] : wS;
@@ -1994,10 +2064,10 @@
 }
 
 constexpr int kGroupsByShape = 8;
+static bool blk_groups_shape(const BlkShape &sh) { return sh.G == 4 && sh.S == 32 && sh.B == 4 && sh.NW == 11 && sh.NL == 4; }
 static int blk_groups(const BlkShape &sh, bool sym, const Options &opt)
 {
-    const bool applies = sym && sh.G == 4 && sh.S == 32 && sh.B == 4 && sh.NW == 11 && sh.NL == 4;
-    if (!applies) return 4;
+    if (!sym || !blk_groups_shape(sh)) return 4;
     return opt.blk_groups ? opt.blk_groups : kGroupsByShape;
 }
 
@@ -2016,7 +2086,10 @@
 
 static size_t blk_recs_bytes(int64_t nblk, const BlkShape &sh)
 {
-    return ((size_t)((nblk + 1) * sh.B + 1) * (size_t)blk_rec_bytes(sh.mp, sh.B, sh.G, sh.NS != 0) + 255) & ~(size_t)255;
+    size_t need = (size_t)blk_rec_map(nblk, sh.mp, sh.B, sh.G, sh.NS != 0).stream_bytes;
+    if (blk_groups_shape(sh))
+        need = std::max(need, (size_t)blk_rec_map(nblk, sh.mp, sh.B, 8, sh.NS != 0).stream_bytes);
+    return (need + 255) & ~(size_t)255;
 }
 static int64_t blk_clusters(int64_t C, const BlkShape &sh) { return (((C + sh.NL * sh.G - 1) / (sh.NL * sh.G)) + 7) / 8 * 8; }
 static size_t blk_mbox_bytes(int64_t C, const BlkShape &sh) { return sh.NS > 1 ? (size_t)blk_clusters(C, sh) * 2 * sh.NS * 64 * 4 * 8 : 0; }
@@ -2073,6 +2146,35 @@
     for (int k = 0; k < a.A.M; ++k) D.a[k] = a.A.a[k];
     if (!blk_uniform(D)) return false;
     return a.N + 64 < (1LL << 31) / 64;
+}
+
+constexpr int kPreparedMax = 64;
+struct PreparedRow { const void *ws; int row; };
+static std::mutex &prepared_mu() { static std::mutex m; return m; }
+static PreparedRow *prepared_rows() { static PreparedRow r[kPreparedMax] = {}; return r; }
+void blk_note_prepared(const PipeArgs &a)
+{
+    BlkShape sh;
+    const BlkInst *inst = blk_instance(a, &sh);
+    if (!inst) return;
+    std::lock_guard<std::mutex> g(prepared_mu());
+    PreparedRow *r = prepared_rows();
+    static int next = 0;
+    int at = -1;
+    for (int i = 0; i < kPreparedMax; ++i) if (r[i].ws == a.workspace) at = i;
+    if (at < 0) { at = next; next = (next + 1) % kPreparedMax; }
+    r[at] = {a.workspace, (int)(inst - kBlkInst)};
+}
+bool blk_prepared_matches(const PipeArgs &a, int *prepared, int *now)
+{
+    BlkShape sh;
+    const BlkInst *inst = blk_instance(a, &sh);
+    if (!inst) return true;
+    std::lock_guard<std::mutex> g(prepared_mu());
+    const PreparedRow *r = prepared_rows();
+    for (int i = 0; i < kPreparedMax; ++i)
+        if (r[i].ws == a.workspace && a.workspace) { *prepared = r[i].row; *now = (int)(inst - kBlkInst); return *prepared == *now; }
+    return true;
 }
 
 constexpr size_t kAlphaBlock = 1024;
@@ -2232,10 +2334,10 @@
     char *const wbase = static_cast<char *>(a.workspace) + kAlphaBlock;
     const int sym_shape = blk_sym_a(a) != 0.f ? 1 : 0;
     const int sym_prep = a.phase == 0 ? sym_shape : 0;
+    const BlkRecMap RM = blk_rec_map(nblk, sh.mp, sh.B, inst->G, inst->CLM != 0);
     if (a.phase == 2 && sym_shape) {
-        const int mps = sh.mp;
         hipLaunchKernelGGL(gpfq_blk_scale_kernel, dim3((unsigned)nrec, (unsigned)(sh.NS ? sh.NS : 1)), dim3(256), 0, stream, wbase,
-                           (int64_t)blk_rec_bytes(mps, sh.B, sh.G, sh.NS != 0), blk_hdr_bytes(sh.B, sh.NS != 0), mps, sh.NS ? (int64_t)blk_recs_bytes(nblk, sh) : (int64_t)0, alpha);
+                           RM, sh.B, sh.NS ? (int64_t)blk_recs_bytes(nblk, sh) : (int64_t)0, alpha);
         e = hipGetLastError();
         if (e != hipSuccess) return e;
     }
@@ -2260,7 +2362,7 @@
     } else if (sh.NS) {
         hipLaunchKernelGGL((gpfq_blk_prep_kernel<4, true, true>), dim3((unsigned)nrec), dim3(256), 0, stream, a.X, a.Xq, a.ld, a.N, (int)a.m, sh.mp * sh.NS,
                            nrm32, wbase, wbase + blk_hdrs_off(nblk, sh), alpha, sym,
-                           sh.NS, (int64_t)blk_recs_bytes(nblk, sh));
+                           sh.NS, (int64_t)blk_recs_bytes(nblk, sh), RM);
     } else if (run_form) {
         int run = 8;
         if (prep_run >= 4 && prep_run <= kPrepRunMax) run = prep_run;
@@ -2274,10 +2376,10 @@
         auto *prun = sh.B == 4 ? (r64 ? gpfq_blk_prep_run_kernel<4, true> : gpfq_blk_prep_run_kernel<4, false>)
                                : (sh.B == 2 ? (r64 ? gpfq_blk_prep_run_kernel<2, true> : gpfq_blk_prep_run_kernel<2, false>) : gpfq_blk_prep_run_kernel<1, false>);
         hipLaunchKernelGGL(prun, dim3((unsigned)((nrec + run - 1) / run)), dim3(256), 0, stream, a.X, a.Xq, a.ld, a.N, (int)a.m, sh.mp, nrec, run,
-                           nrm32, wbase, wbase + blk_recs_bytes(nblk, sh), alpha, sym, zero16);
+                           nrm32, wbase, wbase + blk_recs_bytes(nblk, sh), alpha, sym, zero16, RM);
     } else {
         hipLaunchKernelGGL(prep, dim3((unsigned)nrec), dim3(256), 0, stream, a.X, a.Xq, a.ld, a.N, (int)a.m, sh.mp,
-                           nrm32, wbase, wbase + blk_recs_bytes(nblk, sh), alpha, sym, 1, (int64_t)0);
+                           nrm32, wbase, wbase + blk_recs_bytes(nblk, sh), alpha, sym, 1, (int64_t)0, RM);
     }
     e = hipGetLastError();
     if (e != hipSuccess || !do_run) return e;
diff --git a/quantized_neural_networks_amd/csrc/gpfq_capi.hip b/quantized_neural_networks_amd/csrc/gpfq_capi.hip
--- a/quantized_neural_networks_amd/csrc/gpfq_capi.hip
+++ b/quantized_neural_networks_amd/csrc/gpfq_capi.hip
@@ -516,8 +516,15 @@
     pa.phase = phase;
     pa.workspace = static_cast<char *>(workspace) + onchip_stats_bytes(N);
     pa.fallback_count = static_cast<unsigned long long *>(workspace);
+    if (phase == 2) {
+        int prepared = -1, now = -1;
+        if (!gpfq::blk_prepared_matches(pa, &prepared, &now))
+            return fail(GPFQ_ERR_INVALID_ARG, "%s: the workspace was prepared for row %d of the block kernel's table, this call resolves to row %d "
+                                              "(the options changed between gpfq_dense_layer_prepare and gpfq_dense_layer_run); nothing was computed", what, prepared, now);
+    }
     e = gpfq::launch_blk(pa, s);
     if (e != hipSuccess) return hip_fail(e, what);
+    if (phase == 1) gpfq::blk_note_prepared(pa);
     return (o.sync_errors && phase != 1) ? gpfq_call_status(workspace, stream) : GPFQ_OK;
 }
 
diff --git a/quantized_neural_networks_amd/csrc/gpfq_launch.hpp b/quantized_neural_networks_amd/csrc/gpfq_launch.hpp
--- a/quantized_neural_networks_amd/csrc/gpfq_launch.hpp
+++ b/quantized_neural_networks_amd/csrc/gpfq_launch.hpp
@@ -74,6 +74,8 @@
 hipError_t launch_alphabet_device(const float *median32, double alphabet_scalar, const AlphabetArg &unit, void *dev_alphabet, hipStream_t stream);
 bool blk_supported(const PipeArgs &a);
 bool blk_keras_out_supported(const PipeArgs &a);
+void blk_note_prepared(const PipeArgs &a);
+bool blk_prepared_matches(const PipeArgs &a, int *prepared, int *now);
 bool blk_instance_query(const PipeArgs &a, int32_t out[8]);
 size_t blk_workspace_bytes(int64_t N, int64_t m, int64_t C, const Options &opt);
 hipError_t launch_blk(const PipeArgs &a, hipStream_t stream);
diff --git a/quantized_neural_networks_amd/csrc/gpfq_roles.hpp b/quantized_neural_networks_amd/csrc/gpfq_roles.hpp
--- a/quantized_neural_networks_amd/csrc/gpfq_roles.hpp
+++ b/quantized_neural_networks_amd/csrc/gpfq_roles.hpp
@@ -317,6 +317,58 @@
                    "v159", "v160", "v161", "v162", "v163", "v164", "v165", "v166", "v167");
 #undef GPFQ_TOP2_PAIR_STEP
 }
+template <int SB, int QO>
+__device__ __forceinline__ void slot_rows_early(lchar *px, lchar *pd)
+{
+    static_assert(2 * SB + QO + 16 <= 65536, "the rows of pair-steps 1 and 2 are reached through the 16-bit offset field");
+    asm volatile("s_waitcnt lgkmcnt(0)\n\t"
+                 "ds_read_b128 v[144:147], %[ax]\n\tds_read_b128 v[148:151], %[ax] offset:%[q0]\n\t"
+                 "ds_read_b128 v[152:155], %[ax] offset:%[r1]\n\tds_read_b128 v[156:159], %[ax] offset:%[q1]\n\t"
+                 "ds_read_b128 v[128:131], %[ad]\n\tds_read_b128 v[132:135], %[ad] offset:16\n\t"
+                 "ds_read_b128 v[136:139], %[ax] offset:%[r2]\n\tds_read_b128 v[140:143], %[ax] offset:%[q2]"
+                 :: [ax] "v"((unsigned)(uintptr_t)px), [ad] "v"((unsigned)(uintptr_t)pd),
+                    [q0] "i"(QO), [r1] "i"(SB), [q1] "i"(SB + QO), [r2] "i"(2 * SB), [q2] "i"(2 * SB + QO)
+                 : "memory", "v128", "v129", "v130", "v131", "v132", "v133", "v134", "v135", "v136", "v137", "v138", "v139", "v140", "v141", "v142", "v143",
+                   "v144", "v145", "v146", "v147", "v148", "v149", "v150", "v151", "v152", "v153", "v154", "v155", "v156", "v157", "v158", "v159");
+}
+__device__ __forceinline__ void slot_top_sym2_late(nf4 (&w01)[2], nf4 (&w23)[2], nf4 &x2, nf4 &q2, nd2 (&d)[2],
+                                                   double &u00, double &u01, double &u02, double &u03, double &u10, double &u11, double &u12, double &u13,
+                                                   lchar *pwq)
+{
+#define GPFQ_TOP2_PAIR_STEP(W0, W1, XA, XAL, XAH, XB, XBL, XBH, QA, QB)                                            \
+    "v_pk_fma_f32 v[160:161], " W0 ", " QA ", v[160:161] op_sel:[1,0,0]\n\t"                                       \
+    "v_pk_fma_f32 v[162:163], " W0 ", " QB ", v[162:163] op_sel:[1,0,0]\n\t"                                       \
+    "v_pk_fma_f32 " XA ", " W1 ", " QA ", " XA " op_sel:[1,0,0]\n\t"                                               \
+    "v_pk_fma_f32 " XB ", " W1 ", " QB ", " XB " op_sel:[1,0,0]\n\t"                                               \
+    "v_cvt_f64_f32 " QA ", v160\n\tv_cvt_f64_f32 v[160:161], v161\n\t"                                             \
+    "v_cvt_f64_f32 v[164:165], " XAL "\n\tv_cvt_f64_f32 " XA ", " XAH "\n\t"                                       \
+    "v_cvt_f64_f32 " QB ", v162\n\tv_cvt_f64_f32 v[162:163], v163\n\t"                                             \
+    "v_cvt_f64_f32 v[166:167], " XBL "\n\tv_cvt_f64_f32 " XB ", " XBH "\n\t"                                       \
+    "v_add_f64 %[u01], %[u01], v[160:161]\n\tv_add_f64 %[u10], %[u10], v[164:165]\n\t"                             \
+    "v_add_f64 %[u11], %[u11], " XA "\n\tv_add_f64 %[u02], %[u02], " QB "\n\t"                                     \
+    "v_add_f64 %[u03], %[u03], v[162:163]\n\tv_add_f64 %[u12], %[u12], v[166:167]\n\t"                             \
+    "v_add_f64 %[u00], %[u00], " QA "\n\tv_add_f64 %[u13], %[u13], " XB "\n\t"
+    asm volatile("ds_read_b128 v[26:29], %[aw]\n\tds_read_b128 v[22:25], %[aw] offset:32\n\t"
+                 "ds_read_b128 %[w2], %[aw] offset:16\n\tds_read_b128 %[w3], %[aw] offset:48\n\t"
+                 "s_waitcnt lgkmcnt(3)\n\tv_pk_mul_f32 v[160:161], v[144:145], v[26:27] op_sel_hi:[1,0]\n\t"
+                 "v_pk_mul_f32 v[162:163], v[146:147], v[26:27] op_sel_hi:[1,0]\n\t"
+                 "s_waitcnt lgkmcnt(2)\n\tv_pk_mul_f32 v[144:145], v[144:145], v[22:23] op_sel_hi:[1,0]\n\t"
+                 "v_pk_mul_f32 v[146:147], v[146:147], v[22:23] op_sel_hi:[1,0]\n\t"
+                 GPFQ_TOP2_PAIR_STEP("v[26:27]", "v[22:23]", "v[144:145]", "v144", "v145", "v[146:147]", "v146", "v147", "v[148:149]", "v[150:151]")
+                 "v_pk_mul_f32 v[160:161], v[152:153], v[28:29] op_sel_hi:[1,0]\n\t"
+                 "v_pk_mul_f32 v[162:163], v[154:155], v[28:29] op_sel_hi:[1,0]\n\t"
+                 "v_pk_mul_f32 v[152:153], v[152:153], v[24:25] op_sel_hi:[1,0]\n\t"
+                 "v_pk_mul_f32 v[154:155], v[154:155], v[24:25] op_sel_hi:[1,0]\n\t"
+                 GPFQ_TOP2_PAIR_STEP("v[28:29]", "v[24:25]", "v[152:153]", "v152", "v153", "v[154:155]", "v154", "v155", "v[156:157]", "v[158:159]")
+                 "s_waitcnt lgkmcnt(0)"
+                 : "=&{v[26:29]}"(w01[0]), "=&{v[22:25]}"(w01[1]), [w2] "=&v"(w23[0]), [w3] "=&v"(w23[1]),
+                   "=&{v[128:131]}"(d[0]), "=&{v[132:135]}"(d[1]), "=&{v[136:139]}"(x2), "=&{v[140:143]}"(q2),
+                   [u00] "+v"(u00), [u01] "+v"(u01), [u02] "+v"(u02), [u03] "+v"(u03), [u10] "+v"(u10), [u11] "+v"(u11), [u12] "+v"(u12), [u13] "+v"(u13)
+                 : [aw] "v"((unsigned)(uintptr_t)pwq)
+                 : "memory", "v144", "v145", "v146", "v147", "v148", "v149", "v150", "v151", "v152", "v153", "v154", "v155", "v156", "v157", "v158",
+                   "v159", "v160", "v161", "v162", "v163", "v164", "v165", "v166", "v167");
+#undef GPFQ_TOP2_PAIR_STEP
+}
 __device__ __forceinline__ int lds_read_now(lchar *p)
 {
     int v;
```

Result: faster. 6.645 billion weights/s (median of 6 runs) (+1.9%).
